# kfkq/DQMC

Measured on AMD Instinct MI355X. Metric: MC sweeps/sec, 2D Hubbard N=256 Ltau=200, higher is better.
Workload: dtype f64; 1 GPU; cfg3: 16x16 Hubbard U=8.0 beta=8.0 Ltau=200 n_stab=10 t=1 mu=-0.1; chains_per_gpu=1, n_chains_total=1, parallelism=independent chains, 1 gpu x 1 chain

## Files before the change

### dqmc_amd/csrc/common.h

```cpp
#pragma once

#include <hip/hip_runtime.h>
#include <cstdint>
#include <memory>
#include <string>

struct dqmc_engine;

namespace dq {

constexpr int WAVE = 64;

void set_error(const std::string& msg);
const char* get_error();

#define DQ_HIP(call)                                                                    \
    do {                                                                                \
        hipError_t _e = (call);                                                         \
        if (_e != hipSuccess) {                                                         \
            ::dq::set_error(std::string(#call) + ": " + hipGetErrorString(_e));         \
            return -2;                                              \
        }                                                                               \
    } while (0)

#define DQ_TRY(expr)                \
    do {                            \
        int _rc = (expr);           \
        if (_rc != 0) return _rc;   \
    } while (0)

template <class T, hipError_t (*Free)(void*)> struct HipDelete { void operator()(T* p) const { (void)Free(p); } };
template <class T> using DevPtr = std::unique_ptr<T[], HipDelete<T, hipFree>>;
using PinnedPtr = std::unique_ptr<char[], HipDelete<char, hipHostFree>>;
template <class T> int dev_alloc(DevPtr<T>& out, size_t count) {
    void* p = nullptr;
    DQ_HIP(hipMalloc(&p, sizeof(T) * count));
    out.reset(static_cast<T*>(p));
    return 0;
}

constexpr int DQ_STATUS_PIVOT = 1;
constexpr int DQ_STATUS_COOP_QR = 2;
constexpr int DQ_STATUS_HANDOFF = 4;
constexpr int DQ_STATUS_CENSUS = 8;

struct Mat {
    double* p = nullptr;
    long stride = 0;
    __host__ __device__ double* at(int c) const { return p + (long)c * stride; }
};
struct CMat {
    const double* p = nullptr;
    long stride = 0;
    CMat() = default;
    __host__ __device__ CMat(const double* p_, long s) : p(p_), stride(s) {}
    __host__ __device__ CMat(const Mat& m) : p(m.p), stride(m.stride) {}
    __host__ __device__ const double* at(int c) const { return p + (long)c * stride; }
};
using Vec = Mat;
using CVec = CMat;

struct GemmDesc {
    CMat A, B;
    Mat C;
    Mat CT{nullptr, 0};
    CVec rs, ks, cs;
    int n = 0;
    int transA = 0;
    int accumulate = 0;
};
int launch_gemm(const GemmDesc& g, int n_chains, hipStream_t s);

int launch_build_expv(const int8_t* fields, long f_stride, int nt, int n, const double* tab_expv ,
                      double* expv, double* invexpv, long v_stride, int n_chains, hipStream_t s);
int launch_split_d(CVec d, Vec dl_inv, Vec ds, double* logsum, int n, int n_chains, hipStream_t s);
int launch_split_d2(CVec d1, Vec dl1, Vec ds1, CVec d2, Vec dl2, Vec ds2, int n, int n_chains, hipStream_t s);
int launch_measure_equal_time(CMat G, double* out, long out_stride, int L1, int L2, int accumulate, int n_chains, hipStream_t s);
int launch_measure_unequal_time(const double* Gtt, const double* Gt0, const double* G0t, double* out, long out_stride, int L1, int L2, int nt,
                                int accumulate, int n_chains, hipStream_t s);
int launch_axpb_identity(CMat in, Mat out, double a, double b, int n, int n_chains, hipStream_t s);
int launch_copy(CMat in, Mat out, long count, int n_chains, hipStream_t s);
int launch_set_identity(Mat out, int n, int n_chains, hipStream_t s);
int launch_transpose_scale(CMat in, Mat out, CVec rs, int n, int n_chains, hipStream_t s);
int launch_max_abs_diff(CMat A, CMat B, double* err, long err_stride, int n, int n_chains, hipStream_t s);
int launch_add_scaled_cols(CMat A, CMat B, CVec cs, Mat C, int n, int n_chains, hipStream_t s);
int launch_scale_rows(CMat in, CVec rs, Mat out, int n, int n_chains, hipStream_t s);
struct DevStats { double acc_rate, max_err, sum_err, n_err; long long n_accepted, n_proposed; };
int launch_fold_stats(DevStats* st, const int* acc, long acc_stride, int n_slices, const double* err, long err_stride, int n_err,
                      int n, int nt, int n_chains, hipStream_t s);

struct QrWork {
    double* tau; long tau_stride;
    int* jpvt; long jpvt_stride;
    unsigned long long* sync = nullptr; long sync_stride = 0;
    int* abort_words = nullptr;
    int* info = nullptr;
    double* pw = nullptr; long pw_stride = 0;
    int* pivpos = nullptr; long pivpos_stride = 0;
};
long qr_panel_work_doubles(int n);
int launch_qr_panel(Mat A, Mat L, QrWork w, int n, int n_chains, hipStream_t s);
long qrcp_coop_sync_granules(int n);
int qrcp_coop_workgroups(int n, int n_chains);
enum class QrFamily { Panel, ColumnOwner, Cooperative, Streaming };
int launch_to_ldr(QrFamily f, Mat A, Mat L, Vec d, Mat R, QrWork w, int n, int n_chains, hipStream_t s);

int launch_lu_blocked(Mat A, int* perm, long perm_stride, int* rowpos, long rowpos_stride, double* logabsdet, int accumulate_logdet,
                      int* info, int n, int n_chains, hipStream_t s);
int launch_lu_solve(CMat LU, const int* perm, long perm_stride, Mat X, CVec dg, int mode, int n, int n_chains, hipStream_t s);

int launch_tri_solve(CMat R, const int* perm, long perm_stride, Mat X, CVec dg, double* scratch, long scratch_stride, int n, int n_chains, hipStream_t s);

int launch_gj_solve(Mat A, Mat B, Mat X, Mat SA, double* tinv, int* perm, long perm_stride, int* rowpos, long rowpos_stride,
                    double* logabsdet, int accumulate_logdet, int* info, int n, int n_chains, hipStream_t s);

struct UpdateTables {
    double rb[4][3];
    double delta[4][3];
    double ev[4];
    double iev[4];
    double pad[32];
};
struct UpdateDesc {
    Mat G;
    int8_t* fields; long f_stride;
    double* expv; double* invexpv; long v_stride;
    const UpdateTables* tabs;
    const int32_t* perm; const uint8_t* kprop; const double* u; long rs_stride;
    double* Upanel; double* Wpanel; long panel_stride;
    double* Cpanel = nullptr;
    int* state; long state_stride;
    double* prep; long prep_stride;
    Mat GT{nullptr, 0};
    int gt_valid = 0;
    void* slice_sync = nullptr;
    unsigned slice_epoch = 0;
    int slice_absent_tile = -1;
    int slice_absent_l = -1;
    int slice_late_tile = -1, slice_late_us = 0;
    int* info = nullptr;
    int* acc_out; long acc_stride;
    int n, nt;
};
constexpr int UPDATE_KD = 32;

struct SliceSync {
    unsigned long long seq; unsigned int error; unsigned int solo_count; unsigned int pad[12];
    unsigned int arrive[496];
};
constexpr size_t SLICE_SYNC_BYTES = 2048;
static_assert(sizeof(SliceSync) == SLICE_SYNC_BYTES, "SliceSync layout");
constexpr unsigned SLICE_EPOCH_LIMIT = 1u << 24;
constexpr unsigned SLICE_SOLO_BIT = 1u << 30, SLICE_FINAL_BIT = 1u << 31;
__host__ __device__ inline unsigned slice_tag(unsigned epoch, unsigned window) { return (epoch << 8) | window; }
enum class SlicePath { PersistentWalk, PersistentSubmatrix, Solo, Pairs, PairsTailSolo };
int launch_update_slice(SlicePath path, const UpdateDesc& d, int l, int acc_slot, int n_chains, hipStream_t s);
int launch_update_slice_sm(const UpdateDesc& d, int l, int acc_slot, int n_chains, hipStream_t s);
int slice_flush_workgroups(int n);
bool slice_reserve(int device, int n, int n_chains);
void slice_release(int device, int n, int n_chains);
int launch_rank1(Mat G, int i, double delta, double* scratch , long scratch_stride, int n, int n_chains, hipStream_t s);

int launch_rng_fill(int32_t* perm, uint8_t* kprop, double* u, int n, int nt, unsigned long long seed, unsigned first_chain, unsigned h,
                    int n_chains, hipStream_t s);

struct CbDesc {
    CMat in;
    Mat out{nullptr, 0}, outT{nullptr, 0};
    const int* partner = nullptr;
    int n_groups = 0, reverse = 0, inverse = 0;
    const double* par = nullptr; long par_stride = 0;
    CVec rs_in, cs_in, rs_out, cs_out;
    int n = 0;
};
int launch_cb_apply(const CbDesc& d, int n_chains, hipStream_t s);

int update_init_device();
int update_sm_init_device();
int qr_init_device();
int qr_colown_init_device();
int init_device_kernels(int device);

struct EngineFieldsView { int device, n, nt, n_chains; int8_t* fields; hipStream_t stream; };
int engine_fields_view(dqmc_engine* h, EngineFieldsView* v);
int engine_fields_changed(dqmc_engine* h);
int engine_exchange_scratch(dqmc_engine* h, int8_t** saved, int8_t** recv, int** tab);

}
```

### dqmc_amd/csrc/engine.hip

```cpp
#include "common.h"
#include "../../include/dqmc_hip.h"

#include <cmath>
#include <cstdlib>
#include <cstring>
#include <map>
#include <memory>
#include <mutex>
#include <vector>

namespace dq {

static thread_local std::string g_err;
void set_error(const std::string& msg) { g_err = msg; }
const char* get_error() { return g_err.c_str(); }

int init_device_kernels(int device) {
    static std::mutex mu; static bool done[64] = {};
    std::lock_guard<std::mutex> lk(mu);
    if (device < 0 || device >= 64) { set_error("device ordinal out of range"); return -1; }
    if (done[device]) return 0;
    DQ_HIP(hipSetDevice(device));
    DQ_TRY(update_init_device()); DQ_TRY(update_sm_init_device()); DQ_TRY(qr_init_device()); DQ_TRY(qr_colown_init_device());
    done[device] = true;
// ... 125 lines not shown
        w.pw = qpw.get(); w.pw_stride = qr_panel_work_doubles(n); w.pivpos = qpivpos.get(); w.pivpos_stride = n;
        if (out.tri) *out.tri = keep;
        out.touch();
        return launch_to_ldr(plan.qr, A, out.L, out.d, out.R, w, n, C, stream);
    }
    int r_inverse_scaled(LdrRef F, CVec dinv, Mat scratch, Mat lu_scratch, Mat* Xout) {
        const Mat X = F.X.p ? F.X : scratch;
        *Xout = X;
        if (F.xok && *F.xok) return 0;
        if (F.tri && *F.tri && F.jpvt) {
            if (plan.rinv == KernelPlan::Rinv::Blocked) DQ_TRY(launch_tri_solve(F.R, F.jpvt, n, X, dinv, trinv.get(), 16L * (n + 16), n, C, stream));
            else DQ_TRY(launch_lu_solve(F.R, F.jpvt, n, X, dinv, 2, n, C, stream));
        } else {
            DQ_TRY(launch_copy(F.R, lu_scratch, nn, C, stream));
            DQ_TRY(launch_lu_blocked(lu_scratch, lperm(), n, rowpos(), n, nullptr, 0, info(), n, C, stream));
            DQ_TRY(launch_lu_solve(lu_scratch, lperm(), n, X, dinv, 1, n, C, stream));
        }
        if (F.xok) *F.xok = true;
        return 0;
    }
    int mat_mul_ldr(CMat M, LdrRef F, LdrRef out) {
        DQ_TRY(gemm(M, F.L, T(0), CVec(), CVec(), CVec(F.d)));
        LdrRef q{out.L, out.d, T(1)};
        DQ_TRY(to_ldr(T(0), q));
        if (out.tri) *out.tri = false;
        out.touch();
        return gemm(T(1), F.R, out.R);
    }
    int ldr_mul_mat(LdrRef F, CMat M, LdrRef out) {
        DQ_TRY(gemm(F.R, M, T(0), CVec(F.d)));
        LdrRef q{T(1), out.d, out.R, out.jpvt, out.tri};
        q.xok = out.xok;
        DQ_TRY(to_ldr(T(0), q));
        return gemm(F.L, T(1), out.L);
    }
    int ldr_mul_ldr(LdrRef F1, LdrRef F2, LdrRef out) {
        DQ_TRY(gemm(F1.R, F2.L, T(0), CVec(F1.d), CVec(), CVec(F2.d)));
        LdrRef q{T(1), out.d, T(2)};
        DQ_TRY(to_ldr(T(0), q));
        if (out.tri) *out.tri = false;
        out.touch();
        DQ_TRY(gemm(F1.L, T(1), out.L));
        return gemm(T(2), F2.R, out.R);
    }
    int solve(Mat M, Mat RHS, Mat out, double* logdet_acc, Mat* Y) {
        if (plan.solve == KernelPlan::Solve::GaussJordan) {
            DQ_TRY(launch_gj_solve(M, RHS, out, T(5), tinv.get(), lperm(), n, rowpos(), n, logdet_acc, 1, info(), n, C, stream));
            *Y = out; return 0;
        }
        DQ_TRY(launch_lu_blocked(M, lperm(), n, rowpos(), n, logdet_acc, 1, info(), n, C, stream));
        DQ_TRY(launch_lu_solve(M, lperm(), n, RHS, CVec(), 0, n, C, stream));
        *Y = RHS; return 0;
    }
    int inv_I_plus_ldr(LdrRef F, Mat G, double* logdet ) {
        DQ_TRY(launch_split_d(F.d, V(0), V(1), logdet, n, C, stream));
        Mat X; DQ_TRY(r_inverse_scaled(F, V(0), T(1), T(0), &X));
        DQ_TRY(launch_add_scaled_cols(X, F.L, V(1), T(2), n, C, stream));
        DQ_TRY(launch_transpose_scale(T(2), T(3), CVec(), n, C, stream));
        DQ_TRY(launch_transpose_scale(X, T(4), CVec(), n, C, stream));
        Mat Y; DQ_TRY(solve(T(3), T(4), T(0), logdet, &Y));
        return launch_transpose_scale(Y, G, CVec(), n, C, stream);
    }
    int inv_I_plus_ldr_mul_ldr(LdrRef F1, LdrRef F2, Mat G, Mat GT = Mat{nullptr, 0}) {
        DQ_TRY(launch_split_d2(F1.d, V(0), V(1), F2.d, V(2), V(3), n, C, stream));
        Mat X; DQ_TRY(r_inverse_scaled(F2, V(2), T(1), T(0), &X));
        DQ_TRY(gemm(F1.L, X, T(2), V(0), CVec(), CVec(), 1));
        DQ_TRY(gemm(F1.R, F2.L, T(2), V(1), CVec(), V(3), 0, 1));
        DQ_TRY(launch_transpose_scale(F1.L, T(3), V(0), n, C, stream));
        Mat Y; DQ_TRY(solve(T(2), T(3), T(0), nullptr, &Y));
        return gemm(X, Y, G, CVec(), CVec(), CVec(), 0, 0, GT);
    }
    int inv_invldr_plus_ldr(LdrRef F1, LdrRef F2, Mat G, bool negate) {
        DQ_TRY(launch_split_d(F1.d, V(0), V(1), nullptr, n, C, stream));
        DQ_TRY(launch_split_d(F2.d, V(2), V(3), nullptr, n, C, stream));
        Mat X; DQ_TRY(r_inverse_scaled(F2, V(2), T(1), T(0), &X));
        DQ_TRY(gemm(F1.L, X, T(2), V(0), CVec(), CVec(), 1));
        DQ_TRY(gemm(F1.R, F2.L, T(2), V(1), CVec(), V(3), 0, 1));
        DQ_TRY(launch_scale_rows(F1.R, V(1), T(3), n, C, stream));
        Mat Y; DQ_TRY(solve(T(2), T(3), T(0), nullptr, &Y));
        DQ_TRY(gemm(X, Y, G));
        if (negate) DQ_TRY(launch_axpb_identity(G, G, -1.0, 0.0, n, C, stream));
        return 0;
    }
};

static int take_status(const Ctx& c, int* bits = nullptr) {
    int w[4] = {0, 0, 0, 0};
    DQ_HIP(hipMemcpy(w, c.info(), sizeof w, hipMemcpyDeviceToHost));
    if (bits) *bits = w[0];
    if (w[0] == 0) return 0;
    (void)hipMemset(c.info(), 0, sizeof w);
    if (w[0] & DQ_STATUS_HANDOFF) {
        set_error("persistent slice kernel: a workgroup that had checked in stopped answering (device fault or pre-emption beyond the spin bound); the chain state is undefined -- set the fields again and call dqmc_init; this engine uses the scan / flush kernel pairs from now on");
    } else if (w[0] & DQ_STATUS_CENSUS) {
        char msg[640];
        snprintf(msg, sizeof msg, "persistent sub-matrix slice kernel: its workgroups did not all become resident at time slice %d (device shared with other "
                 "work?).  That slice and every later slice of the call(s) in flight proposed NOTHING (fields unchanged there, acceptance counts 0, their part of "
                 "the random stream is spent); wraps and stabilisations ran, so fields, G and the stack are consistent with each other, but the sweep is not the "
                 "one the stream describes from that slice on.  This engine uses the scan / flush kernel pairs from now on: restore the fields of the last "
                 "completed sweep and call dqmc_init, or keep the state as a valid (shortened) sweep", w[1] - 1);
        set_error(msg);
    } else if (w[0] & DQ_STATUS_COOP_QR) {
        set_error("cooperative QRCP gave up waiting for a partner workgroup (not co-resident?)");
    } else {
        set_error("LU factorisation hit a zero or NaN pivot");
    }
    return DQMC_ENUMERIC;
}

struct Engine {
    int n = 0, nt = 0, n_stab = 0, n_stack = 0, C = 1, device = 0;
    long nn = 0;
    std::vector<int> loc_l_end;
    std::vector<double> g_host, gamma_host, eta_host;
    std::vector<unsigned char> seen;
    Ctx ctx;
    hipStream_t s = nullptr;

    DevPtr<double> expK, invexpK;
    bool cb = false; int cb_groups = 0;
    DevPtr<int> cb_partner;
    DevPtr<double> cb_par;
    DevPtr<int8_t> fields;
    DevPtr<double> expv, invexpv;
    DevPtr<UpdateTables> tabs; DevPtr<double> tab8;
    bool gt_valid = false;
    bool gt_check = false; long long gt_checks = 0; DevPtr<double> gt_err;
    DevPtr<double> G, Gtmp, GT;
    DevPtr<double> pg_eye, pg_ones;
    DevPtr<double> bb0, bb1;
    LdrStore stack;
    LdrStore spare;
    DevPtr<double> logdet;
    DevPtr<int32_t> rs_perm; DevPtr<uint8_t> rs_k; DevPtr<double> rs_u;
    PinnedPtr h_stage;
    bool rng_seeded = false; uint64_t rng_seed = 0; uint32_t rng_first_chain = 0, rng_counter = 0;
    hipEvent_t stage_free = nullptr;
    DevPtr<double> Upanel, Wpanel;
    DevPtr<double> Cpanel;
    struct InitBatch { DevPtr<double> bb, tau; LdrStore f; } ib;
    DevPtr<int> state;
    DevPtr<double> prep;
    DevPtr<double> meas_now, meas_sum;
    struct UnequalTime { DevPtr<double> G[3], tmp, err, meas_now, meas_sum; LdrStore bt; } ut;
    bool ut_valid = false; long long ut_meas_count = 0;
    struct HalfWarp { DevPtr<double> expK, invexpK, out; } hw;
    long long meas_count = 0;
    DevPtr<char> slice_sync;
    bool reserved = false;
    SlicePath slice_path = SlicePath::Pairs;
    unsigned slice_epoch = 0;
    int slice_absent_l = -1;
    int slice_late_tile = -1, slice_late_us = 0;
    int slice_absent_tile = -1;
    DevPtr<int> acc;
    struct Exchange { DevPtr<int8_t> saved, recv; DevPtr<int> tab; } xch;
    DevPtr<double> err;
    DevPtr<DevStats> dstats;
    bool stack_valid = false;
    bool profiling = false;
    std::vector<std::pair<hipEvent_t, hipEvent_t>> ev_pairs;
    size_t ev_used = 0;
    double upd_ms = 0.0; long long upd_launches = 0; long long upd_accept_base = 0;

    Mat mG() const { return Mat{G.get(), nn}; }
    CVec ev(int l) const { return CVec(expv.get() + (long)l * n, (long)nt * n); }
    CVec iev(int l) const { return CVec(invexpv.get() + (long)l * n, (long)nt * n); }
    int stack_idx(int l) const { return l / n_stab; }
    int local_l(int l) const { return l % n_stab; }

    ~Engine() {
        if (s) (void)hipStreamSynchronize(s);
        if (reserved) slice_release(device, n, C);
        for (auto& p : ev_pairs) { (void)hipEventDestroy(p.first); (void)hipEventDestroy(p.second); }
        if (stage_free) (void)hipEventDestroy(stage_free);
    }

    int create(int device_, int C_, int n_, int nt_, int n_stab_, const double* g, const double* gamma, const double* eta,
               const double* eK, const double* ieK) {
        device = device_; C = C_; n = n_; nt = nt_; n_stab = n_stab_; nn = (long)n * n;
        n_stack = (int)std::ceil(static_cast<double>(nt) / n_stab);
        loc_l_end.assign(n_stack, n_stab - 1);
        if (nt % n_stab != 0) loc_l_end[n_stack - 1] = nt % n_stab - 1;
        g_host.assign(g, g + C); gamma_host.assign(gamma, gamma + 4); eta_host.assign(eta, eta + 4);
        DQ_TRY(ctx.init(n, C, device)); s = ctx.stream;
        reserved = slice_reserve(device, n, C);
        slice_path = pick_slice_path(n, C, reserved);
        if (const char* a = getenv("DQMC_DEBUG_SLICE_ABSENT")) { slice_absent_tile = atoi(a); if (const char* c = strchr(a, ':')) slice_absent_l = atoi(c + 1); }
        if (const char* a = getenv("DQMC_DEBUG_SLICE_LATE")) { slice_late_tile = atoi(a); if (const char* c = strchr(a, ':')) slice_late_us = atoi(c + 1); }
        DQ_TRY(dev_alloc(expK, C * nn)); DQ_TRY(dev_alloc(invexpK, C * nn));
        DQ_TRY(dev_alloc(fields, (size_t)C * nt * n)); DQ_TRY(dev_alloc(expv, (size_t)C * nt * n)); DQ_TRY(dev_alloc(invexpv, (size_t)C * nt * n));
        DQ_TRY(dev_alloc(tabs, C)); DQ_TRY(dev_alloc(tab8, (size_t)C * 8));
        if (C == 1) { DQ_TRY(dev_alloc(pg_eye, nn)); DQ_TRY(dev_alloc(pg_ones, (size_t)n)); DQ_TRY(launch_set_identity(Mat{pg_eye.get(), nn}, n, 1, s)); const std::vector<double> one_h((size_t)n, 1.0); DQ_HIP(hipMemcpy(pg_ones.get(), one_h.data(), sizeof(double) * n, hipMemcpyHostToDevice)); }
        DQ_TRY(dev_alloc(G, C * nn)); DQ_TRY(dev_alloc(Gtmp, C * nn)); DQ_TRY(dev_alloc(GT, C * nn)); DQ_TRY(dev_alloc(bb0, C * nn)); DQ_TRY(dev_alloc(bb1, C * nn));
        DQ_TRY(stack.alloc(n_stack, n, C, C <= 8)); DQ_TRY(spare.alloc(1, n, C));
        DQ_TRY(dev_alloc(logdet, C));
        DQ_TRY(dev_alloc(rs_perm, (size_t)C * nt * n)); DQ_TRY(dev_alloc(rs_k, (size_t)C * nt * n)); DQ_TRY(dev_alloc(rs_u, (size_t)C * nt * n));
        DQ_TRY(dev_alloc(Upanel, (size_t)C * UPDATE_KD * n)); DQ_TRY(dev_alloc(Wpanel, (size_t)C * UPDATE_KD * n)); DQ_TRY(dev_alloc(Cpanel, (size_t)C * UPDATE_KD * UPDATE_KD));
        DQ_TRY(dev_alloc(state, (size_t)C * 4)); DQ_TRY(dev_alloc(prep, (size_t)C * 4 * n)); DQ_TRY(dev_alloc(meas_now, (size_t)C * (3 + n))); DQ_TRY(dev_alloc(meas_sum, (size_t)C * (3 + n))); DQ_HIP(hipMemsetAsync(meas_sum.get(), 0, sizeof(double) * C * (3 + n), s)); DQ_TRY(dev_alloc(slice_sync, (size_t)C * SLICE_SYNC_BYTES)); DQ_HIP(hipMemsetAsync(slice_sync.get(), 0, (size_t)C * SLICE_SYNC_BYTES, s)); DQ_TRY(dev_alloc(acc, (size_t)C * nt)); DQ_TRY(dev_alloc(err, (size_t)C * n_stack));
        DQ_TRY(dev_alloc(dstats, C));
        void* stage = nullptr;
        DQ_HIP(hipHostMalloc(&stage, (size_t)C * nt * n * (sizeof(int32_t) + sizeof(uint8_t) + sizeof(double)), hipHostMallocDefault)); h_stage.reset(static_cast<char*>(stage));
        DQ_HIP(hipEventCreateWithFlags(&stage_free, hipEventDisableTiming));
        DQ_HIP(hipEventRecord(stage_free, s));
        DQ_HIP(hipMemcpyAsync(expK.get(), eK, sizeof(double) * C * nn, hipMemcpyHostToDevice, s));
        DQ_HIP(hipMemcpyAsync(invexpK.get(), ieK, sizeof(double) * C * nn, hipMemcpyHostToDevice, s));
        DQ_HIP(hipMemsetAsync(fields.get(), 0, (size_t)C * nt * n, s));
        DQ_HIP(hipMemsetAsync(G.get(), 0, sizeof(double) * C * nn, s));
        DQ_HIP(hipMemsetAsync(dstats.get(), 0, sizeof(DevStats) * C, s));
        DQ_HIP(hipMemsetAsync(logdet.get(), 0, sizeof(double) * C, s));
        DQ_HIP(hipMemsetAsync(state.get(), 0, sizeof(int) * C * 4, s));
        std::vector<UpdateTables> ht(C); std::vector<double> h8((size_t)C * 8);
        static const int proposal[4][3] = {{1, 2, 3}, {0, 2, 3}, {0, 1, 3}, {0, 1, 2}};
        const double alpha = -1.0;
        for (int c = 0; c < C; ++c) {
            std::memset(&ht[c], 0, sizeof(UpdateTables));
            for (int o = 0; o < 4; ++o) for (int k = 0; k < 3; ++k) {
                const int nf = proposal[o][k];
                const double gammaR = gamma[nf] / gamma[o];
                const double d_eta = eta[nf] - eta[o];
                const double bosonR = std::exp(alpha * g[c] * d_eta);
                ht[c].rb[o][k] = gammaR * bosonR;
                ht[c].delta[o][k] = (1.0 / bosonR) - 1.0;
            }
            for (int f = 0; f < 4; ++f) { ht[c].ev[f] = std::exp(g[c] * eta[f]); ht[c].iev[f] = std::exp(-g[c] * eta[f]); h8[(size_t)c * 8 + f] = ht[c].ev[f]; h8[(size_t)c * 8 + 4 + f] = ht[c].iev[f]; }
        }
        DQ_HIP(hipMemcpyAsync(tabs.get(), ht.data(), sizeof(UpdateTables) * C, hipMemcpyHostToDevice, s));
        DQ_HIP(hipMemcpyAsync(tab8.get(), h8.data(), sizeof(double) * C * 8, hipMemcpyHostToDevice, s));
        DQ_TRY(launch_build_expv(fields.get(), (long)nt * n, nt, n, tab8.get(), expv.get(), invexpv.get(), (long)nt * n, C, s));
        DQ_HIP(hipStreamSynchronize(s));
        return 0;
    }

    int cb_apply(CMat in, Mat out, Mat outT, bool reverse, bool inverse, CVec rs_in, CVec cs_in, CVec rs_out, CVec cs_out, int chains, long par_stride) {
        CbDesc d; d.in = in; d.out = out; d.outT = outT; d.partner = cb_partner.get(); d.n_groups = cb_groups; d.reverse = reverse ? 1 : 0; d.inverse = inverse ? 1 : 0;
        d.par = cb_par.get(); d.par_stride = par_stride; d.rs_in = rs_in; d.cs_in = cs_in; d.rs_out = rs_out; d.cs_out = cs_out; d.n = n;
        return launch_cb_apply(d, chains, s);
    }
    int set_checkerboard(int n_groups, const int32_t* bonds, const int32_t* group_sizes, const double* ch, const double* sh, const double* f) {
        if (n_groups < 1 || n_groups > 64 || !bonds || !group_sizes || !ch || !sh || !f) { set_error("set_checkerboard: bad argument"); return DQMC_EINVAL; }
        if (n > 4096) { set_error("set_checkerboard: n_sites > 4096"); return DQMC_EINVAL; }
        std::vector<int> partner((size_t)n_groups * n);
        size_t b = 0;
        for (int g = 0; g < n_groups; ++g) {
            int* pt = partner.data() + (size_t)g * n;
            for (int i = 0; i < n; ++i) pt[i] = i;
            if (group_sizes[g] < 0 || group_sizes[g] > n / 2) { set_error("set_checkerboard: a group holds at most n_sites/2 bonds"); return DQMC_EINVAL; }
            for (int k = 0; k < group_sizes[g]; ++k, ++b) {
                const int i = bonds[2 * b], j = bonds[2 * b + 1];
                if (i < 0 || i >= n || j < 0 || j >= n || i == j) { set_error("set_checkerboard: bond site out of range"); return DQMC_EINVAL; }
                if (pt[i] != i || pt[j] != j) { set_error("set_checkerboard: the bonds of one group must be disjoint"); return DQMC_EINVAL; }
                pt[i] = j; pt[j] = i;
            }
        }
        std::vector<double> par((size_t)C * 4);
        for (int c = 0; c < C; ++c) {
            if (!(f[c] > 0.0) || !std::isfinite(ch[c]) || !std::isfinite(sh[c])) { set_error("set_checkerboard: diag_factor must be positive, cosh / sinh finite"); return DQMC_EINVAL; }
            par[4 * c] = ch[c]; par[4 * c + 1] = sh[c]; par[4 * c + 2] = f[c]; par[4 * c + 3] = 1.0 / f[c];
        }
        DQ_HIP(hipStreamSynchronize(s));
        if (!cb_par) DQ_TRY(dev_alloc(cb_par, (size_t)C * 4));
        DevPtr<int> pt;
        DQ_TRY(dev_alloc(pt, partner.size()));
        DQ_HIP(hipMemcpy(pt.get(), partner.data(), sizeof(int) * partner.size(), hipMemcpyHostToDevice));
        DQ_HIP(hipMemcpy(cb_par.get(), par.data(), sizeof(double) * par.size(), hipMemcpyHostToDevice));
        cb_partner = std::move(pt); cb_groups = n_groups; cb = true;
        Mat id{bb0.get(), nn};
        DQ_TRY(launch_set_identity(id, n, C, s));
        DQ_TRY(cb_apply(id, Mat{expK.get(), nn}, Mat{nullptr, 0}, false, false, CVec(), CVec(), CVec(), CVec(), C, 4));
        DQ_TRY(cb_apply(id, Mat{invexpK.get(), nn}, Mat{nullptr, 0}, true, true, CVec(), CVec(), CVec(), CVec(), C, 4));
        stack_valid = false; gt_valid = false; ut_valid = false;
        DQ_HIP(hipStreamSynchronize(s));
        return 0;
    }

    int Bbar(int is, Mat* out) {
        const int l0 = is * n_stab;
        Mat cur{bb0.get(), nn}, nxt{bb1.get(), nn};
        DQ_TRY(launch_scale_rows(CMat(expK.get(), nn), ev(l0), cur, n, C, s));
        for (int loc = 1; loc <= loc_l_end[is]; ++loc) {
            if (cb) DQ_TRY(cb_apply(cur, nxt, Mat{nullptr, 0}, false, false, CVec(), CVec(), ev(l0 + loc), CVec(), C, 4));
            else DQ_TRY(ctx.gemm(CMat(expK.get(), nn), cur, nxt, ev(l0 + loc)));
            std::swap(cur, nxt);
        }
        *out = cur; return 0;
    }
    int init() {
        if (C == 1 && n <= 256 && nt % n_stab == 0 && n_stack >= 2) return init_batched();
        const LdrRef tmp = spare.at(0);
        for (int i = n_stack - 1; i >= 0; --i) {
            Mat bb; DQ_TRY(Bbar(i, &bb));
            if (i == n_stack - 1) DQ_TRY(ctx.to_ldr(bb, stack.at(i)));
            else { DQ_TRY(ctx.to_ldr(bb, tmp)); DQ_TRY(ctx.ldr_mul_ldr(stack.at(i + 1), tmp, stack.at(i))); }
        }
        stack_valid = true;
        gt_valid = false;
        return ctx.inv_I_plus_ldr(stack.at(0), mG(), logdet.get());
    }
    int init_batched() {
        const int S = n_stack;
        if (!ib.tau) {
            InitBatch b; DQ_TRY(dev_alloc(b.bb, (size_t)2 * S * nn)); DQ_TRY(dev_alloc(b.tau, (size_t)S * n)); DQ_TRY(b.f.alloc(S, n, 1));
            ib = std::move(b);
        }
        const long bstride = (long)n_stab * n;
        Mat cur{ib.bb.get(), nn}, nxt{ib.bb.get() + (size_t)S * nn, nn};
        DQ_TRY(launch_scale_rows(CMat(expK.get(), 0), CVec(expv.get(), bstride), cur, n, S, s));
        for (int loc = 1; loc < n_stab; ++loc) {
            if (cb) DQ_TRY(cb_apply(cur, nxt, Mat{nullptr, 0}, false, false, CVec(), CVec(), CVec(expv.get() + (long)loc * n, bstride), CVec(), S, 0));
            else {
                GemmDesc g; g.A = CMat(expK.get(), 0); g.B = cur; g.C = nxt; g.rs = CVec(expv.get() + (long)loc * n, bstride); g.n = n;
                DQ_TRY(launch_gemm(g, S, s));
            }
            std::swap(cur, nxt);
        }
        const LdrRef all = ib.f.at(0);
        QrWork w{ib.tau.get(), (long)n, all.jpvt, (long)n};
        w.info = ctx.info();
        DQ_TRY(launch_to_ldr(pick_qr(n, S, false), cur, all.L, all.d, all.R, w, n, S, s));
        const LdrRef last = stack.at(S - 1), own = ib.f.at(S - 1);
        DQ_TRY(launch_copy(own.L, last.L, nn, 1, s));
        DQ_TRY(launch_copy(own.R, last.R, nn, 1, s));
        DQ_HIP(hipMemcpyAsync(last.d.p, own.d.p, sizeof(double) * n, hipMemcpyDeviceToDevice, s));
        DQ_HIP(hipMemcpyAsync(last.jpvt, own.jpvt, sizeof(int) * n, hipMemcpyDeviceToDevice, s));
        *last.tri = true; last.touch();
        for (int i = S - 2; i >= 0; --i) DQ_TRY(ctx.ldr_mul_ldr(stack.at(i + 1), ib.f.at(i), stack.at(i)));
        stack_valid = true;
        gt_valid = false;
        return ctx.inv_I_plus_ldr(stack.at(0), mG(), logdet.get());
    }
    int wrap_forward(int l) {
        if (cb) {
            DQ_TRY(cb_apply(mG(), Mat{nullptr, 0}, ctx.T(0), false, false, CVec(), CVec(), CVec(), CVec(), C, 4));
            gt_valid = use_gt();
            return cb_apply(ctx.T(0), Mat{GT.get(), nn}, mG(), false, true, CVec(), CVec(), iev(l), ev(l), C, 4);
        }
        DQ_TRY(ctx.gemm(CMat(expK.get(), nn), mG(), ctx.T(0)));
        gt_valid = use_gt();
        return ctx.gemm(ctx.T(0), CMat(invexpK.get(), nn), mG(), ev(l), CVec(), iev(l), 0, 0, use_gt() ? Mat{GT.get(), nn} : Mat{nullptr, 0});
    }
    bool piggyback() const { return C == 1 && !cb && n <= 256 && pg_eye != nullptr; }
    int wrap_forward_piggy(int l, const double* Pprev, double* Pnext) {
        GemmDesc g; g.A = CMat(expK.get(), 0); g.B = CMat(G.get(), (long)(Pprev - G.get())); g.C = Mat{ctx.T(0).p, (long)(Pnext - ctx.T(0).p)};
        g.rs = CVec(pg_ones.get(), (long)((expv.get() + (long)(l - 1) * n) - pg_ones.get())); g.n = n;
        DQ_TRY(launch_gemm(g, 2, s));
        gt_valid = use_gt();
        return ctx.gemm(ctx.T(0), CMat(invexpK.get(), nn), mG(), ev(l), CVec(), iev(l), 0, 0, use_gt() ? Mat{GT.get(), nn} : Mat{nullptr, 0});
    }
    int wrap_backward_piggy(int l, const double* Pprev, double* Pnext) {
        DQ_TRY(ctx.gemm(CMat(invexpK.get(), nn), mG(), ctx.T(0), CVec(), iev(l)));
        gt_valid = use_gt();
        GemmDesc g; g.A = CMat(ctx.T(0).p, (long)(Pprev - ctx.T(0).p)); g.B = CMat(expK.get(), 0); g.C = Mat{G.get(), (long)(Pnext - G.get())};
        g.ks = CVec(expv.get() + (long)l * n, 0); g.n = n;
        if (use_gt()) g.CT = Mat{GT.get(), (long)(ctx.T(1).p - GT.get())};
        return launch_gemm(g, 2, s);
    }
    int wrap_backward(int l) {
        if (cb) {
            DQ_TRY(cb_apply(mG(), Mat{nullptr, 0}, ctx.T(0), true, true, iev(l), ev(l), CVec(), CVec(), C, 4));
            gt_valid = use_gt();
            return cb_apply(ctx.T(0), Mat{GT.get(), nn}, mG(), true, false, CVec(), CVec(), CVec(), CVec(), C, 4);
        }
        DQ_TRY(ctx.gemm(CMat(invexpK.get(), nn), mG(), ctx.T(0), CVec(), iev(l)));
        gt_valid = use_gt();
        return ctx.gemm(ctx.T(0), CMat(expK.get(), nn), mG(), CVec(), ev(l), CVec(), 0, 0, use_gt() ? Mat{GT.get(), nn} : Mat{nullptr, 0});
    }
    bool use_gt() const { return n <= 256 || slice_path == SlicePath::PersistentSubmatrix; }
    UpdateDesc udesc() const {
        UpdateDesc d; d.G = mG(); d.fields = fields.get(); d.f_stride = (long)nt * n; d.expv = expv.get(); d.invexpv = invexpv.get(); d.v_stride = (long)nt * n;
        d.tabs = tabs.get(); d.perm = rs_perm.get(); d.kprop = rs_k.get(); d.u = rs_u.get(); d.rs_stride = (long)nt * n; d.Upanel = Upanel.get(); d.Wpanel = Wpanel.get(); d.Cpanel = Cpanel.get();
        d.panel_stride = (long)UPDATE_KD * n; d.state = state.get(); d.state_stride = 4; d.prep = prep.get(); d.prep_stride = 4L * n; d.slice_sync = is_persistent(slice_path) ? slice_sync.get() : nullptr; d.slice_epoch = slice_epoch; d.slice_absent_tile = slice_absent_tile; d.slice_absent_l = slice_absent_l; d.slice_late_tile = slice_late_tile; d.slice_late_us = slice_late_us; d.GT = Mat{GT.get(), nn}; d.gt_valid = gt_valid ? 1 : 0; d.info = ctx.info(); d.acc_out = acc.get(); d.acc_stride = nt; d.n = n; d.nt = nt;
        return d;
    }
    int local_update(int l) {
        hipEvent_t e0 = nullptr, e1 = nullptr;
        if (profiling) {
            if (ev_used == ev_pairs.size()) { hipEvent_t a, b; DQ_HIP(hipEventCreate(&a)); DQ_HIP(hipEventCreate(&b)); ev_pairs.emplace_back(a, b); }
            e0 = ev_pairs[ev_used].first; e1 = ev_pairs[ev_used].second; ++ev_used;
            DQ_HIP(hipEventRecord(e0, s));
        }
        if (is_persistent(slice_path)) {
            if (++slice_epoch >= SLICE_EPOCH_LIMIT) { DQ_HIP(hipMemsetAsync(slice_sync.get(), 0, (size_t)C * SLICE_SYNC_BYTES, s)); slice_epoch = 1; }
        }
        DQ_TRY(launch_update_slice(slice_path, udesc(), l, l, C, s));
        if (profiling) DQ_HIP(hipEventRecord(e1, s));
        return 0;
    }
    int check_stream(const char* who, const int32_t* perm, const uint8_t* kprop, const double* u, size_t rows) {
        if (!perm || !kprop || !u) { set_error(std::string(who) + ": null random-stream pointer"); return DQMC_EINVAL; }
        seen.assign((size_t)n, 0);
        for (size_t row = 0; row < rows; ++row) {
            const int32_t* pr = perm + row * n; const uint8_t* kr = kprop + row * n; const unsigned char mark = (unsigned char)(1 + (row & 1));
            if ((row & 1) == 0) std::fill(seen.begin(), seen.end(), 0);
            for (int idx = 0; idx < n; ++idx) {
                const int32_t i = pr[idx];
                if (i < 0 || i >= n || seen[i] == mark || kr[idx] > 2) { set_error(std::string(who) + ": perm is not a permutation of the sites, or kprop > 2"); return DQMC_EINVAL; }
                seen[i] = mark;
            }
        }
        return 0;
    }
    int upload_stream(const int32_t* perm, const uint8_t* kprop, const double* u) {
        const size_t cnt = (size_t)C * nt * n;
        DQ_TRY(check_stream("sweep", perm, kprop, u, (size_t)C * nt));
        DQ_HIP(hipEventSynchronize(stage_free));
        char* base = h_stage.get();
        double* hu = reinterpret_cast<double*>(base);
        int32_t* hp = reinterpret_cast<int32_t*>(base + cnt * sizeof(double));
        uint8_t* hk = reinterpret_cast<uint8_t*>(base + cnt * (sizeof(double) + sizeof(int32_t)));
        std::memcpy(hu, u, cnt * sizeof(double)); std::memcpy(hp, perm, cnt * sizeof(int32_t)); std::memcpy(hk, kprop, cnt);
        DQ_HIP(hipMemcpyAsync(rs_u.get(), hu, cnt * sizeof(double), hipMemcpyHostToDevice, s));
        DQ_HIP(hipMemcpyAsync(rs_perm.get(), hp, cnt * sizeof(int32_t), hipMemcpyHostToDevice, s));
        DQ_HIP(hipMemcpyAsync(rs_k.get(), hk, cnt, hipMemcpyHostToDevice, s));
        DQ_HIP(hipEventRecord(stage_free, s));
        return 0;
    }
    int fill_stream(uint32_t h) {
        return launch_rng_fill(rs_perm.get(), rs_k.get(), rs_u.get(), n, nt, rng_seed, rng_first_chain, h, C, s);
    }
    int stage_stream(const char* who, const int32_t* perm, const uint8_t* kprop, const double* u) {
        if (perm && kprop && u) return upload_stream(perm, kprop, u);
        if (perm || kprop || u) { set_error(std::string(who) + ": pass all three random-stream arrays or none"); return DQMC_EINVAL; }
        if (!rng_seeded) { set_error(std::string(who) + ": null random-stream pointer (the engine draws its own stream only after dqmc_rng_seed)"); return DQMC_EINVAL; }
        if (rng_counter == UINT32_MAX) { set_error(std::string(who) + ": the half-sweep counter of this seed is used up (2^32 - 1)"); return DQMC_ERANGE; }
        DQ_TRY(fill_stream(rng_counter));
        ++rng_counter;
        return 0;
    }
    int sweep_fwd() {
        int n_err = 0;
        DQ_HIP(hipMemsetAsync(err.get(), 0, sizeof(double) * C * n_stack, s));
        const bool pg = piggyback();
        double* Pcur = bb0.get(); double* Pnxt = bb1.get();
        for (int l = 0; l < nt; ++l) {
            const int is = stack_idx(l), loc = local_l(l);
            if (pg && loc >= 1) { DQ_TRY(wrap_forward_piggy(l, loc == 1 ? pg_eye.get() : Pcur, Pnxt)); std::swap(Pcur, Pnxt); }
            else DQ_TRY(wrap_forward(l));
            DQ_TRY(local_update(l));
            if (loc == loc_l_end[is]) {
                std::swap(G, Gtmp);
                Mat bb;
                if (pg) {
                    if (loc == 0) DQ_TRY(launch_scale_rows(CMat(expK.get(), nn), ev(l), Mat{Pnxt, nn}, n, C, s));
                    else DQ_TRY(ctx.gemm(CMat(expK.get(), nn), CMat(Pcur, nn), Mat{Pnxt, nn}, ev(l)));
                    std::swap(Pcur, Pnxt); bb = Mat{Pcur, nn};
                } else DQ_TRY(Bbar(is, &bb));
                if (is == 0) DQ_TRY(ctx.to_ldr(bb, stack.at(0)));
                else DQ_TRY(ctx.mat_mul_ldr(bb, stack.at(is - 1), stack.at(is)));
                gt_valid = false;
                if (l == nt - 1) DQ_TRY(ctx.inv_I_plus_ldr(stack.at(is), mG(), logdet.get()));
                else DQ_TRY(ctx.inv_I_plus_ldr_mul_ldr(stack.at(is), stack.at(is + 1), mG()));
                DQ_TRY(launch_max_abs_diff(CMat(Gtmp.get(), nn), mG(), err.get() + n_err, n_stack, n, C, s));
                ++n_err;
            }
        }
        return launch_fold_stats(dstats.get(), acc.get(), nt, nt, err.get(), n_stack, n_err, n, nt, C, s);
    }
    int sweep_bwd() {
        int n_err = 0;
        DQ_HIP(hipMemsetAsync(err.get(), 0, sizeof(double) * C * n_stack, s));
        const bool pg = piggyback();
        double* Pcur = bb0.get(); double* Pnxt = bb1.get();
        for (int l = nt - 1; l >= 0; --l) {
            DQ_TRY(local_update(l));
            const int is = stack_idx(l);
            if (pg) { DQ_TRY(wrap_backward_piggy(l, local_l(l) == loc_l_end[is] ? pg_eye.get() : Pcur, Pnxt)); std::swap(Pcur, Pnxt); }
            else DQ_TRY(wrap_backward(l));
            if (local_l(l) == 0) {
                std::swap(G, Gtmp);
                Mat bb;
                if (pg) bb = Mat{Pcur, nn}; else DQ_TRY(Bbar(is, &bb));
                if (is == n_stack - 1) DQ_TRY(ctx.to_ldr(bb, stack.at(is)));
                else DQ_TRY(ctx.ldr_mul_mat(stack.at(is + 1), bb, stack.at(is)));
                gt_valid = false;
                if (l == 0) DQ_TRY(ctx.inv_I_plus_ldr(stack.at(is), mG(), logdet.get()));
                else {
                    DQ_TRY(ctx.inv_I_plus_ldr_mul_ldr(stack.at(is - 1), stack.at(is), mG(), use_gt() ? Mat{GT.get(), nn} : Mat{nullptr, 0}));
                    gt_valid = use_gt();
                    if (gt_check && gt_valid) {
                        DQ_TRY(launch_transpose_scale(mG(), ctx.T(0), CVec(), n, C, s));
                        DQ_TRY(launch_max_abs_diff(CMat(GT.get(), nn), ctx.T(0), gt_err.get(), 1, n, C, s));
                        ++gt_checks;
                    }
                }
                DQ_TRY(launch_max_abs_diff(CMat(Gtmp.get(), nn), mG(), err.get() + n_err, n_stack, n, C, s));
                ++n_err;
            }
        }
        return launch_fold_stats(dstats.get(), acc.get(), nt, nt, err.get(), n_stack, n_err, n, nt, C, s);
    }
    Mat utm(int which, int l) const { return Mat{ut.G[which].get() + (long)l * C * nn, nn}; }
    int sweep_unequal() {
        if (!ut.tmp) {
            UnequalTime u;
            for (int w = 0; w < 3; ++w) DQ_TRY(dev_alloc(u.G[w], (size_t)(nt + 1) * C * nn));
            DQ_TRY(dev_alloc(u.tmp, (size_t)3 * C * nn)); DQ_TRY(dev_alloc(u.err, (size_t)C * 3 * n_stack));
            const size_t mcount = (size_t)C * 3 * (nt + 1) * n;
            DQ_TRY(dev_alloc(u.meas_now, mcount)); DQ_TRY(dev_alloc(u.meas_sum, mcount)); DQ_TRY(u.bt.alloc(2, n, C));
            DQ_HIP(hipMemsetAsync(u.meas_sum.get(), 0, sizeof(double) * mcount, s));
            ut = std::move(u);
        }
        auto bt = [&](int b) { return ut.bt.at(b); };
        int cur = 0, n_err = 0;
        DQ_HIP(hipMemsetAsync(ut.err.get(), 0, sizeof(double) * C * 3 * n_stack, s));
        DQ_TRY(launch_copy(mG(), utm(0, 0), nn, C, s));
        for (int l = 0; l < nt; ++l) {
            if (l == 0) {
                DQ_TRY(launch_copy(utm(0, 0), utm(1, 0), nn, C, s));
                DQ_TRY(launch_axpb_identity(utm(0, 0), utm(2, 0), 1.0, -1.0, n, C, s));
            }
            DQ_TRY(ctx.gemm(CMat(expK.get(), nn), utm(0, l), ctx.T(0)));
            DQ_TRY(ctx.gemm(ctx.T(0), CMat(invexpK.get(), nn), utm(0, l + 1), ev(l), CVec(), iev(l)));
            DQ_TRY(ctx.gemm(CMat(expK.get(), nn), utm(1, l), utm(1, l + 1), ev(l)));
            DQ_TRY(ctx.gemm(utm(2, l), CMat(invexpK.get(), nn), utm(2, l + 1), CVec(), CVec(), iev(l)));
            const int is = stack_idx(l);
            if (local_l(l) == loc_l_end[is]) {
                for (int w = 0; w < 3; ++w) DQ_TRY(launch_copy(utm(w, l + 1), Mat{ut.tmp.get() + (long)w * C * nn, nn}, nn, C, s));
                Mat bb; DQ_TRY(Bbar(is, &bb));
                if (is == 0) DQ_TRY(ctx.to_ldr(bb, bt(cur)));
                else { DQ_TRY(ctx.mat_mul_ldr(bb, bt(cur), bt(cur ^ 1))); cur ^= 1; }
                if (l == nt - 1) {
                    DQ_TRY(ctx.inv_I_plus_ldr(bt(cur), utm(0, l + 1), logdet.get()));
                    DQ_TRY(launch_axpb_identity(utm(0, l + 1), utm(1, l + 1), -1.0, 1.0, n, C, s));
                    DQ_TRY(launch_axpb_identity(utm(0, l + 1), utm(2, l + 1), -1.0, 0.0, n, C, s));
// ... 502 lines not shown
```

### dqmc_amd/csrc/update.hip

```cpp
#include "common.h"
#include <cstdlib>
#include <mutex>
#include "wave.h"

namespace dq {

using d4 = __attribute__((ext_vector_type(4))) double;

__constant__ int c_proposal[4][3] = {{1, 2, 3}, {0, 2, 3}, {0, 1, 3}, {0, 1, 2}};

constexpr int SCAN_PF = 8;

__device__ __forceinline__ double ld_coh(const double* p) {
    return __longlong_as_double((long long)__hip_atomic_load(reinterpret_cast<const unsigned long long*>(p), __ATOMIC_RELAXED, __HIP_MEMORY_SCOPE_AGENT));
}
__device__ __forceinline__ void st_coh(double* p, double x) {
    __hip_atomic_store(reinterpret_cast<unsigned long long*>(p), (unsigned long long)__double_as_longlong(x), __ATOMIC_RELAXED, __HIP_MEMORY_SCOPE_AGENT);
}

__host__ __device__ inline size_t scan_lds_bytes(int n, int kd, bool regs) {
    const size_t base = (((size_t)16 * kd * n + (size_t)n * 32 + 256 + (size_t)n * 4 + (size_t)n) + 63) & ~(size_t)63;
    return base + (regs ? (size_t)n * 8 + 4 * (UPDATE_KD + 4) : 0);
}

__device__ __forceinline__ void lds_barrier() {
    asm volatile("s_waitcnt lgkmcnt(0)" ::: "memory");
    __builtin_amdgcn_s_barrier();
    asm volatile("" ::: "memory");
}

struct ScanShared {
    double2* UW; double* diag; double* dlt; double* rbv; double* ur; double* tl; int* site; signed char* newf;
    double* diag2 = nullptr;
    int* acc_site = nullptr;
};

template <bool COH>
__device__ __forceinline__ void scan_prefetch(double (&pc)[SCAN_PF], double (&pr)[SCAN_PF], const double* __restrict__ G, const ScanShared& sh,
                                              int g, int n, int j, bool live) {
#pragma unroll
    for (int q = 0; q < SCAN_PF; ++q) {
        const int pos = min(g * SCAN_PF + q, n - 1);
        const int jj = live ? j : n - 1;
        const int i = sh.site[pos];
        if (COH) { pc[q] = ld_coh(G + jj + (long)n * i); pr[q] = ld_coh(G + i + (long)n * jj); }
        else { pc[q] = G[jj + (long)n * i]; pr[q] = G[i + (long)n * jj]; }
    }
}

#ifdef DQ_SCAN_STAMPS
#define STAMP(v) { unsigned long long _t; asm volatile("s_memtime %0\n\ts_waitcnt lgkmcnt(0)" : "=s"(_t) :: "memory"); v = _t; }
struct ScanProf { unsigned long long t_rej = 0, t_kloop = 0, t_tail = 0, t_wait = 0, t_first = 0, t_dump = 0, t_noacc = 0, t_pub = 0, t_fin = 0, t_finwait = 0; int n_rej = 0, n_acc = 0, n_noacc = 0, n_pub = 0, n_fin_k = 0, n_fin_g = 0, n_fin_e = 0; };
#define PROF_ARG , ScanProf& prof
#else
#define PROF_ARG
#endif
template <bool COH>
__device__ __forceinline__ bool scan_group(const double (&pc)[SCAN_PF], const double (&pr)[SCAN_PF], const ScanShared& sh, int g, int n, int kd,
                                           int j, bool live, int& pos, int& k, const UpdateDesc& d, long slice_off, int chain, int8_t* fields_g,
                                           double* __restrict__ Up, double* __restrict__ Wp PROF_ARG) {
#pragma unroll
    for (int q = 0; q < SCAN_PF; ++q) {
        const int mypos = g * SCAN_PF + q;
        if (mypos < pos) continue;
        if (mypos >= n || k >= kd) return false;
#ifdef DQ_SCAN_STAMPS
        unsigned long long t0, t1, t2, t3; STAMP(t0)
#endif
        const int i = sh.site[mypos];
        const double delta = sh.dlt[mypos];
        const double r = 1.0 + (1.0 - sh.diag[i]) * delta;
        const double R = sh.rbv[mypos] * (r * r);
        const double pacc = fmin(1.0, fabs(R));
        if (sh.ur[mypos] < pacc) {
            const double pref = delta / r;
            double uj = pc[q], wj = pr[q];
#ifdef DQ_SCAN_STAMPS
            asm volatile("s_waitcnt vmcnt(0)" ::: "memory"); STAMP(t1)
#endif
            if (live) {
                const double2* own_p = sh.UW + j;
                const double2* piv_p = sh.UW + i;
                double u1 = 0.0, w1 = 0.0, u2 = 0.0, w2 = 0.0, u3 = 0.0, w3 = 0.0;
                int m = 0;
                for (; m + 8 <= k; m += 8) {
                    double2 o[8], pv[8];
#pragma unroll
                    for (int e = 0; e < 8; ++e) { const int off = (m + e) * n; o[e] = own_p[off]; pv[e] = piv_p[off]; }
                    uj += o[0].x * pv[0].y; wj += pv[0].x * o[0].y; u1 += o[1].x * pv[1].y; w1 += pv[1].x * o[1].y;
                    u2 += o[2].x * pv[2].y; w2 += pv[2].x * o[2].y; u3 += o[3].x * pv[3].y; w3 += pv[3].x * o[3].y;
                    uj += o[4].x * pv[4].y; wj += pv[4].x * o[4].y; u1 += o[5].x * pv[5].y; w1 += pv[5].x * o[5].y;
                    u2 += o[6].x * pv[6].y; w2 += pv[6].x * o[6].y; u3 += o[7].x * pv[7].y; w3 += pv[7].x * o[7].y;
                }
                if (m < k) {
                    double2 o[8], pv[8];
#pragma unroll
                    for (int e = 0; e < 8; ++e) {
                        const int mm = (m + e < k) ? m + e : m;
                        const int off = mm * n; o[e] = own_p[off]; pv[e] = piv_p[off];
                    }
#pragma unroll
                    for (int e = 1; e < 8; ++e) if (m + e >= k) { o[e].x = 0.0; o[e].y = 0.0; }
                    uj += o[0].x * pv[0].y; wj += pv[0].x * o[0].y; u1 += o[1].x * pv[1].y; w1 += pv[1].x * o[1].y;
                    u2 += o[2].x * pv[2].y; w2 += pv[2].x * o[2].y; u3 += o[3].x * pv[3].y; w3 += pv[3].x * o[3].y;
                    uj += o[4].x * pv[4].y; wj += pv[4].x * o[4].y; u1 += o[5].x * pv[5].y; w1 += pv[5].x * o[5].y;
                    u2 += o[6].x * pv[6].y; w2 += pv[6].x * o[6].y; u3 += o[7].x * pv[7].y; w3 += pv[7].x * o[7].y;
                }
                uj += (u1 + u2) + u3; wj += (w1 + w2) + w3;
                if (j == i) wj -= 1.0;
            }
#ifdef DQ_SCAN_STAMPS
            STAMP(t2)
#endif
            lds_barrier();
            if (live) {
                const double pu = pref * uj;
                sh.UW[k * n + j] = make_double2(pu, wj);
                sh.diag[j] += pu * wj;
                if (COH) { st_coh(Up + k * n + j, pu); st_coh(Wp + k * n + j, wj); }
                else { Up[k * n + j] = pu; Wp[k * n + j] = wj; }
                if (j == i) {
                    const int new_f = sh.newf[mypos];
                    fields_g[i] = (int8_t)new_f;
                    d.expv[(long)chain * d.v_stride + slice_off + i] = sh.tl[24 + new_f];
                    d.invexpv[(long)chain * d.v_stride + slice_off + i] = sh.tl[28 + new_f];
                }
            }
            ++k;
            lds_barrier();
#ifdef DQ_SCAN_STAMPS
            STAMP(t3) prof.t_wait += t1 - t0; prof.t_kloop += t2 - t1; prof.t_tail += t3 - t2; prof.n_acc++;
        } else { STAMP(t1) prof.t_rej += t1 - t0; prof.n_rej++;
#endif
        }
        pos = mypos + 1;
    }
    return true;
}


#define DQ_WALK_REGS __attribute__((amdgpu_num_vgpr(128)))
#ifndef DQ_W6_KPUB
#define DQ_W6_KPUB 24
#define DQ_W6_XOVER 8
#endif
#define DQ_W6_CAT2(a, b) a##b
#define DQ_W6_CAT(a, b) DQ_W6_CAT2(a, b)
#define DQ_W6_REBASE DQ_W6_CAT(DQ_W6_REBASE_, DQ_W6_KPUB)
#include "walk_bodies.inc"
#pragma clang diagnostic ignored "-Winline-asm"

template <bool COH>
__device__ __forceinline__ void walk6_load_group(const double* __restrict__ G, const double* __restrict__ GT, const ScanShared& sh, int g, int gs, int n, int j, bool live) {
    const unsigned jj8 = (unsigned)(live ? j : n - 1) * 8u, n8 = (unsigned)n * 8u;
    const int ig = sh.site[min(g * 8 + (int)(threadIdx.x & 7), n - 1)];
    const unsigned igs = (unsigned)ig * n8;
    unsigned off8[8];
    asm("s_nop 1\n\t"
        "v_add_u32_dpp %0, %8, %9 row_newbcast:0 row_mask:0xf bank_mask:0xf\n\tv_add_u32_dpp %1, %8, %9 row_newbcast:1 row_mask:0xf bank_mask:0xf\n\t"
        "v_add_u32_dpp %2, %8, %9 row_newbcast:2 row_mask:0xf bank_mask:0xf\n\tv_add_u32_dpp %3, %8, %9 row_newbcast:3 row_mask:0xf bank_mask:0xf\n\t"
        "v_add_u32_dpp %4, %8, %9 row_newbcast:4 row_mask:0xf bank_mask:0xf\n\tv_add_u32_dpp %5, %8, %9 row_newbcast:5 row_mask:0xf bank_mask:0xf\n\t"
        "v_add_u32_dpp %6, %8, %9 row_newbcast:6 row_mask:0xf bank_mask:0xf\n\tv_add_u32_dpp %7, %8, %9 row_newbcast:7 row_mask:0xf bank_mask:0xf"
        : "=&v"(off8[0]), "=&v"(off8[1]), "=&v"(off8[2]), "=&v"(off8[3]), "=&v"(off8[4]), "=&v"(off8[5]), "=&v"(off8[6]), "=&v"(off8[7])
        : "v"(igs), "v"(jj8));
    if (gs == 0) { if (COH) { DQ_W6_LOADSET_0_COH } else { DQ_W6_LOADSET_0_PLAIN } }
    else if (gs == 1) { if (COH) { DQ_W6_LOADSET_1_COH } else { DQ_W6_LOADSET_1_PLAIN } }
    else { if (COH) { DQ_W6_LOADSET_2_COH } else { DQ_W6_LOADSET_2_PLAIN } }
}

constexpr unsigned SLICE_SPIN_LIMIT = 1u << 22;
constexpr unsigned SLICE_CENSUS_SPINS = 256;

__device__ __attribute__((noinline)) void solo_flush(double* G, double* GT, const double2* UW, int n, int k);
__device__ __forceinline__ bool slice_census_missing(SliceSync* sy, unsigned epoch, int F, unsigned first, int* flag) {
    const int lane = threadIdx.x & 63, wave = threadIdx.x >> 6;
    if (wave == 0) {
        unsigned spins = 0; bool all_in = __all(first == slice_tag(epoch, 0));
        while (!all_in) {
            if (++spins > SLICE_CENSUS_SPINS) break;
            __builtin_amdgcn_s_sleep(8);
            const unsigned a = lane < F ? __hip_atomic_load(&sy->arrive[lane], __ATOMIC_RELAXED, __HIP_MEMORY_SCOPE_AGENT) : slice_tag(epoch, 0);
            all_in = __all(a == slice_tag(epoch, 0));
        }
        if (lane == 0) *flag = all_in ? 0 : 1;
    }
    __syncthreads();
    const bool missing = *flag != 0;
    __syncthreads();
    return missing;
}
__device__ __forceinline__ void slice_wait_arrivals(SliceSync* sy, unsigned epoch, unsigned win, int F, int* info) {
    const int lane = threadIdx.x & 63, wave = threadIdx.x >> 6;
    if (wave == 0) {
        unsigned spins = 0; bool broken = false;
        for (;;) {
            const unsigned a = lane < F ? __hip_atomic_load(&sy->arrive[lane], __ATOMIC_RELAXED, __HIP_MEMORY_SCOPE_AGENT) : slice_tag(epoch, win);
            if (__all(a == slice_tag(epoch, win))) break;
            if (++spins > SLICE_SPIN_LIMIT) { broken = true; break; }
            __builtin_amdgcn_s_sleep(1);
        }
        if (broken && lane == 0) { __hip_atomic_store(&sy->error, 1u, __ATOMIC_RELAXED, __HIP_MEMORY_SCOPE_AGENT); if (info) atomicOr(info, DQ_STATUS_HANDOFF); }
    }
    __syncthreads();
}

struct NoAsync { static constexpr bool enabled = false; };
__device__ __forceinline__ bool as_inflight(const NoAsync&) { return false; }
struct SliceAsync {
    static constexpr bool enabled = true;
    SliceSync* sy; unsigned epoch; int F; int* info; int* flag;
    unsigned win = 1;
    int published = 0;
    bool solo = false;
    bool inflight = false;
    int g_limit = 0;
};

__device__ __forceinline__ bool as_inflight(const SliceAsync& a) { return a.inflight; }

template <bool COH, bool PANELS = true, class AS = NoAsync>
__device__ __forceinline__ int walk_window6(const ScanShared& sh, int& pos, double& dg, int n, int kd, int j, bool live, const double* __restrict__ G,
                                            const double* __restrict__ GT, const UpdateDesc& d, long slice_off, int chain, int8_t* fields_g,
                                            double* __restrict__ Up, double* __restrict__ Wp, AS& as PROF_ARG) {
    const int lane = threadIdx.x & 63, r16 = lane & 15, q8 = lane & 7;
    DQ_W6_RESERVE;
    int par = 0, k = 0;
#ifdef DQ_SCAN_STAMPS
#define DQ_ST(...) __VA_ARGS__
#else
#define DQ_ST(...)
#endif
    auto async_finish = [&]() {
        if constexpr (AS::enabled) {
            DQ_ST(unsigned long long tf0, tf1, tf2; STAMP(tf0))
            slice_wait_arrivals(as.sy, as.epoch, as.win, as.F, as.info);
            DQ_ST(STAMP(tf1))
            DQ_W6_REBASE;
            if (live) for (int t = 0; t < k - DQ_W6_KPUB; ++t) sh.UW[t * n + j] = sh.UW[(DQ_W6_KPUB + t) * n + j];
            if (j < k - DQ_W6_KPUB) sh.acc_site[j] = sh.acc_site[DQ_W6_KPUB + j];
            k -= DQ_W6_KPUB; ++as.win; as.inflight = false;
            lds_barrier();
            DQ_ST(STAMP(tf2) prof.t_finwait += tf1 - tf0; prof.t_fin += tf2 - tf1;)
        }
    };
    int g = pos >> 3;
    bool done = false;
    asm volatile("s_waitcnt vmcnt(0)" ::: "memory");
    __builtin_amdgcn_s_waitcnt(0x0F70);
    walk6_load_group<COH>(G, GT, sh, g, g % 3, n, j, live);
    walk6_load_group<COH>(G, GT, sh, g + 1, (g + 1) % 3, n, j, live);
    while (!done) {
        DQ_ST(unsigned long long tg0, tg1; STAMP(tg0))
        const int gs = g % 3;
        if constexpr (AS::enabled) {
            if (as.inflight && g > as.g_limit) {
                DQ_ST(prof.n_fin_g++;)
                async_finish();
                walk6_load_group<COH>(G, GT, sh, g, gs, n, j, live);
                walk6_load_group<COH>(G, GT, sh, g + 1, (g + 1) % 3, n, j, live);
            }
            if (!as.inflight) walk6_load_group<COH>(G, GT, sh, g + 2, (g + 2) % 3, n, j, live);
        } else
        walk6_load_group<COH>(G, GT, sh, g + 2, (g + 2) % 3, n, j, live);
        DQ_ST(STAMP(tg1) prof.t_first += tg1 - tg0;)
        const int gbase = g * 8;
        const int p_l = gbase + q8, pc_l = min(p_l, n - 1);
        const int i_l = sh.site[pc_l];
        const double dl_l = sh.dlt[pc_l], rb_l = sh.rbv[pc_l], ur_l = sh.ur[pc_l];
        for (;;) {
            DQ_ST(unsigned long long t0, t1, t2, t3; STAMP(t0))
            const double* dcur = par ? sh.diag2 : sh.diag;
            const double r_l = 1.0 + (1.0 - dcur[i_l]) * dl_l;
            const double R_l = rb_l * (r_l * r_l);
            const bool acc_l = p_l >= pos && p_l < n && ur_l < fmin(1.0, fabs(R_l));
            const unsigned bal = (unsigned)__ballot(acc_l) & 0xffu;
            if (bal == 0u) { pos = min(gbase + 8, n); DQ_ST(STAMP(t1) prof.t_noacc += t1 - t0; prof.n_noacc++;) break; }
            const int first = __ffs((int)bal) - 1;
            const int p = gbase + first;
            pos = p + 1;
            const int i = __builtin_amdgcn_readlane(i_l, first);
            const double dl_p = readlane_f64(dl_l, first), r_p = readlane_f64(r_l, first);
            const int kc = max(k - 1, 0);
            const double2 pa = sh.UW[min(r16, kc) * n + i], pb = sh.UW[min(16 + r16, kc) * n + i];
            const double pref = dl_p / r_p;
            int ulo, uhi, wlo, whi;
            asm volatile("s_waitcnt vmcnt(32)" ::: "memory");
            DQ_W6_PICK(gs * 8 + first);
            double uj = __hiloint2double(uhi, ulo), wj = __hiloint2double(whi, wlo);
            DQ_ST(STAMP(t1))
            {
                double u1 = 0.0, w1 = 0.0;
                DQ_W6_PAIRS;
                uj += u1; wj += w1;
                if (j == i) wj -= 1.0;
                const double pu = pref * uj;
                dg += pu * wj;
                if (live) { sh.UW[k * n + j] = make_double2(pu, wj); (par ? sh.diag : sh.diag2)[j] = dg; }
                if (j == 0) sh.acc_site[k] = p;
                DQ_W6_SETPAIR(pu, wj);
            }
            DQ_ST(STAMP(t2))
            ++k; par ^= 1;
            lds_barrier();
            DQ_ST(STAMP(t3) prof.t_wait += t1 - t0; prof.t_kloop += t2 - t1; prof.t_tail += t3 - t2; prof.n_acc++;)
            if constexpr (AS::enabled) {
                if (k == DQ_W6_KPUB && kd == UPDATE_KD && !as.inflight && !as.solo && pos < n) {
                    DQ_ST(unsigned long long tp0, tp1; STAMP(tp0))
                    if (live) DQ_W6_DUMP_PUB;
                    if (j < DQ_W6_KPUB) {
                        const int pp = sh.acc_site[j];
                        const int ii = sh.site[pp], new_f = sh.newf[pp];
                        fields_g[ii] = (int8_t)new_f;
                        d.expv[(long)chain * d.v_stride + slice_off + ii] = sh.tl[24 + new_f];
                        d.invexpv[(long)chain * d.v_stride + slice_off + ii] = sh.tl[28 + new_f];
                    }
                    unsigned census = slice_tag(as.epoch, 0);
                    if (as.win == 1 && threadIdx.x < (unsigned)as.F) census = __hip_atomic_load(&as.sy->arrive[threadIdx.x], __ATOMIC_RELAXED, __HIP_MEMORY_SCOPE_AGENT);
                    asm volatile("s_waitcnt vmcnt(0)" ::: "memory");
                    __syncthreads();
                    if (as.win == 1 && slice_census_missing(as.sy, as.epoch, as.F, census, as.flag)) {
                        as.solo = true;
                        if (threadIdx.x == 0) {
                            __hip_atomic_store(&as.sy->seq, ((unsigned long long)slice_tag(as.epoch, as.win) << 32) | SLICE_SOLO_BIT | (unsigned)k, __ATOMIC_RELAXED, __HIP_MEMORY_SCOPE_AGENT);
                            __hip_atomic_fetch_add(&as.sy->solo_count, 1u, __ATOMIC_RELAXED, __HIP_MEMORY_SCOPE_AGENT);
                        }
                        solo_flush(const_cast<double*>(G), const_cast<double*>(GT), sh.UW, n, k);
                        asm volatile("s_waitcnt vmcnt(0)" ::: "memory");
                        __syncthreads();
                        as.published += k; k = 0; ++as.win;
                        walk6_load_group<COH>(G, GT, sh, g, gs, n, j, live);
                        walk6_load_group<COH>(G, GT, sh, g + 1, (g + 1) % 3, n, j, live);
                        walk6_load_group<COH>(G, GT, sh, g + 2, (g + 2) % 3, n, j, live);
                    } else {
                        if (threadIdx.x == 0)
                            __hip_atomic_store(&as.sy->seq, ((unsigned long long)slice_tag(as.epoch, as.win) << 32) | (unsigned)DQ_W6_KPUB, __ATOMIC_RELAXED, __HIP_MEMORY_SCOPE_AGENT);
                        as.published += DQ_W6_KPUB; as.inflight = true; as.g_limit = g + 2;
                    }
                    DQ_ST(STAMP(tp1) prof.t_pub += tp1 - tp0; prof.n_pub++;)
                }
                if (k >= kd || (as.inflight && k >= DQ_W6_KPUB + DQ_W6_XOVER)) {
                    if (!as.inflight) { done = true; break; }
                    DQ_ST(prof.n_fin_k++;)
                    async_finish();
                    walk6_load_group<COH>(G, GT, sh, g, gs, n, j, live);
                    walk6_load_group<COH>(G, GT, sh, g + 1, (g + 1) % 3, n, j, live);
                    walk6_load_group<COH>(G, GT, sh, g + 2, (g + 2) % 3, n, j, live);
                }
            } else
            if (k >= kd) { done = true; break; }
        }
        if (pos >= n) done = true;
        ++g;
    }
    if constexpr (AS::enabled) { if (as.inflight) { DQ_ST(prof.n_fin_e++;) async_finish(); } }
#undef DQ_ST
#ifdef DQ_SCAN_STAMPS
    unsigned long long td0; STAMP(td0)
#endif
    if (PANELS && live) DQ_W6_DUMP;
    if (j < k) {
        const int p = sh.acc_site[j];
        const int i = sh.site[p], new_f = sh.newf[p];
        fields_g[i] = (int8_t)new_f;
        d.expv[(long)chain * d.v_stride + slice_off + i] = sh.tl[24 + new_f];
        d.invexpv[(long)chain * d.v_stride + slice_off + i] = sh.tl[28 + new_f];
    }
#ifdef DQ_SCAN_STAMPS
    { asm volatile("s_waitcnt vmcnt(0)" ::: "memory"); unsigned long long td1; STAMP(td1) prof.t_dump += td1 - td0; }
#endif
    return k;
}

__device__ __forceinline__ void scan_shared_init(ScanShared& sh, unsigned char* smem, int n, int kd, bool regs) {
    sh.UW = reinterpret_cast<double2*>(smem);
    sh.diag = reinterpret_cast<double*>(sh.UW + (size_t)kd * n);
    sh.dlt = sh.diag + n; sh.rbv = sh.dlt + n; sh.ur = sh.rbv + n; sh.tl = sh.ur + n;
    sh.site = reinterpret_cast<int*>(sh.tl + 32);
    sh.newf = reinterpret_cast<signed char*>(sh.site + n);
    if (regs) { sh.diag2 = reinterpret_cast<double*>(smem + scan_lds_bytes(n, kd, false)); sh.acc_site = reinterpret_cast<int*>(sh.diag2 + n); }
}

template <int MAXT>
__global__ __launch_bounds__(MAXT) DQ_WALK_REGS void scan_kernel(UpdateDesc d, int l, int acc_slot, int first, int kd) {
    extern __shared__ __attribute__((aligned(16))) unsigned char smem[];
    const int chain = blockIdx.y;
    const int n = d.n;
    const int j = threadIdx.x;
    const bool live = j < n;
    constexpr bool REGS = MAXT <= 256;

    ScanShared sh;
    scan_shared_init(sh, smem, n, kd, REGS);

    double* __restrict__ G = d.G.at(chain);
    int* state = d.state + (long)chain * d.state_stride;
    const double* tab_g = reinterpret_cast<const double*>(d.tabs + chain);
    const long slice_off = (long)l * n;
    int8_t* fields_g = d.fields + (long)chain * d.f_stride + slice_off;

    int pos = first ? 0 : state[0];
    if (pos >= n) {
        if (j == 0) state[1] = 0;
        return;
    }
    if (live) {
        double* prep = d.prep + (long)chain * d.prep_stride;
        if (first) {
            const long off = (long)chain * d.rs_stride + slice_off + j;
            const int i = d.perm[off];
            const int kp = d.kprop[off];
            const int old_f = fields_g[i];
            const int new_f = c_proposal[old_f][kp];
            const double rb = tab_g[old_f * 3 + kp], dl = tab_g[12 + old_f * 3 + kp], uu = d.u[off];
            sh.site[j] = i; sh.newf[j] = (signed char)new_f; sh.rbv[j] = rb; sh.dlt[j] = dl; sh.ur[j] = uu;
            prep[j] = __longlong_as_double(((long long)new_f << 32) | (unsigned int)i);
            prep[n + j] = dl; prep[2 * n + j] = rb; prep[3 * n + j] = uu;
        } else {
            const long long pk = __double_as_longlong(prep[j]);
            sh.site[j] = (int)(pk & 0xffffffffLL); sh.newf[j] = (signed char)(pk >> 32);
            sh.dlt[j] = prep[n + j]; sh.rbv[j] = prep[2 * n + j]; sh.ur[j] = prep[3 * n + j];
        }
        sh.diag[j] = G[j + (long)n * j];
    }
    if (j < 32) sh.tl[j] = tab_g[j];
    __syncthreads();

    int k = 0;
    double* __restrict__ Up = d.Upanel + (long)chain * d.panel_stride;
    double* __restrict__ Wp = d.Wpanel + (long)chain * d.panel_stride;
#ifdef DQ_SCAN_STAMPS
    ScanProf prof; unsigned long long tk0; STAMP(tk0)
#define PROF_PASS , prof
#else
#define PROF_PASS
#endif
    if constexpr (REGS) {
        const double* __restrict__ GT = d.GT.at(chain);
        double dg0 = live ? sh.diag[j] : 0.0;
        { NoAsync na; k = walk_window6<false>(sh, pos, dg0, n, kd, j, live, G, GT, d, slice_off, chain, fields_g, Up, Wp, na PROF_PASS); }
    } else {
        double pcA[SCAN_PF], prA[SCAN_PF], pcB[SCAN_PF], prB[SCAN_PF];
        int g = pos / SCAN_PF;
        scan_prefetch<false>(pcA, prA, G, sh, g, n, j, live);
        scan_prefetch<false>(pcB, prB, G, sh, g + 1, n, j, live);
        for (;;) {
            if (!scan_group<false>(pcA, prA, sh, g, n, kd, j, live, pos, k, d, slice_off, chain, fields_g, Up, Wp PROF_PASS)) break;
            scan_prefetch<false>(pcA, prA, G, sh, g + 2, n, j, live);
            if (!scan_group<false>(pcB, prB, sh, g + 1, n, kd, j, live, pos, k, d, slice_off, chain, fields_g, Up, Wp PROF_PASS)) break;
            scan_prefetch<false>(pcB, prB, G, sh, g + 3, n, j, live);
            g += 2;
        }
    }
    if (j == 0) {
        state[0] = pos;
        state[1] = k;
        int* acc = d.acc_out + (long)chain * d.acc_stride + acc_slot;
        *acc = (first ? 0 : *acc) + k;
#ifdef DQ_SCAN_STAMPS
        unsigned long long tk1; STAMP(tk1)
        printf("scan l=%d first=%d: total %llu cyc | %d rej %llu cyc | %d acc: wait %llu kloop %llu tail %llu\n", l, first, tk1 - tk0,
               prof.n_rej, prof.t_rej, prof.n_acc, prof.t_wait, prof.t_kloop, prof.t_tail);
#endif
    }
}

template <bool COH, bool WITH_GT, bool PAIRED>
__device__ __forceinline__ void flush_tile(double* __restrict__ G, double* __restrict__ GT, const double* __restrict__ Up, const double* __restrict__ Wp,
                                           int a0, int b0, int n, int k, int kd, int lane) {
    const int r = lane & 15, kk = lane >> 4;
    const int a = min(a0 + r, n - 1), b = min(b0 + r, n - 1);
    const bool a_ok = a0 + r < n, b_ok = b0 + r < n;
    double uv[UPDATE_KD / 4], wv[UPDATE_KD / 4], gv[4], gt[4];
#pragma unroll
    for (int s = 0; s < UPDATE_KD / 4; ++s) {
        const int m = min(4 * s + kk, kd - 1);
        const int ib = PAIRED ? (m >> 1) * 2 * n + 2 * b + (m & 1) : m * n + b, ia = PAIRED ? (m >> 1) * 2 * n + 2 * a + (m & 1) : m * n + a;
        if (COH) { wv[s] = ld_coh(Wp + ib); uv[s] = ld_coh(Up + ia); }
        else { wv[s] = Wp[ib]; uv[s] = Up[ia]; }
    }
#pragma unroll
    for (int reg = 0; reg < 4; ++reg) {
        const int bb = min(b0 + kk + 4 * reg, n - 1), aa = min(a0 + kk + 4 * reg, n - 1);
        if (COH) { gv[reg] = ld_coh(G + a + (long)n * bb); if (WITH_GT) gt[reg] = ld_coh(GT + b + (long)n * aa); }
        else { gv[reg] = G[a + (long)n * bb]; if (WITH_GT) gt[reg] = GT[b + (long)n * aa]; }
    }
    if (k == 0) return;
    d4 acc = {0.0, 0.0, 0.0, 0.0}, acc_t = {0.0, 0.0, 0.0, 0.0};
#pragma unroll
    for (int s = 0; s < UPDATE_KD / 4; ++s) {
        const bool ok = 4 * s + kk < k;
        const double wm = (ok && b_ok) ? wv[s] : 0.0, um = (ok && a_ok) ? uv[s] : 0.0;
        acc = __builtin_amdgcn_mfma_f64_16x16x4f64(wm, um, acc, 0, 0, 0);
        if (WITH_GT) acc_t = __builtin_amdgcn_mfma_f64_16x16x4f64(um, wm, acc_t, 0, 0, 0);
    }
#pragma unroll
    for (int reg = 0; reg < 4; ++reg) {
        const int bb = b0 + kk + 4 * reg, aa = a0 + kk + 4 * reg;
        if (a_ok && bb < n) { if (COH) st_coh(G + a + (long)n * bb, gv[reg] + acc[reg]); else G[a + (long)n * bb] = gv[reg] + acc[reg]; }
        if (WITH_GT && b_ok && aa < n) { if (COH) st_coh(GT + b + (long)n * aa, gt[reg] + acc_t[reg]); else GT[b + (long)n * aa] = gt[reg] + acc_t[reg]; }
    }
}

template <bool WITH_GT>
__global__ __launch_bounds__(256) void flush_kernel(UpdateDesc d, int tiles_per_dim, int kd) {
    const int chain = blockIdx.y;
    const int n = d.n;
    const int lane = threadIdx.x & 63, wave = threadIdx.x >> 6;
    const int a0 = (blockIdx.x % tiles_per_dim) * 32 + (wave & 1) * 16;
    const int b0 = (blockIdx.x / tiles_per_dim) * 32 + (wave >> 1) * 16;
    if (a0 >= n || b0 >= n) return;
    const int k = __builtin_amdgcn_readfirstlane(d.state[(long)chain * d.state_stride + 1]);
    if (k == 0) return;
    flush_tile<false, WITH_GT, WITH_GT>(d.G.at(chain), WITH_GT ? d.GT.at(chain) : nullptr, d.Upanel + (long)chain * d.panel_stride, d.Wpanel + (long)chain * d.panel_stride,
                               a0, b0, n, k, kd, lane);
}

template <int NB>
__device__ __forceinline__ void flush_tiles_lds(double* __restrict__ G, double* __restrict__ GT, const double2* __restrict__ UW, int st0, int st_step,
                                                int n_st, int tiles16, int n, int k, int lane) {
    const int r = lane & 15, kk = lane >> 4;
    double gv[NB][4], gt[NB][4];
#pragma unroll
    for (int q = 0; q < NB; ++q) {
        const int st = min(st0 + q * st_step, n_st - 1);
        const int a0 = (st % tiles16) * 16, b0 = (st / tiles16) * 16;
        const int a = min(a0 + r, n - 1), b = min(b0 + r, n - 1);
#pragma unroll
        for (int reg = 0; reg < 4; ++reg) {
            const int bb = min(b0 + kk + 4 * reg, n - 1), aa = min(a0 + kk + 4 * reg, n - 1);
            gv[q][reg] = G[a + (long)n * bb]; gt[q][reg] = GT[b + (long)n * aa];
        }
    }
#pragma unroll
    for (int q = 0; q < NB; ++q) {
        const int st = st0 + q * st_step;
        if (st >= n_st) break;
        const int a0 = (st % tiles16) * 16, b0 = (st / tiles16) * 16;
        const int a = min(a0 + r, n - 1), b = min(b0 + r, n - 1);
        const bool a_ok = a0 + r < n, b_ok = b0 + r < n;
        d4 acc = {0.0, 0.0, 0.0, 0.0}, acc_t = {0.0, 0.0, 0.0, 0.0};
#pragma unroll
        for (int s = 0; s < UPDATE_KD / 4; ++s) {
            if (4 * s >= k) break;
            const int m = 4 * s + kk;
            const bool ok = m < k;
            const int mc = min(m, k - 1);
            const double um = (ok && a_ok) ? UW[mc * n + a].x : 0.0, wm = (ok && b_ok) ? UW[mc * n + b].y : 0.0;
            acc = __builtin_amdgcn_mfma_f64_16x16x4f64(wm, um, acc, 0, 0, 0);
            acc_t = __builtin_amdgcn_mfma_f64_16x16x4f64(um, wm, acc_t, 0, 0, 0);
        }
#pragma unroll
        for (int reg = 0; reg < 4; ++reg) {
            const int bb = b0 + kk + 4 * reg, aa = a0 + kk + 4 * reg;
            if (a_ok && bb < n) G[a + (long)n * bb] = gv[q][reg] + acc[reg];
            if (b_ok && aa < n) GT[b + (long)n * aa] = gt[q][reg] + acc_t[reg];
        }
    }
}

__device__ __attribute__((noinline)) void solo_flush(double* G, double* GT, const double2* UW, int n, int k) {
    const int lane = threadIdx.x & 63, wave = threadIdx.x >> 6;
    const int tiles16 = (n + 15) / 16, n_st = tiles16 * tiles16;
    for (int st = wave; st < n_st; st += 4 * 4) flush_tiles_lds<4>(G, GT, UW, st, 4, n_st, tiles16, n, k, lane);
}

template <int NFIX, int KFIX>
__global__ __launch_bounds__(256) DQ_WALK_REGS void slice_kernel(UpdateDesc d, SliceSync* sync_p, int l, int acc_slot, int kd_arg, int tiles_arg, int* info) {
    extern __shared__ __attribute__((aligned(16))) unsigned char smem[];
    const int chain = blockIdx.y;
    const int n = NFIX ? NFIX : d.n;
    const int kd = KFIX ? KFIX : kd_arg;
    const int tiles_per_dim = NFIX ? (NFIX + 31) / 32 : tiles_arg;
    const int F = tiles_per_dim * tiles_per_dim;
    SliceSync* sy = sync_p + chain;
    double* __restrict__ G = d.G.at(chain);
    double* __restrict__ GT = d.GT.at(chain);
    double* __restrict__ Up = d.Upanel + (long)chain * d.panel_stride;
    double* __restrict__ Wp = d.Wpanel + (long)chain * d.panel_stride;
    const int t = threadIdx.x, lane = t & 63, wave = t >> 6;
    const unsigned epoch = d.slice_epoch;

    if (blockIdx.x > 0) {
        const int tile = blockIdx.x - 1;
        if (tile == d.slice_absent_tile && (d.slice_absent_l < 0 || d.slice_absent_l == l)) return;
        if (tile == d.slice_late_tile) {
            const unsigned long long t0 = wall_clock64();
            while (wall_clock64() - t0 < 100ull * (unsigned long long)d.slice_late_us) __builtin_amdgcn_s_sleep(64);
        }
        const int a0 = (tile % tiles_per_dim) * 32 + (wave & 1) * 16;
        const int b0 = (tile / tiles_per_dim) * 32 + (wave >> 1) * 16;
        if (t == 0) __hip_atomic_store(&sy->arrive[tile], slice_tag(epoch, 0), __ATOMIC_RELAXED, __HIP_MEMORY_SCOPE_AGENT);
        unsigned long long* bcast = reinterpret_cast<unsigned long long*>(smem);
        for (unsigned win = 1;; ++win) {
            if (wave == 0) {
                unsigned long long word = 0; unsigned spins = 0; bool give_up = false;
                for (;;) {
                    word = __hip_atomic_load(&sy->seq, __ATOMIC_RELAXED, __HIP_MEMORY_SCOPE_AGENT);
                    const unsigned tag = (unsigned)(word >> 32);
                    if (tag == slice_tag(epoch, win)) break;
                    if ((tag >> 8) == (slice_tag(epoch, 0) >> 8)) {
                        if ((unsigned)word & SLICE_SOLO_BIT) break;
                        if ((tag & 0xffu) > win) { give_up = true; break; }
                    }
                    if (++spins > SLICE_SPIN_LIMIT) { give_up = true; break; }
                    __builtin_amdgcn_s_sleep(1);
                }
                if (give_up && lane == 0) { __hip_atomic_store(&sy->error, 1u, __ATOMIC_RELAXED, __HIP_MEMORY_SCOPE_AGENT); if (info) atomicOr(info, DQ_STATUS_HANDOFF); }
                if (lane == 0) bcast[win & 1] = give_up ? ~0ULL : word;
            }
            __syncthreads();
            const unsigned long long word = bcast[win & 1];
            if (word == ~0ULL) break;
            const unsigned lo = (unsigned)word;
            if (lo & SLICE_SOLO_BIT) break;
            const int k = (int)(lo & 0x3fffffffu);
            const bool final = (lo & SLICE_FINAL_BIT) != 0;
            if (k > 0 && a0 < n && b0 < n) flush_tile<true, true, true>(G, GT, Up, Wp, a0, b0, n, k, kd, lane);
            if (final) break;
            asm volatile("s_waitcnt vmcnt(0)" ::: "memory");
            __syncthreads();
            if (t == 0) __hip_atomic_store(&sy->arrive[tile], slice_tag(epoch, win), __ATOMIC_RELAXED, __HIP_MEMORY_SCOPE_AGENT);
        }
    } else {
        const int j = t;
        const bool live = j < n;
        ScanShared sh;
        scan_shared_init(sh, smem, n, kd, true);
        const double* tab_g = reinterpret_cast<const double*>(d.tabs + chain);
        const long slice_off = (long)l * n;
        int8_t* fields_g = d.fields + (long)chain * d.f_stride + slice_off;
        double dg = 0.0;
        if (live) {
            const long off = (long)chain * d.rs_stride + slice_off + j;
            const int i = d.perm[off];
            const int kp = d.kprop[off];
            const int old_f = fields_g[i];
            sh.site[j] = i; sh.newf[j] = (signed char)c_proposal[old_f][kp];
            sh.rbv[j] = tab_g[old_f * 3 + kp]; sh.dlt[j] = tab_g[12 + old_f * 3 + kp]; sh.ur[j] = d.u[off];
            dg = G[j + (long)n * j];
            sh.diag[j] = dg;
        }
        if (j < 32) sh.tl[j] = tab_g[j];
        __syncthreads();
        int pos = 0, total_acc = 0;
        int* flag = sh.acc_site + UPDATE_KD;
#ifdef DQ_SCAN_STAMPS
        ScanProf prof; unsigned long long tk0, t_hand = 0; STAMP(tk0)
#endif
        SliceAsync as{sy, epoch, F, info, flag};
        for (;; ++as.win) {
            const int k = walk_window6<true, true, SliceAsync>(sh, pos, dg, n, kd, j, live, G, GT, d, slice_off, chain, fields_g, Up, Wp, as PROF_PASS);
            total_acc += k + as.published; as.published = 0;
            const unsigned win = as.win;
            bool solo = as.solo;
            const bool final = pos >= n;
#ifdef DQ_SCAN_STAMPS
            unsigned long long th0; STAMP(th0)
#endif
            unsigned census = slice_tag(epoch, 0);
            if (win == 1 && wave == 0 && lane < F) census = __hip_atomic_load(&sy->arrive[lane], __ATOMIC_RELAXED, __HIP_MEMORY_SCOPE_AGENT);
            asm volatile("s_waitcnt vmcnt(0)" ::: "memory");
            __syncthreads();
            if (win == 1) { solo = slice_census_missing(sy, epoch, F, census, flag); as.solo = solo; }
            if (t == 0) {
                __hip_atomic_store(&sy->seq, ((unsigned long long)slice_tag(epoch, win) << 32) | (final ? SLICE_FINAL_BIT : 0u) | (solo ? SLICE_SOLO_BIT : 0u) | (unsigned)k,
                                   __ATOMIC_RELAXED, __HIP_MEMORY_SCOPE_AGENT);
                if (solo && win == 1) __hip_atomic_fetch_add(&sy->solo_count, 1u, __ATOMIC_RELAXED, __HIP_MEMORY_SCOPE_AGENT);
            }
            if (solo) {
                if (k > 0) solo_flush(G, GT, sh.UW, n, k);
                if (final) break;
                asm volatile("s_waitcnt vmcnt(0)" ::: "memory");
                __syncthreads();
                if (live) sh.diag[j] = dg;
                __syncthreads();
                continue;
            }
            if (final) break;
            slice_wait_arrivals(sy, epoch, win, F, info);
            if (live) sh.diag[j] = dg;
            __syncthreads();
#ifdef DQ_SCAN_STAMPS
            { unsigned long long th1; STAMP(th1) t_hand += th1 - th0; }
#endif
        }
        if (j == 0) d.acc_out[(long)chain * d.acc_stride + acc_slot] = total_acc;
#ifdef DQ_SCAN_STAMPS
        if (j == 0) { unsigned long long tk1; STAMP(tk1)
#if 1
            printf("slice l=%d: total %llu cyc | hand-offs %llu | %d acc: decide+fetch %llu pairs %llu tail %llu | window start->first flip %llu | %d empty passes %llu | dump+drain %llu | %d async publishes %llu, finishes (full %d / columns %d / end %d): wait %llu rebase %llu\n",
                   l, tk1 - tk0, t_hand, prof.n_acc, prof.t_wait, prof.t_kloop, prof.t_tail, prof.t_first, prof.n_noacc, prof.t_noacc, prof.t_dump,
                   prof.n_pub, prof.t_pub, prof.n_fin_k, prof.n_fin_g, prof.n_fin_e, prof.t_finwait, prof.t_fin);
#endif
        }
#endif
    }
}

__global__ __launch_bounds__(256) DQ_WALK_REGS void slice_solo_kernel(UpdateDesc d, int l, int acc_slot, int kd, int resume) {
    extern __shared__ __attribute__((aligned(16))) unsigned char smem[];
    const int chain = blockIdx.y;
    const int n = d.n;
    double* __restrict__ G = d.G.at(chain);
    double* __restrict__ GT = d.GT.at(chain);
    const int j = threadIdx.x, lane = j & 63, wave = j >> 6;
    const bool live = j < n;
    int pos = resume ? d.state[(long)chain * d.state_stride] : 0;
    if (pos >= n) return;
    ScanShared sh;
    scan_shared_init(sh, smem, n, kd, true);
    const double* tab_g = reinterpret_cast<const double*>(d.tabs + chain);
    const long slice_off = (long)l * n;
    int8_t* fields_g = d.fields + (long)chain * d.f_stride + slice_off;
    double dg = 0.0;
    if (live) {
        const long off = (long)chain * d.rs_stride + slice_off + j;
        const int i = d.perm[off];
        const int kp = d.kprop[off];
        const int old_f = fields_g[i];
        sh.site[j] = i; sh.newf[j] = (signed char)c_proposal[old_f][kp];
        sh.rbv[j] = tab_g[old_f * 3 + kp]; sh.dlt[j] = tab_g[12 + old_f * 3 + kp]; sh.ur[j] = d.u[off];
        dg = G[j + (long)n * j];
        sh.diag[j] = dg;
    }
    if (j < 32) sh.tl[j] = tab_g[j];
    __syncthreads();
    int total_acc = 0;
    const int tiles16 = (n + 15) / 16;
#ifdef DQ_SCAN_STAMPS
    ScanProf prof;
#endif
    for (;;) {
        NoAsync na; const int k = walk_window6<false, false>(sh, pos, dg, n, kd, j, live, G, GT, d, slice_off, chain, fields_g, nullptr, nullptr, na PROF_PASS);
        total_acc += k;
        __syncthreads();
        if (k > 0) {
            const int n_st = tiles16 * tiles16;
            for (int st = wave; st < n_st; st += 4 * 8) flush_tiles_lds<8>(G, GT, sh.UW, st, 4, n_st, tiles16, n, k, lane);
        }
        if (pos >= n) break;
        __syncthreads();
        if (live) { dg = G[j + (long)n * j]; sh.diag[j] = dg; }
        __syncthreads();
    }
    if (j == 0) { int* acc = d.acc_out + (long)chain * d.acc_stride + acc_slot; *acc = (resume ? *acc : 0) + total_acc; }
}

static int pick_kd(int n) {
    const long budget = 150 * 1024 - (long)n * 48 - 1024;
    long kd = budget / (16L * n);
    if (kd > UPDATE_KD) kd = UPDATE_KD;
    if (kd < 1) kd = 1;
    return (int)kd;
}

static std::mutex g_resv_mu;
static int g_resv_used[64] = {};
static int g_resv_cap[64] = {};
int slice_workgroups(int n, int n_chains) { return (1 + slice_flush_workgroups(n)) * n_chains; }
bool slice_reserve(int device, int n, int n_chains) {
    if (device < 0 || device >= 64 || n > 1024) return false;
    std::lock_guard<std::mutex> lk(g_resv_mu);
    if (g_resv_cap[device] == 0) {
        hipDeviceProp_t prop;
        if (hipGetDeviceProperties(&prop, device) != hipSuccess) return false;
        const char* m = getenv("DQMC_SLICE_CU_MARGIN");
        g_resv_cap[device] = prop.multiProcessorCount - (m ? atoi(m) : 32);
    }
    const int want = slice_workgroups(n, n_chains);
    if (g_resv_used[device] + want > g_resv_cap[device]) return false;
    g_resv_used[device] += want;
    return true;
}
void slice_release(int device, int n, int n_chains) {
    if (device < 0 || device >= 64) return;
    std::lock_guard<std::mutex> lk(g_resv_mu);
    g_resv_used[device] -= slice_workgroups(n, n_chains);
}

int update_init_device() {
    DQ_HIP(hipFuncSetAttribute(reinterpret_cast<const void*>(scan_kernel<256>), hipFuncAttributeMaxDynamicSharedMemorySize, 160 * 1024));
    DQ_HIP(hipFuncSetAttribute(reinterpret_cast<const void*>(scan_kernel<1024>), hipFuncAttributeMaxDynamicSharedMemorySize, 160 * 1024));
    DQ_HIP(hipFuncSetAttribute(reinterpret_cast<const void*>(slice_kernel<0, 0>), hipFuncAttributeMaxDynamicSharedMemorySize, 160 * 1024));
    DQ_HIP(hipFuncSetAttribute(reinterpret_cast<const void*>(slice_kernel<256, UPDATE_KD>), hipFuncAttributeMaxDynamicSharedMemorySize, 160 * 1024));
    DQ_HIP(hipFuncSetAttribute(reinterpret_cast<const void*>(slice_solo_kernel), hipFuncAttributeMaxDynamicSharedMemorySize, 160 * 1024));
    return 0;
}

int launch_update_slice(SlicePath path, const UpdateDesc& d, int l, int acc_slot, int n_chains, hipStream_t s) {
    const int n = d.n;
    if (n > 1024) { set_error("local update kernel supports n_sites <= 1024"); return -1; }
    const int kd = pick_kd(n);
    const int threads = ((n + 63) / 64) * 64;
    const bool regs = threads <= 256;
    const size_t lds = scan_lds_bytes(n, kd, regs);
    const int tiles = (n + 31) / 32;
    if (!regs && path != SlicePath::Pairs && path != SlicePath::PersistentSubmatrix) { set_error("local update: the walk kernels of update.hip need n_sites <= 256"); return -1; }
    if (regs || path == SlicePath::PersistentSubmatrix) {
        if (!d.GT.p) { set_error("local update: transposed workspace missing"); return -1; }
        if (!d.gt_valid) { if (int rc = launch_transpose_scale(CMat(d.G.p, d.G.stride), d.GT, CVec(), n, n_chains, s)) return rc; }
    }
    switch (path) {
    case SlicePath::PersistentSubmatrix: return launch_update_slice_sm(d, l, acc_slot, n_chains, s);
    case SlicePath::PersistentWalk:
        if (!d.slice_sync) { set_error("persistent slice kernel: hand-off words missing"); return -1; }
        if (n == 256 && kd == UPDATE_KD)
            hipLaunchKernelGGL((slice_kernel<256, UPDATE_KD>), dim3(1 + tiles * tiles, n_chains), dim3(256), lds, s, d, reinterpret_cast<SliceSync*>(d.slice_sync), l, acc_slot, kd,
                               tiles, d.info);
        else
            hipLaunchKernelGGL((slice_kernel<0, 0>), dim3(1 + tiles * tiles, n_chains), dim3(256), lds, s, d, reinterpret_cast<SliceSync*>(d.slice_sync), l, acc_slot, kd,
                               tiles, d.info);
        DQ_HIP(hipGetLastError());
        return 0;
    case SlicePath::Solo:
        hipLaunchKernelGGL(slice_solo_kernel, dim3(1, n_chains), dim3(256), lds, s, d, l, acc_slot, kd, 0);
        DQ_HIP(hipGetLastError());
        return 0;
    case SlicePath::Pairs: case SlicePath::PairsTailSolo: break;
    }
    int windows = (n + kd - 1) / kd;
    const bool tail_solo = path == SlicePath::PairsTailSolo && windows > 4;
    if (tail_solo) windows = 4;
    for (int w = 0; w < windows; ++w) {
        if (regs) {
            hipLaunchKernelGGL(scan_kernel<256>, dim3(1, n_chains), dim3(threads), lds, s, d, l, acc_slot, w == 0 ? 1 : 0, kd);
            hipLaunchKernelGGL(flush_kernel<true>, dim3(tiles * tiles, n_chains), dim3(256), 0, s, d, tiles, kd);
        } else {
            hipLaunchKernelGGL(scan_kernel<1024>, dim3(1, n_chains), dim3(threads), lds, s, d, l, acc_slot, w == 0 ? 1 : 0, kd);
            hipLaunchKernelGGL(flush_kernel<false>, dim3(tiles * tiles, n_chains), dim3(256), 0, s, d, tiles, kd);
        }
    }
    if (tail_solo) {
        hipLaunchKernelGGL(slice_solo_kernel, dim3(1, n_chains), dim3(256), lds, s, d, l, acc_slot, kd, 1);
    }
    DQ_HIP(hipGetLastError());
    return 0;
}

__global__ void rank1_gather_kernel(Mat G, int i, double delta, double* scratch, long scratch_stride, int n) {
    const int c = blockIdx.y;
    const double* g = G.at(c);
    double* sc = scratch + (long)c * scratch_stride;
    for (int j = threadIdx.x; j < n; j += blockDim.x) {
        sc[j] = g[j + (long)n * i];
        sc[n + j] = g[i + (long)n * j] - (j == i ? 1.0 : 0.0);
// ... 24 lines not shown
```

### dqmc_amd/csrc/walk_bodies.inc

```
#define DQ_W6_RESERVE asm volatile("" ::: "v128", "v129", "v130", "v131", "v132", "v133", "v134", "v135", "v136", "v137", "v138", "v139", "v140", "v141", "v142", "v143", "v144", "v145", "v146", "v147", "v148", "v149", "v150", "v151", "v152", "v153", "v154", "v155", "v156", "v157", "v158", "v159", "v160", "v161", "v162", "v163", "v164", "v165", "v166", "v167", "v168", "v169", "v170", "v171", "v172", "v173", "v174", "v175", "v176", "v177", "v178", "v179", "v180", "v181", "v182", "v183", "v184", "v185", "v186", "v187", "v188", "v189", "v190", "v191", "v192", "v193", "v194", "v195", "v196", "v197", "v198", "v199", "v200", "v201", "v202", "v203", "v204", "v205", "v206", "v207", "v208", "v209", "v210", "v211", "v212", "v213", "v214", "v215", "v216", "v217", "v218", "v219", "v220", "v221", "v222", "v223", "v224", "v225", "v226", "v227", "v228", "v229", "v230", "v231", "v232", "v233", "v234", "v235", "v236", "v237", "v238", "v239", "v240", "v241", "v242", "v243", "v244", "v245", "v246", "v247", "v248", "v249", "v250", "v251", "v252", "v253", "v254", "v255", "a128", "a129", "a130", "a131", "a132", "a133", "a134", "a135", "a136", "a137", "a138", "a139", "a140", "a141", "a142", "a143", "a144", "a145", "a146", "a147", "a148", "a149", "a150", "a151", "a152", "a153", "a154", "a155", "a156", "a157", "a158", "a159", "a160", "a161", "a162", "a163", "a164", "a165", "a166", "a167", "a168", "a169", "a170", "a171", "a172", "a173", "a174", "a175", "a176", "a177", "a178", "a179", "a180", "a181", "a182", "a183", "a184", "a185", "a186", "a187", "a188", "a189", "a190", "a191", "a192", "a193", "a194", "a195", "a196", "a197", "a198", "a199", "a200", "a201", "a202", "a203", "a204", "a205", "a206", "a207", "a208", "a209", "a210", "a211", "a212", "a213", "a214", "a215", "a216", "a217", "a218", "a219", "a220", "a221", "a222", "a223")
#define DQ_W6_LOADSET_0_PLAIN asm volatile("global_load_dwordx2 a[128:129], %0, %1\n\tglobal_load_dwordx2 a[130:131], %0, %2" :: "v"(off8[0]), "s"(G), "s"(GT)); asm volatile("global_load_dwordx2 a[132:133], %0, %1\n\tglobal_load_dwordx2 a[134:135], %0, %2" :: "v"(off8[1]), "s"(G), "s"(GT)); asm volatile("global_load_dwordx2 a[136:137], %0, %1\n\tglobal_load_dwordx2 a[138:139], %0, %2" :: "v"(off8[2]), "s"(G), "s"(GT)); asm volatile("global_load_dwordx2 a[140:141], %0, %1\n\tglobal_load_dwordx2 a[142:143], %0, %2" :: "v"(off8[3]), "s"(G), "s"(GT)); asm volatile("global_load_dwordx2 a[144:145], %0, %1\n\tglobal_load_dwordx2 a[146:147], %0, %2" :: "v"(off8[4]), "s"(G), "s"(GT)); asm volatile("global_load_dwordx2 a[148:149], %0, %1\n\tglobal_load_dwordx2 a[150:151], %0, %2" :: "v"(off8[5]), "s"(G), "s"(GT)); asm volatile("global_load_dwordx2 a[152:153], %0, %1\n\tglobal_load_dwordx2 a[154:155], %0, %2" :: "v"(off8[6]), "s"(G), "s"(GT)); asm volatile("global_load_dwordx2 a[156:157], %0, %1\n\tglobal_load_dwordx2 a[158:159], %0, %2" :: "v"(off8[7]), "s"(G), "s"(GT));
#define DQ_W6_LOADSET_0_COH asm volatile("global_load_dwordx2 a[128:129], %0, %1 sc1\n\tglobal_load_dwordx2 a[130:131], %0, %2 sc1" :: "v"(off8[0]), "s"(G), "s"(GT)); asm volatile("global_load_dwordx2 a[132:133], %0, %1 sc1\n\tglobal_load_dwordx2 a[134:135], %0, %2 sc1" :: "v"(off8[1]), "s"(G), "s"(GT)); asm volatile("global_load_dwordx2 a[136:137], %0, %1 sc1\n\tglobal_load_dwordx2 a[138:139], %0, %2 sc1" :: "v"(off8[2]), "s"(G), "s"(GT)); asm volatile("global_load_dwordx2 a[140:141], %0, %1 sc1\n\tglobal_load_dwordx2 a[142:143], %0, %2 sc1" :: "v"(off8[3]), "s"(G), "s"(GT)); asm volatile("global_load_dwordx2 a[144:145], %0, %1 sc1\n\tglobal_load_dwordx2 a[146:147], %0, %2 sc1" :: "v"(off8[4]), "s"(G), "s"(GT)); asm volatile("global_load_dwordx2 a[148:149], %0, %1 sc1\n\tglobal_load_dwordx2 a[150:151], %0, %2 sc1" :: "v"(off8[5]), "s"(G), "s"(GT)); asm volatile("global_load_dwordx2 a[152:153], %0, %1 sc1\n\tglobal_load_dwordx2 a[154:155], %0, %2 sc1" :: "v"(off8[6]), "s"(G), "s"(GT)); asm volatile("global_load_dwordx2 a[156:157], %0, %1 sc1\n\tglobal_load_dwordx2 a[158:159], %0, %2 sc1" :: "v"(off8[7]), "s"(G), "s"(GT));
#define DQ_W6_LOADSET_1_PLAIN asm volatile("global_load_dwordx2 a[160:161], %0, %1\n\tglobal_load_dwordx2 a[162:163], %0, %2" :: "v"(off8[0]), "s"(G), "s"(GT)); asm volatile("global_load_dwordx2 a[164:165], %0, %1\n\tglobal_load_dwordx2 a[166:167], %0, %2" :: "v"(off8[1]), "s"(G), "s"(GT)); asm volatile("global_load_dwordx2 a[168:169], %0, %1\n\tglobal_load_dwordx2 a[170:171], %0, %2" :: "v"(off8[2]), "s"(G), "s"(GT)); asm volatile("global_load_dwordx2 a[172:173], %0, %1\n\tglobal_load_dwordx2 a[174:175], %0, %2" :: "v"(off8[3]), "s"(G), "s"(GT)); asm volatile("global_load_dwordx2 a[176:177], %0, %1\n\tglobal_load_dwordx2 a[178:179], %0, %2" :: "v"(off8[4]), "s"(G), "s"(GT)); asm volatile("global_load_dwordx2 a[180:181], %0, %1\n\tglobal_load_dwordx2 a[182:183], %0, %2" :: "v"(off8[5]), "s"(G), "s"(GT)); asm volatile("global_load_dwordx2 a[184:185], %0, %1\n\tglobal_load_dwordx2 a[186:187], %0, %2" :: "v"(off8[6]), "s"(G), "s"(GT)); asm volatile("global_load_dwordx2 a[188:189], %0, %1\n\tglobal_load_dwordx2 a[190:191], %0, %2" :: "v"(off8[7]), "s"(G), "s"(GT));
#define DQ_W6_LOADSET_1_COH asm volatile("global_load_dwordx2 a[160:161], %0, %1 sc1\n\tglobal_load_dwordx2 a[162:163], %0, %2 sc1" :: "v"(off8[0]), "s"(G), "s"(GT)); asm volatile("global_load_dwordx2 a[164:165], %0, %1 sc1\n\tglobal_load_dwordx2 a[166:167], %0, %2 sc1" :: "v"(off8[1]), "s"(G), "s"(GT)); asm volatile("global_load_dwordx2 a[168:169], %0, %1 sc1\n\tglobal_load_dwordx2 a[170:171], %0, %2 sc1" :: "v"(off8[2]), "s"(G), "s"(GT)); asm volatile("global_load_dwordx2 a[172:173], %0, %1 sc1\n\tglobal_load_dwordx2 a[174:175], %0, %2 sc1" :: "v"(off8[3]), "s"(G), "s"(GT)); asm volatile("global_load_dwordx2 a[176:177], %0, %1 sc1\n\tglobal_load_dwordx2 a[178:179], %0, %2 sc1" :: "v"(off8[4]), "s"(G), "s"(GT)); asm volatile("global_load_dwordx2 a[180:181], %0, %1 sc1\n\tglobal_load_dwordx2 a[182:183], %0, %2 sc1" :: "v"(off8[5]), "s"(G), "s"(GT)); asm volatile("global_load_dwordx2 a[184:185], %0, %1 sc1\n\tglobal_load_dwordx2 a[186:187], %0, %2 sc1" :: "v"(off8[6]), "s"(G), "s"(GT)); asm volatile("global_load_dwordx2 a[188:189], %0, %1 sc1\n\tglobal_load_dwordx2 a[190:191], %0, %2 sc1" :: "v"(off8[7]), "s"(G), "s"(GT));
#define DQ_W6_LOADSET_2_PLAIN asm volatile("global_load_dwordx2 a[192:193], %0, %1\n\tglobal_load_dwordx2 a[194:195], %0, %2" :: "v"(off8[0]), "s"(G), "s"(GT)); asm volatile("global_load_dwordx2 a[196:197], %0, %1\n\tglobal_load_dwordx2 a[198:199], %0, %2" :: "v"(off8[1]), "s"(G), "s"(GT)); asm volatile("global_load_dwordx2 a[200:201], %0, %1\n\tglobal_load_dwordx2 a[202:203], %0, %2" :: "v"(off8[2]), "s"(G), "s"(GT)); asm volatile("global_load_dwordx2 a[204:205], %0, %1\n\tglobal_load_dwordx2 a[206:207], %0, %2" :: "v"(off8[3]), "s"(G), "s"(GT)); asm volatile("global_load_dwordx2 a[208:209], %0, %1\n\tglobal_load_dwordx2 a[210:211], %0, %2" :: "v"(off8[4]), "s"(G), "s"(GT)); asm volatile("global_load_dwordx2 a[212:213], %0, %1\n\tglobal_load_dwordx2 a[214:215], %0, %2" :: "v"(off8[5]), "s"(G), "s"(GT)); asm volatile("global_load_dwordx2 a[216:217], %0, %1\n\tglobal_load_dwordx2 a[218:219], %0, %2" :: "v"(off8[6]), "s"(G), "s"(GT)); asm volatile("global_load_dwordx2 a[220:221], %0, %1\n\tglobal_load_dwordx2 a[222:223], %0, %2" :: "v"(off8[7]), "s"(G), "s"(GT));
#define DQ_W6_LOADSET_2_COH asm volatile("global_load_dwordx2 a[192:193], %0, %1 sc1\n\tglobal_load_dwordx2 a[194:195], %0, %2 sc1" :: "v"(off8[0]), "s"(G), "s"(GT)); asm volatile("global_load_dwordx2 a[196:197], %0, %1 sc1\n\tglobal_load_dwordx2 a[198:199], %0, %2 sc1" :: "v"(off8[1]), "s"(G), "s"(GT)); asm volatile("global_load_dwordx2 a[200:201], %0, %1 sc1\n\tglobal_load_dwordx2 a[202:203], %0, %2 sc1" :: "v"(off8[2]), "s"(G), "s"(GT)); asm volatile("global_load_dwordx2 a[204:205], %0, %1 sc1\n\tglobal_load_dwordx2 a[206:207], %0, %2 sc1" :: "v"(off8[3]), "s"(G), "s"(GT)); asm volatile("global_load_dwordx2 a[208:209], %0, %1 sc1\n\tglobal_load_dwordx2 a[210:211], %0, %2 sc1" :: "v"(off8[4]), "s"(G), "s"(GT)); asm volatile("global_load_dwordx2 a[212:213], %0, %1 sc1\n\tglobal_load_dwordx2 a[214:215], %0, %2 sc1" :: "v"(off8[5]), "s"(G), "s"(GT)); asm volatile("global_load_dwordx2 a[216:217], %0, %1 sc1\n\tglobal_load_dwordx2 a[218:219], %0, %2 sc1" :: "v"(off8[6]), "s"(G), "s"(GT)); asm volatile("global_load_dwordx2 a[220:221], %0, %1 sc1\n\tglobal_load_dwordx2 a[222:223], %0, %2 sc1" :: "v"(off8[7]), "s"(G), "s"(GT));
#define DQ_W6_PICK(SEL) do { const unsigned poff_ = (unsigned)__builtin_amdgcn_readfirstlane((int)(12u + (unsigned)(SEL) * 40u)); asm volatile("s_getpc_b64 s[96:97]\n\ts_add_u32 s96, s96, %4\n\ts_addc_u32 s97, s97, 0\n\ts_setpc_b64 s[96:97]\n\t" "v_accvgpr_read_b32 %0, a128\n\tv_accvgpr_read_b32 %1, a129\n\tv_accvgpr_read_b32 %2, a130\n\tv_accvgpr_read_b32 %3, a131\n\ts_branch 1f\n\ts_nop 0\n\t" "v_accvgpr_read_b32 %0, a132\n\tv_accvgpr_read_b32 %1, a133\n\tv_accvgpr_read_b32 %2, a134\n\tv_accvgpr_read_b32 %3, a135\n\ts_branch 1f\n\ts_nop 0\n\t" "v_accvgpr_read_b32 %0, a136\n\tv_accvgpr_read_b32 %1, a137\n\tv_accvgpr_read_b32 %2, a138\n\tv_accvgpr_read_b32 %3, a139\n\ts_branch 1f\n\ts_nop 0\n\t" "v_accvgpr_read_b32 %0, a140\n\tv_accvgpr_read_b32 %1, a141\n\tv_accvgpr_read_b32 %2, a142\n\tv_accvgpr_read_b32 %3, a143\n\ts_branch 1f\n\ts_nop 0\n\t" "v_accvgpr_read_b32 %0, a144\n\tv_accvgpr_read_b32 %1, a145\n\tv_accvgpr_read_b32 %2, a146\n\tv_accvgpr_read_b32 %3, a147\n\ts_branch 1f\n\ts_nop 0\n\t" "v_accvgpr_read_b32 %0, a148\n\tv_accvgpr_read_b32 %1, a149\n\tv_accvgpr_read_b32 %2, a150\n\tv_accvgpr_read_b32 %3, a151\n\ts_branch 1f\n\ts_nop 0\n\t" "v_accvgpr_read_b32 %0, a152\n\tv_accvgpr_read_b32 %1, a153\n\tv_accvgpr_read_b32 %2, a154\n\tv_accvgpr_read_b32 %3, a155\n\ts_branch 1f\n\ts_nop 0\n\t" "v_accvgpr_read_b32 %0, a156\n\tv_accvgpr_read_b32 %1, a157\n\tv_accvgpr_read_b32 %2, a158\n\tv_accvgpr_read_b32 %3, a159\n\ts_branch 1f\n\ts_nop 0\n\t" "v_accvgpr_read_b32 %0, a160\n\tv_accvgpr_read_b32 %1, a161\n\tv_accvgpr_read_b32 %2, a162\n\tv_accvgpr_read_b32 %3, a163\n\ts_branch 1f\n\ts_nop 0\n\t" "v_accvgpr_read_b32 %0, a164\n\tv_accvgpr_read_b32 %1, a165\n\tv_accvgpr_read_b32 %2, a166\n\tv_accvgpr_read_b32 %3, a167\n\ts_branch 1f\n\ts_nop 0\n\t" "v_accvgpr_read_b32 %0, a168\n\tv_accvgpr_read_b32 %1, a169\n\tv_accvgpr_read_b32 %2, a170\n\tv_accvgpr_read_b32 %3, a171\n\ts_branch 1f\n\ts_nop 0\n\t" "v_accvgpr_read_b32 %0, a172\n\tv_accvgpr_read_b32 %1, a173\n\tv_accvgpr_read_b32 %2, a174\n\tv_accvgpr_read_b32 %3, a175\n\ts_branch 1f\n\ts_nop 0\n\t" "v_accvgpr_read_b32 %0, a176\n\tv_accvgpr_read_b32 %1, a177\n\tv_accvgpr_read_b32 %2, a178\n\tv_accvgpr_read_b32 %3, a179\n\ts_branch 1f\n\ts_nop 0\n\t" "v_accvgpr_read_b32 %0, a180\n\tv_accvgpr_read_b32 %1, a181\n\tv_accvgpr_read_b32 %2, a182\n\tv_accvgpr_read_b32 %3, a183\n\ts_branch 1f\n\ts_nop 0\n\t" "v_accvgpr_read_b32 %0, a184\n\tv_accvgpr_read_b32 %1, a185\n\tv_accvgpr_read_b32 %2, a186\n\tv_accvgpr_read_b32 %3, a187\n\ts_branch 1f\n\ts_nop 0\n\t" "v_accvgpr_read_b32 %0, a188\n\tv_accvgpr_read_b32 %1, a189\n\tv_accvgpr_read_b32 %2, a190\n\tv_accvgpr_read_b32 %3, a191\n\ts_branch 1f\n\ts_nop 0\n\t" "v_accvgpr_read_b32 %0, a192\n\tv_accvgpr_read_b32 %1, a193\n\tv_accvgpr_read_b32 %2, a194\n\tv_accvgpr_read_b32 %3, a195\n\ts_branch 1f\n\ts_nop 0\n\t" "v_accvgpr_read_b32 %0, a196\n\tv_accvgpr_read_b32 %1, a197\n\tv_accvgpr_read_b32 %2, a198\n\tv_accvgpr_read_b32 %3, a199\n\ts_branch 1f\n\ts_nop 0\n\t" "v_accvgpr_read_b32 %0, a200\n\tv_accvgpr_read_b32 %1, a201\n\tv_accvgpr_read_b32 %2, a202\n\tv_accvgpr_read_b32 %3, a203\n\ts_branch 1f\n\ts_nop 0\n\t" "v_accvgpr_read_b32 %0, a204\n\tv_accvgpr_read_b32 %1, a205\n\tv_accvgpr_read_b32 %2, a206\n\tv_accvgpr_read_b32 %3, a207\n\ts_branch 1f\n\ts_nop 0\n\t" "v_accvgpr_read_b32 %0, a208\n\tv_accvgpr_read_b32 %1, a209\n\tv_accvgpr_read_b32 %2, a210\n\tv_accvgpr_read_b32 %3, a211\n\ts_branch 1f\n\ts_nop 0\n\t" "v_accvgpr_read_b32 %0, a212\n\tv_accvgpr_read_b32 %1, a213\n\tv_accvgpr_read_b32 %2, a214\n\tv_accvgpr_read_b32 %3, a215\n\ts_branch 1f\n\ts_nop 0\n\t" "v_accvgpr_read_b32 %0, a216\n\tv_accvgpr_read_b32 %1, a217\n\tv_accvgpr_read_b32 %2, a218\n\tv_accvgpr_read_b32 %3, a219\n\ts_branch 1f\n\ts_nop 0\n\t" "v_accvgpr_read_b32 %0, a220\n\tv_accvgpr_read_b32 %1, a221\n\tv_accvgpr_read_b32 %2, a222\n\tv_accvgpr_read_b32 %3, a223\n\ts_branch 1f\n\ts_nop 0\n\t" "1:" : "=v"(ulo), "=v"(uhi), "=v"(wlo), "=v"(whi) : "s"(poff_) : "s96", "s97", "scc"); } while (0)
#define DQ_W6_PAIRS do { const unsigned off_ = (unsigned)__builtin_amdgcn_readfirstlane((int)(12u + (unsigned)(32 - k) * 16u)); asm("s_getpc_b64 s[96:97]\n\t" "s_add_u32 s96, s96, %[off]\n\t" "s_addc_u32 s97, s97, 0\n\t" "s_setpc_b64 s[96:97]\n\t" "v_fmac_f64_dpp %[u1], %[pby], v[190:191] row_newbcast:15 row_mask:0xf bank_mask:0xf\n\t" "v_fmac_f64_dpp %[w1], %[pbx], v[254:255] row_newbcast:15 row_mask:0xf bank_mask:0xf\n\t" "v_fmac_f64_dpp %[uj], %[pby], v[188:189] row_newbcast:14 row_mask:0xf bank_mask:0xf\n\t" "v_fmac_f64_dpp %[wj], %[pbx], v[252:253] row_newbcast:14 row_mask:0xf bank_mask:0xf\n\t" "v_fmac_f64_dpp %[u1], %[pby], v[186:187] row_newbcast:13 row_mask:0xf bank_mask:0xf\n\t" "v_fmac_f64_dpp %[w1], %[pbx], v[250:251] row_newbcast:13 row_mask:0xf bank_mask:0xf\n\t" "v_fmac_f64_dpp %[uj], %[pby], v[184:185] row_newbcast:12 row_mask:0xf bank_mask:0xf\n\t" "v_fmac_f64_dpp %[wj], %[pbx], v[248:249] row_newbcast:12 row_mask:0xf bank_mask:0xf\n\t" "v_fmac_f64_dpp %[u1], %[pby], v[182:183] row_newbcast:11 row_mask:0xf bank_mask:0xf\n\t" "v_fmac_f64_dpp %[w1], %[pbx], v[246:247] row_newbcast:11 row_mask:0xf bank_mask:0xf\n\t" "v_fmac_f64_dpp %[uj], %[pby], v[180:181] row_newbcast:10 row_mask:0xf bank_mask:0xf\n\t" "v_fmac_f64_dpp %[wj], %[pbx], v[244:245] row_newbcast:10 row_mask:0xf bank_mask:0xf\n\t" "v_fmac_f64_dpp %[u1], %[pby], v[178:179] row_newbcast:9 row_mask:0xf bank_mask:0xf\n\t" "v_fmac_f64_dpp %[w1], %[pbx], v[242:243] row_newbcast:9 row_mask:0xf bank_mask:0xf\n\t" "v_fmac_f64_dpp %[uj], %[pby], v[176:177] row_newbcast:8 row_mask:0xf bank_mask:0xf\n\t" "v_fmac_f64_dpp %[wj], %[pbx], v[240:241] row_newbcast:8 row_mask:0xf bank_mask:0xf\n\t" "v_fmac_f64_dpp %[u1], %[pby], v[174:175] row_newbcast:7 row_mask:0xf bank_mask:0xf\n\t" "v_fmac_f64_dpp %[w1], %[pbx], v[238:239] row_newbcast:7 row_mask:0xf bank_mask:0xf\n\t" "v_fmac_f64_dpp %[uj], %[pby], v[172:173] row_newbcast:6 row_mask:0xf bank_mask:0xf\n\t" "v_fmac_f64_dpp %[wj], %[pbx], v[236:237] row_newbcast:6 row_mask:0xf bank_mask:0xf\n\t" "v_fmac_f64_dpp %[u1], %[pby], v[170:171] row_newbcast:5 row_mask:0xf bank_mask:0xf\n\t" "v_fmac_f64_dpp %[w1], %[pbx], v[234:235] row_newbcast:5 row_mask:0xf bank_mask:0xf\n\t" "v_fmac_f64_dpp %[uj], %[pby], v[168:169] row_newbcast:4 row_mask:0xf bank_mask:0xf\n\t" "v_fmac_f64_dpp %[wj], %[pbx], v[232:233] row_newbcast:4 row_mask:0xf bank_mask:0xf\n\t" "v_fmac_f64_dpp %[u1], %[pby], v[166:167] row_newbcast:3 row_mask:0xf bank_mask:0xf\n\t" "v_fmac_f64_dpp %[w1], %[pbx], v[230:231] row_newbcast:3 row_mask:0xf bank_mask:0xf\n\t" "v_fmac_f64_dpp %[uj], %[pby], v[164:165] row_newbcast:2 row_mask:0xf bank_mask:0xf\n\t" "v_fmac_f64_dpp %[wj], %[pbx], v[228:229] row_newbcast:2 row_mask:0xf bank_mask:0xf\n\t" "v_fmac_f64_dpp %[u1], %[pby], v[162:163] row_newbcast:1 row_mask:0xf bank_mask:0xf\n\t" "v_fmac_f64_dpp %[w1], %[pbx], v[226:227] row_newbcast:1 row_mask:0xf bank_mask:0xf\n\t" "v_fmac_f64_dpp %[uj], %[pby], v[160:161] row_newbcast:0 row_mask:0xf bank_mask:0xf\n\t" "v_fmac_f64_dpp %[wj], %[pbx], v[224:225] row_newbcast:0 row_mask:0xf bank_mask:0xf\n\t" "v_fmac_f64_dpp %[u1], %[pay], v[158:159] row_newbcast:15 row_mask:0xf bank_mask:0xf\n\t" "v_fmac_f64_dpp %[w1], %[pax], v[222:223] row_newbcast:15 row_mask:0xf bank_mask:0xf\n\t" "v_fmac_f64_dpp %[uj], %[pay], v[156:157] row_newbcast:14 row_mask:0xf bank_mask:0xf\n\t" "v_fmac_f64_dpp %[wj], %[pax], v[220:221] row_newbcast:14 row_mask:0xf bank_mask:0xf\n\t" "v_fmac_f64_dpp %[u1], %[pay], v[154:155] row_newbcast:13 row_mask:0xf bank_mask:0xf\n\t" "v_fmac_f64_dpp %[w1], %[pax], v[218:219] row_newbcast:13 row_mask:0xf bank_mask:0xf\n\t" "v_fmac_f64_dpp %[uj], %[pay], v[152:153] row_newbcast:12 row_mask:0xf bank_mask:0xf\n\t" "v_fmac_f64_dpp %[wj], %[pax], v[216:217] row_newbcast:12 row_mask:0xf bank_mask:0xf\n\t" "v_fmac_f64_dpp %[u1], %[pay], v[150:151] row_newbcast:11 row_mask:0xf bank_mask:0xf\n\t" "v_fmac_f64_dpp %[w1], %[pax], v[214:215] row_newbcast:11 row_mask:0xf bank_mask:0xf\n\t" "v_fmac_f64_dpp %[uj], %[pay], v[148:149] row_newbcast:10 row_mask:0xf bank_mask:0xf\n\t" "v_fmac_f64_dpp %[wj], %[pax], v[212:213] row_newbcast:10 row_mask:0xf bank_mask:0xf\n\t" "v_fmac_f64_dpp %[u1], %[pay], v[146:147] row_newbcast:9 row_mask:0xf bank_mask:0xf\n\t" "v_fmac_f64_dpp %[w1], %[pax], v[210:211] row_newbcast:9 row_mask:0xf bank_mask:0xf\n\t" "v_fmac_f64_dpp %[uj], %[pay], v[144:145] row_newbcast:8 row_mask:0xf bank_mask:0xf\n\t" "v_fmac_f64_dpp %[wj], %[pax], v[208:209] row_newbcast:8 row_mask:0xf bank_mask:0xf\n\t" "v_fmac_f64_dpp %[u1], %[pay], v[142:143] row_newbcast:7 row_mask:0xf bank_mask:0xf\n\t" "v_fmac_f64_dpp %[w1], %[pax], v[206:207] row_newbcast:7 row_mask:0xf bank_mask:0xf\n\t" "v_fmac_f64_dpp %[uj], %[pay], v[140:141] row_newbcast:6 row_mask:0xf bank_mask:0xf\n\t" "v_fmac_f64_dpp %[wj], %[pax], v[204:205] row_newbcast:6 row_mask:0xf bank_mask:0xf\n\t" "v_fmac_f64_dpp %[u1], %[pay], v[138:139] row_newbcast:5 row_mask:0xf bank_mask:0xf\n\t" "v_fmac_f64_dpp %[w1], %[pax], v[202:203] row_newbcast:5 row_mask:0xf bank_mask:0xf\n\t" "v_fmac_f64_dpp %[uj], %[pay], v[136:137] row_newbcast:4 row_mask:0xf bank_mask:0xf\n\t" "v_fmac_f64_dpp %[wj], %[pax], v[200:201] row_newbcast:4 row_mask:0xf bank_mask:0xf\n\t" "v_fmac_f64_dpp %[u1], %[pay], v[134:135] row_newbcast:3 row_mask:0xf bank_mask:0xf\n\t" "v_fmac_f64_dpp %[w1], %[pax], v[198:199] row_newbcast:3 row_mask:0xf bank_mask:0xf\n\t" "v_fmac_f64_dpp %[uj], %[pay], v[132:133] row_newbcast:2 row_mask:0xf bank_mask:0xf\n\t" "v_fmac_f64_dpp %[wj], %[pax], v[196:197] row_newbcast:2 row_mask:0xf bank_mask:0xf\n\t" "v_fmac_f64_dpp %[u1], %[pay], v[130:131] row_newbcast:1 row_mask:0xf bank_mask:0xf\n\t" "v_fmac_f64_dpp %[w1], %[pax], v[194:195] row_newbcast:1 row_mask:0xf bank_mask:0xf\n\t" "v_fmac_f64_dpp %[uj], %[pay], v[128:129] row_newbcast:0 row_mask:0xf bank_mask:0xf\n\t" "v_fmac_f64_dpp %[wj], %[pax], v[192:193] row_newbcast:0 row_mask:0xf bank_mask:0xf" : [uj] "+v"(uj), [wj] "+v"(wj), [u1] "+v"(u1), [w1] "+v"(w1) : [pax] "v"(pa.x), [pay] "v"(pa.y), [pbx] "v"(pb.x), [pby] "v"(pb.y), [off] "s"(off_) : "s96", "s97", "scc"); } while (0)
#define DQ_W6_SETPAIR(PU, WJ) asm volatile("s_set_gpr_idx_on %4, gpr_idx(DST)\n\tv_mov_b32 v128, %0\n\tv_mov_b32 v129, %1\n\tv_mov_b32 v192, %2\n\tv_mov_b32 v193, %3\n\ts_set_gpr_idx_off" :: "v"(__double2loint(PU)), "v"(__double2hiint(PU)), "v"(__double2loint(WJ)), "v"(__double2hiint(WJ)), "s"(__builtin_amdgcn_readfirstlane(2 * k)) : "m0")
#define DQ_W6_DUMP do { const unsigned long long rowpair_bytes = 16ull * (unsigned)n; unsigned long long ua_ = (unsigned long long)Up + 16ull * (unsigned)j, wa_ = (unsigned long long)Wp + 16ull * (unsigned)j; \
    if (0 >= k) break; if (COH) asm volatile("global_store_dwordx4 %0, v[128:131], off sc1\n\tglobal_store_dwordx4 %1, v[192:195], off sc1" : "+v"(ua_), "+v"(wa_) :: "memory"); else asm volatile("global_store_dwordx4 %0, v[128:131], off\n\tglobal_store_dwordx4 %1, v[192:195], off" : "+v"(ua_), "+v"(wa_) :: "memory"); ua_ += rowpair_bytes; wa_ += rowpair_bytes; \
    if (2 >= k) break; if (COH) asm volatile("global_store_dwordx4 %0, v[132:135], off sc1\n\tglobal_store_dwordx4 %1, v[196:199], off sc1" : "+v"(ua_), "+v"(wa_) :: "memory"); else asm volatile("global_store_dwordx4 %0, v[132:135], off\n\tglobal_store_dwordx4 %1, v[196:199], off" : "+v"(ua_), "+v"(wa_) :: "memory"); ua_ += rowpair_bytes; wa_ += rowpair_bytes; \
    if (4 >= k) break; if (COH) asm volatile("global_store_dwordx4 %0, v[136:139], off sc1\n\tglobal_store_dwordx4 %1, v[200:203], off sc1" : "+v"(ua_), "+v"(wa_) :: "memory"); else asm volatile("global_store_dwordx4 %0, v[136:139], off\n\tglobal_store_dwordx4 %1, v[200:203], off" : "+v"(ua_), "+v"(wa_) :: "memory"); ua_ += rowpair_bytes; wa_ += rowpair_bytes; \
    if (6 >= k) break; if (COH) asm volatile("global_store_dwordx4 %0, v[140:143], off sc1\n\tglobal_store_dwordx4 %1, v[204:207], off sc1" : "+v"(ua_), "+v"(wa_) :: "memory"); else asm volatile("global_store_dwordx4 %0, v[140:143], off\n\tglobal_store_dwordx4 %1, v[204:207], off" : "+v"(ua_), "+v"(wa_) :: "memory"); ua_ += rowpair_bytes; wa_ += rowpair_bytes; \
    if (8 >= k) break; if (COH) asm volatile("global_store_dwordx4 %0, v[144:147], off sc1\n\tglobal_store_dwordx4 %1, v[208:211], off sc1" : "+v"(ua_), "+v"(wa_) :: "memory"); else asm volatile("global_store_dwordx4 %0, v[144:147], off\n\tglobal_store_dwordx4 %1, v[208:211], off" : "+v"(ua_), "+v"(wa_) :: "memory"); ua_ += rowpair_bytes; wa_ += rowpair_bytes; \
    if (10 >= k) break; if (COH) asm volatile("global_store_dwordx4 %0, v[148:151], off sc1\n\tglobal_store_dwordx4 %1, v[212:215], off sc1" : "+v"(ua_), "+v"(wa_) :: "memory"); else asm volatile("global_store_dwordx4 %0, v[148:151], off\n\tglobal_store_dwordx4 %1, v[212:215], off" : "+v"(ua_), "+v"(wa_) :: "memory"); ua_ += rowpair_bytes; wa_ += rowpair_bytes; \
    if (12 >= k) break; if (COH) asm volatile("global_store_dwordx4 %0, v[152:155], off sc1\n\tglobal_store_dwordx4 %1, v[216:219], off sc1" : "+v"(ua_), "+v"(wa_) :: "memory"); else asm volatile("global_store_dwordx4 %0, v[152:155], off\n\tglobal_store_dwordx4 %1, v[216:219], off" : "+v"(ua_), "+v"(wa_) :: "memory"); ua_ += rowpair_bytes; wa_ += rowpair_bytes; \
    if (14 >= k) break; if (COH) asm volatile("global_store_dwordx4 %0, v[156:159], off sc1\n\tglobal_store_dwordx4 %1, v[220:223], off sc1" : "+v"(ua_), "+v"(wa_) :: "memory"); else asm volatile("global_store_dwordx4 %0, v[156:159], off\n\tglobal_store_dwordx4 %1, v[220:223], off" : "+v"(ua_), "+v"(wa_) :: "memory"); ua_ += rowpair_bytes; wa_ += rowpair_bytes; \
    if (16 >= k) break; if (COH) asm volatile("global_store_dwordx4 %0, v[160:163], off sc1\n\tglobal_store_dwordx4 %1, v[224:227], off sc1" : "+v"(ua_), "+v"(wa_) :: "memory"); else asm volatile("global_store_dwordx4 %0, v[160:163], off\n\tglobal_store_dwordx4 %1, v[224:227], off" : "+v"(ua_), "+v"(wa_) :: "memory"); ua_ += rowpair_bytes; wa_ += rowpair_bytes; \
    if (18 >= k) break; if (COH) asm volatile("global_store_dwordx4 %0, v[164:167], off sc1\n\tglobal_store_dwordx4 %1, v[228:231], off sc1" : "+v"(ua_), "+v"(wa_) :: "memory"); else asm volatile("global_store_dwordx4 %0, v[164:167], off\n\tglobal_store_dwordx4 %1, v[228:231], off" : "+v"(ua_), "+v"(wa_) :: "memory"); ua_ += rowpair_bytes; wa_ += rowpair_bytes; \
    if (20 >= k) break; if (COH) asm volatile("global_store_dwordx4 %0, v[168:171], off sc1\n\tglobal_store_dwordx4 %1, v[232:235], off sc1" : "+v"(ua_), "+v"(wa_) :: "memory"); else asm volatile("global_store_dwordx4 %0, v[168:171], off\n\tglobal_store_dwordx4 %1, v[232:235], off" : "+v"(ua_), "+v"(wa_) :: "memory"); ua_ += rowpair_bytes; wa_ += rowpair_bytes; \
    if (22 >= k) break; if (COH) asm volatile("global_store_dwordx4 %0, v[172:175], off sc1\n\tglobal_store_dwordx4 %1, v[236:239], off sc1" : "+v"(ua_), "+v"(wa_) :: "memory"); else asm volatile("global_store_dwordx4 %0, v[172:175], off\n\tglobal_store_dwordx4 %1, v[236:239], off" : "+v"(ua_), "+v"(wa_) :: "memory"); ua_ += rowpair_bytes; wa_ += rowpair_bytes; \
    if (24 >= k) break; if (COH) asm volatile("global_store_dwordx4 %0, v[176:179], off sc1\n\tglobal_store_dwordx4 %1, v[240:243], off sc1" : "+v"(ua_), "+v"(wa_) :: "memory"); else asm volatile("global_store_dwordx4 %0, v[176:179], off\n\tglobal_store_dwordx4 %1, v[240:243], off" : "+v"(ua_), "+v"(wa_) :: "memory"); ua_ += rowpair_bytes; wa_ += rowpair_bytes; \
    if (26 >= k) break; if (COH) asm volatile("global_store_dwordx4 %0, v[180:183], off sc1\n\tglobal_store_dwordx4 %1, v[244:247], off sc1" : "+v"(ua_), "+v"(wa_) :: "memory"); else asm volatile("global_store_dwordx4 %0, v[180:183], off\n\tglobal_store_dwordx4 %1, v[244:247], off" : "+v"(ua_), "+v"(wa_) :: "memory"); ua_ += rowpair_bytes; wa_ += rowpair_bytes; \
    if (28 >= k) break; if (COH) asm volatile("global_store_dwordx4 %0, v[184:187], off sc1\n\tglobal_store_dwordx4 %1, v[248:251], off sc1" : "+v"(ua_), "+v"(wa_) :: "memory"); else asm volatile("global_store_dwordx4 %0, v[184:187], off\n\tglobal_store_dwordx4 %1, v[248:251], off" : "+v"(ua_), "+v"(wa_) :: "memory"); ua_ += rowpair_bytes; wa_ += rowpair_bytes; \
    if (30 >= k) break; if (COH) asm volatile("global_store_dwordx4 %0, v[188:191], off sc1\n\tglobal_store_dwordx4 %1, v[252:255], off sc1" : "+v"(ua_), "+v"(wa_) :: "memory"); else asm volatile("global_store_dwordx4 %0, v[188:191], off\n\tglobal_store_dwordx4 %1, v[252:255], off" : "+v"(ua_), "+v"(wa_) :: "memory"); ua_ += rowpair_bytes; wa_ += rowpair_bytes; \
} while (0)
#define DQ_W6_DUMP_PUB do { const unsigned long long rowpair_bytes = 16ull * (unsigned)n; unsigned long long ua_ = (unsigned long long)Up + 16ull * (unsigned)j, wa_ = (unsigned long long)Wp + 16ull * (unsigned)j; \
    if (0 >= DQ_W6_KPUB) break; asm volatile("global_store_dwordx4 %0, v[128:131], off sc1\n\tglobal_store_dwordx4 %1, v[192:195], off sc1" : "+v"(ua_), "+v"(wa_) :: "memory"); ua_ += rowpair_bytes; wa_ += rowpair_bytes; \
    if (2 >= DQ_W6_KPUB) break; asm volatile("global_store_dwordx4 %0, v[132:135], off sc1\n\tglobal_store_dwordx4 %1, v[196:199], off sc1" : "+v"(ua_), "+v"(wa_) :: "memory"); ua_ += rowpair_bytes; wa_ += rowpair_bytes; \
    if (4 >= DQ_W6_KPUB) break; asm volatile("global_store_dwordx4 %0, v[136:139], off sc1\n\tglobal_store_dwordx4 %1, v[200:203], off sc1" : "+v"(ua_), "+v"(wa_) :: "memory"); ua_ += rowpair_bytes; wa_ += rowpair_bytes; \
    if (6 >= DQ_W6_KPUB) break; asm volatile("global_store_dwordx4 %0, v[140:143], off sc1\n\tglobal_store_dwordx4 %1, v[204:207], off sc1" : "+v"(ua_), "+v"(wa_) :: "memory"); ua_ += rowpair_bytes; wa_ += rowpair_bytes; \
    if (8 >= DQ_W6_KPUB) break; asm volatile("global_store_dwordx4 %0, v[144:147], off sc1\n\tglobal_store_dwordx4 %1, v[208:211], off sc1" : "+v"(ua_), "+v"(wa_) :: "memory"); ua_ += rowpair_bytes; wa_ += rowpair_bytes; \
    if (10 >= DQ_W6_KPUB) break; asm volatile("global_store_dwordx4 %0, v[148:151], off sc1\n\tglobal_store_dwordx4 %1, v[212:215], off sc1" : "+v"(ua_), "+v"(wa_) :: "memory"); ua_ += rowpair_bytes; wa_ += rowpair_bytes; \
    if (12 >= DQ_W6_KPUB) break; asm volatile("global_store_dwordx4 %0, v[152:155], off sc1\n\tglobal_store_dwordx4 %1, v[216:219], off sc1" : "+v"(ua_), "+v"(wa_) :: "memory"); ua_ += rowpair_bytes; wa_ += rowpair_bytes; \
    if (14 >= DQ_W6_KPUB) break; asm volatile("global_store_dwordx4 %0, v[156:159], off sc1\n\tglobal_store_dwordx4 %1, v[220:223], off sc1" : "+v"(ua_), "+v"(wa_) :: "memory"); ua_ += rowpair_bytes; wa_ += rowpair_bytes; \
    if (16 >= DQ_W6_KPUB) break; asm volatile("global_store_dwordx4 %0, v[160:163], off sc1\n\tglobal_store_dwordx4 %1, v[224:227], off sc1" : "+v"(ua_), "+v"(wa_) :: "memory"); ua_ += rowpair_bytes; wa_ += rowpair_bytes; \
    if (18 >= DQ_W6_KPUB) break; asm volatile("global_store_dwordx4 %0, v[164:167], off sc1\n\tglobal_store_dwordx4 %1, v[228:231], off sc1" : "+v"(ua_), "+v"(wa_) :: "memory"); ua_ += rowpair_bytes; wa_ += rowpair_bytes; \
    if (20 >= DQ_W6_KPUB) break; asm volatile("global_store_dwordx4 %0, v[168:171], off sc1\n\tglobal_store_dwordx4 %1, v[232:235], off sc1" : "+v"(ua_), "+v"(wa_) :: "memory"); ua_ += rowpair_bytes; wa_ += rowpair_bytes; \
    if (22 >= DQ_W6_KPUB) break; asm volatile("global_store_dwordx4 %0, v[172:175], off sc1\n\tglobal_store_dwordx4 %1, v[236:239], off sc1" : "+v"(ua_), "+v"(wa_) :: "memory"); ua_ += rowpair_bytes; wa_ += rowpair_bytes; \
    if (24 >= DQ_W6_KPUB) break; asm volatile("global_store_dwordx4 %0, v[176:179], off sc1\n\tglobal_store_dwordx4 %1, v[240:243], off sc1" : "+v"(ua_), "+v"(wa_) :: "memory"); ua_ += rowpair_bytes; wa_ += rowpair_bytes; \
    if (26 >= DQ_W6_KPUB) break; asm volatile("global_store_dwordx4 %0, v[180:183], off sc1\n\tglobal_store_dwordx4 %1, v[244:247], off sc1" : "+v"(ua_), "+v"(wa_) :: "memory"); ua_ += rowpair_bytes; wa_ += rowpair_bytes; \
    if (28 >= DQ_W6_KPUB) break; asm volatile("global_store_dwordx4 %0, v[184:187], off sc1\n\tglobal_store_dwordx4 %1, v[248:251], off sc1" : "+v"(ua_), "+v"(wa_) :: "memory"); ua_ += rowpair_bytes; wa_ += rowpair_bytes; \
    if (30 >= DQ_W6_KPUB) break; asm volatile("global_store_dwordx4 %0, v[188:191], off sc1\n\tglobal_store_dwordx4 %1, v[252:255], off sc1" : "+v"(ua_), "+v"(wa_) :: "memory"); ua_ += rowpair_bytes; wa_ += rowpair_bytes; \
} while (0)
#define DQ_W6_REBASE_16 asm volatile("v_mov_b64 v[128:129], v[160:161]\n\tv_mov_b64 v[192:193], v[224:225]\n\t" "v_mov_b64 v[130:131], v[162:163]\n\tv_mov_b64 v[194:195], v[226:227]\n\t" "v_mov_b64 v[132:133], v[164:165]\n\tv_mov_b64 v[196:197], v[228:229]\n\t" "v_mov_b64 v[134:135], v[166:167]\n\tv_mov_b64 v[198:199], v[230:231]\n\t" "v_mov_b64 v[136:137], v[168:169]\n\tv_mov_b64 v[200:201], v[232:233]\n\t" "v_mov_b64 v[138:139], v[170:171]\n\tv_mov_b64 v[202:203], v[234:235]\n\t" "v_mov_b64 v[140:141], v[172:173]\n\tv_mov_b64 v[204:205], v[236:237]\n\t" "v_mov_b64 v[142:143], v[174:175]\n\tv_mov_b64 v[206:207], v[238:239]\n\t" "v_mov_b64 v[144:145], v[176:177]\n\tv_mov_b64 v[208:209], v[240:241]\n\t" "v_mov_b64 v[146:147], v[178:179]\n\tv_mov_b64 v[210:211], v[242:243]\n\t" "v_mov_b64 v[148:149], v[180:181]\n\tv_mov_b64 v[212:213], v[244:245]\n\t" "v_mov_b64 v[150:151], v[182:183]\n\tv_mov_b64 v[214:215], v[246:247]\n\t" "v_mov_b64 v[152:153], v[184:185]\n\tv_mov_b64 v[216:217], v[248:249]\n\t" "v_mov_b64 v[154:155], v[186:187]\n\tv_mov_b64 v[218:219], v[250:251]\n\t" "v_mov_b64 v[156:157], v[188:189]\n\tv_mov_b64 v[220:221], v[252:253]\n\t" "v_mov_b64 v[158:159], v[190:191]\n\tv_mov_b64 v[222:223], v[254:255]")
#define DQ_W6_REBASE_20 asm volatile("v_mov_b64 v[128:129], v[168:169]\n\tv_mov_b64 v[192:193], v[232:233]\n\t" "v_mov_b64 v[130:131], v[170:171]\n\tv_mov_b64 v[194:195], v[234:235]\n\t" "v_mov_b64 v[132:133], v[172:173]\n\tv_mov_b64 v[196:197], v[236:237]\n\t" "v_mov_b64 v[134:135], v[174:175]\n\tv_mov_b64 v[198:199], v[238:239]\n\t" "v_mov_b64 v[136:137], v[176:177]\n\tv_mov_b64 v[200:201], v[240:241]\n\t" "v_mov_b64 v[138:139], v[178:179]\n\tv_mov_b64 v[202:203], v[242:243]\n\t" "v_mov_b64 v[140:141], v[180:181]\n\tv_mov_b64 v[204:205], v[244:245]\n\t" "v_mov_b64 v[142:143], v[182:183]\n\tv_mov_b64 v[206:207], v[246:247]\n\t" "v_mov_b64 v[144:145], v[184:185]\n\tv_mov_b64 v[208:209], v[248:249]\n\t" "v_mov_b64 v[146:147], v[186:187]\n\tv_mov_b64 v[210:211], v[250:251]\n\t" "v_mov_b64 v[148:149], v[188:189]\n\tv_mov_b64 v[212:213], v[252:253]\n\t" "v_mov_b64 v[150:151], v[190:191]\n\tv_mov_b64 v[214:215], v[254:255]")
#define DQ_W6_REBASE_22 asm volatile("v_mov_b64 v[128:129], v[172:173]\n\tv_mov_b64 v[192:193], v[236:237]\n\t" "v_mov_b64 v[130:131], v[174:175]\n\tv_mov_b64 v[194:195], v[238:239]\n\t" "v_mov_b64 v[132:133], v[176:177]\n\tv_mov_b64 v[196:197], v[240:241]\n\t" "v_mov_b64 v[134:135], v[178:179]\n\tv_mov_b64 v[198:199], v[242:243]\n\t" "v_mov_b64 v[136:137], v[180:181]\n\tv_mov_b64 v[200:201], v[244:245]\n\t" "v_mov_b64 v[138:139], v[182:183]\n\tv_mov_b64 v[202:203], v[246:247]\n\t" "v_mov_b64 v[140:141], v[184:185]\n\tv_mov_b64 v[204:205], v[248:249]\n\t" "v_mov_b64 v[142:143], v[186:187]\n\tv_mov_b64 v[206:207], v[250:251]\n\t" "v_mov_b64 v[144:145], v[188:189]\n\tv_mov_b64 v[208:209], v[252:253]\n\t" "v_mov_b64 v[146:147], v[190:191]\n\tv_mov_b64 v[210:211], v[254:255]")
#define DQ_W6_REBASE_24 asm volatile("v_mov_b64 v[128:129], v[176:177]\n\tv_mov_b64 v[192:193], v[240:241]\n\t" "v_mov_b64 v[130:131], v[178:179]\n\tv_mov_b64 v[194:195], v[242:243]\n\t" "v_mov_b64 v[132:133], v[180:181]\n\tv_mov_b64 v[196:197], v[244:245]\n\t" "v_mov_b64 v[134:135], v[182:183]\n\tv_mov_b64 v[198:199], v[246:247]\n\t" "v_mov_b64 v[136:137], v[184:185]\n\tv_mov_b64 v[200:201], v[248:249]\n\t" "v_mov_b64 v[138:139], v[186:187]\n\tv_mov_b64 v[202:203], v[250:251]\n\t" "v_mov_b64 v[140:141], v[188:189]\n\tv_mov_b64 v[204:205], v[252:253]\n\t" "v_mov_b64 v[142:143], v[190:191]\n\tv_mov_b64 v[206:207], v[254:255]")
#define DQ_W6_REBASE_26 asm volatile("v_mov_b64 v[128:129], v[180:181]\n\tv_mov_b64 v[192:193], v[244:245]\n\t" "v_mov_b64 v[130:131], v[182:183]\n\tv_mov_b64 v[194:195], v[246:247]\n\t" "v_mov_b64 v[132:133], v[184:185]\n\tv_mov_b64 v[196:197], v[248:249]\n\t" "v_mov_b64 v[134:135], v[186:187]\n\tv_mov_b64 v[198:199], v[250:251]\n\t" "v_mov_b64 v[136:137], v[188:189]\n\tv_mov_b64 v[200:201], v[252:253]\n\t" "v_mov_b64 v[138:139], v[190:191]\n\tv_mov_b64 v[202:203], v[254:255]")
#define DQ_W6_REBASE_28 asm volatile("v_mov_b64 v[128:129], v[184:185]\n\tv_mov_b64 v[192:193], v[248:249]\n\t" "v_mov_b64 v[130:131], v[186:187]\n\tv_mov_b64 v[194:195], v[250:251]\n\t" "v_mov_b64 v[132:133], v[188:189]\n\tv_mov_b64 v[196:197], v[252:253]\n\t" "v_mov_b64 v[134:135], v[190:191]\n\tv_mov_b64 v[198:199], v[254:255]")
```

Baseline: 12.78 sweeps/s.

## Deepen group prefetch to four slots and add optional early arrival polling

New measurement: 12.00 sweeps/s. 6.1% lower.

```diff
diff --git a/dqmc_amd/csrc/common.h b/dqmc_amd/csrc/common.h
--- a/dqmc_amd/csrc/common.h
+++ b/dqmc_amd/csrc/common.h
@@ -138,6 +138,7 @@
     int slice_absent_tile = -1;
     int slice_absent_l = -1;
     int slice_late_tile = -1, slice_late_us = 0;
+    int slice_no_early = 0;
     int* info = nullptr;
     int* acc_out; long acc_stride;
     int n, nt;
@@ -145,7 +146,7 @@
 constexpr int UPDATE_KD = 32;
 
 struct SliceSync {
-    unsigned long long seq; unsigned int error; unsigned int solo_count; unsigned int pad[12];
+    unsigned long long seq; unsigned int error; unsigned int solo_count; unsigned int win_early, win_block; unsigned int pad[10];
     unsigned int arrive[496];
 };
 constexpr size_t SLICE_SYNC_BYTES = 2048;
diff --git a/dqmc_amd/csrc/engine.hip b/dqmc_amd/csrc/engine.hip
--- a/dqmc_amd/csrc/engine.hip
+++ b/dqmc_amd/csrc/engine.hip
@@ -301,6 +301,7 @@
     unsigned slice_epoch = 0;
     int slice_absent_l = -1;
     int slice_late_tile = -1, slice_late_us = 0;
+    int slice_no_early = 1;
     int slice_absent_tile = -1;
     DevPtr<int> acc;
     struct Exchange { DevPtr<int8_t> saved, recv; DevPtr<int> tab; } xch;
@@ -336,6 +337,8 @@
         reserved = slice_reserve(device, n, C);
         slice_path = pick_slice_path(n, C, reserved);
         if (const char* a = getenv("DQMC_DEBUG_SLICE_ABSENT")) { slice_absent_tile = atoi(a); if (const char* c = strchr(a, ':')) slice_absent_l = atoi(c + 1); }
+        if (const char* a = getenv("DQMC_SLICE_EARLY_POLL")) slice_no_early = atoi(a) == 0;
+        if (const char* a = getenv("DQMC_DEBUG_SLICE_NOPOLL")) { if (atoi(a) != 0) slice_no_early = 1; }
         if (const char* a = getenv("DQMC_DEBUG_SLICE_LATE")) { slice_late_tile = atoi(a); if (const char* c = strchr(a, ':')) slice_late_us = atoi(c + 1); }
         DQ_TRY(dev_alloc(expK, C * nn)); DQ_TRY(dev_alloc(invexpK, C * nn));
         DQ_TRY(dev_alloc(fields, (size_t)C * nt * n)); DQ_TRY(dev_alloc(expv, (size_t)C * nt * n)); DQ_TRY(dev_alloc(invexpv, (size_t)C * nt * n));
@@ -518,7 +521,7 @@
     UpdateDesc udesc() const {
         UpdateDesc d; d.G = mG(); d.fields = fields.get(); d.f_stride = (long)nt * n; d.expv = expv.get(); d.invexpv = invexpv.get(); d.v_stride = (long)nt * n;
         d.tabs = tabs.get(); d.perm = rs_perm.get(); d.kprop = rs_k.get(); d.u = rs_u.get(); d.rs_stride = (long)nt * n; d.Upanel = Upanel.get(); d.Wpanel = Wpanel.get(); d.Cpanel = Cpanel.get();
-        d.panel_stride = (long)UPDATE_KD * n; d.state = state.get(); d.state_stride = 4; d.prep = prep.get(); d.prep_stride = 4L * n; d.slice_sync = is_persistent(slice_path) ? slice_sync.get() : nullptr; d.slice_epoch = slice_epoch; d.slice_absent_tile = slice_absent_tile; d.slice_absent_l = slice_absent_l; d.slice_late_tile = slice_late_tile; d.slice_late_us = slice_late_us; d.GT = Mat{GT.get(), nn}; d.gt_valid = gt_valid ? 1 : 0; d.info = ctx.info(); d.acc_out = acc.get(); d.acc_stride = nt; d.n = n; d.nt = nt;
+        d.panel_stride = (long)UPDATE_KD * n; d.state = state.get(); d.state_stride = 4; d.prep = prep.get(); d.prep_stride = 4L * n; d.slice_sync = is_persistent(slice_path) ? slice_sync.get() : nullptr; d.slice_epoch = slice_epoch; d.slice_absent_tile = slice_absent_tile; d.slice_absent_l = slice_absent_l; d.slice_late_tile = slice_late_tile; d.slice_late_us = slice_late_us; d.slice_no_early = slice_no_early; d.GT = Mat{GT.get(), nn}; d.gt_valid = gt_valid ? 1 : 0; d.info = ctx.info(); d.acc_out = acc.get(); d.acc_stride = nt; d.n = n; d.nt = nt;
         return d;
     }
     int local_update(int l) {
diff --git a/dqmc_amd/csrc/update.hip b/dqmc_amd/csrc/update.hip
--- a/dqmc_amd/csrc/update.hip
+++ b/dqmc_amd/csrc/update.hip
@@ -50,7 +50,7 @@
 
 #ifdef DQ_SCAN_STAMPS
 #define STAMP(v) { unsigned long long _t; asm volatile("s_memtime %0\n\ts_waitcnt lgkmcnt(0)" : "=s"(_t) :: "memory"); v = _t; }
-struct ScanProf { unsigned long long t_rej = 0, t_kloop = 0, t_tail = 0, t_wait = 0, t_first = 0, t_dump = 0, t_noacc = 0, t_pub = 0, t_fin = 0, t_finwait = 0; int n_rej = 0, n_acc = 0, n_noacc = 0, n_pub = 0, n_fin_k = 0, n_fin_g = 0, n_fin_e = 0; };
+struct ScanProf { unsigned long long t_rej = 0, t_kloop = 0, t_tail = 0, t_wait = 0, t_first = 0, t_dump = 0, t_noacc = 0, t_pub = 0, t_fin = 0, t_finwait = 0; int n_rej = 0, n_acc = 0, n_noacc = 0, n_pub = 0, n_fin_k = 0, n_fin_g = 0, n_fin_e = 0, n_seen = 0, seen_flips = 0, seen_groups = 0; };
 #define PROF_ARG , ScanProf& prof
 #else
 #define PROF_ARG
@@ -144,6 +144,9 @@
 #define DQ_W6_KPUB 24
 #define DQ_W6_XOVER 8
 #endif
+#ifndef DQ_W6_POLL_FROM
+#define DQ_W6_POLL_FROM 4
+#endif
 #define DQ_W6_CAT2(a, b) a##b
 #define DQ_W6_CAT(a, b) DQ_W6_CAT2(a, b)
 #define DQ_W6_REBASE DQ_W6_CAT(DQ_W6_REBASE_, DQ_W6_KPUB)
@@ -165,7 +168,8 @@
         : "v"(igs), "v"(jj8));
     if (gs == 0) { if (COH) { DQ_W6_LOADSET_0_COH } else { DQ_W6_LOADSET_0_PLAIN } }
     else if (gs == 1) { if (COH) { DQ_W6_LOADSET_1_COH } else { DQ_W6_LOADSET_1_PLAIN } }
-    else { if (COH) { DQ_W6_LOADSET_2_COH } else { DQ_W6_LOADSET_2_PLAIN } }
+    else if (gs == 2) { if (COH) { DQ_W6_LOADSET_2_COH } else { DQ_W6_LOADSET_2_PLAIN } }
+    else { if (COH) { DQ_W6_LOADSET_3_COH } else { DQ_W6_LOADSET_3_PLAIN } }
 }
 
 constexpr unsigned SLICE_SPIN_LIMIT = 1u << 22;
@@ -214,6 +218,12 @@
     bool solo = false;
     bool inflight = false;
     int g_limit = 0;
+    bool poll = true;
+    bool polling = false;
+    bool seen = false;
+    int g_early = 0;
+    int since = 0;
+    int n_early = 0, n_block = 0;
 };
 
 __device__ __forceinline__ bool as_inflight(const SliceAsync& a) { return a.inflight; }
@@ -230,15 +240,20 @@
 #else
 #define DQ_ST(...)
 #endif
-    auto async_finish = [&]() {
+    const int wave = __builtin_amdgcn_readfirstlane((int)(threadIdx.x >> 6));
+    unsigned arr = 0; bool polled = false, w0_seen = false;
+    auto load_g = [&](int gg) { walk6_load_group<COH>(G, GT, sh, gg, gg & 3, n, j, live); };
+    auto async_finish = [&](int g_from, int g_to, bool keep_early) {
         if constexpr (AS::enabled) {
             DQ_ST(unsigned long long tf0, tf1, tf2; STAMP(tf0))
-            slice_wait_arrivals(as.sy, as.epoch, as.win, as.F, as.info);
+            if (as.seen) ++as.n_early;
+            else { slice_wait_arrivals(as.sy, as.epoch, as.win, as.F, as.info); ++as.n_block; }
             DQ_ST(STAMP(tf1))
+            for (int gg = g_from; gg <= g_to; ++gg) if (!keep_early || gg > as.g_early) load_g(gg);
             DQ_W6_REBASE;
             if (live) for (int t = 0; t < k - DQ_W6_KPUB; ++t) sh.UW[t * n + j] = sh.UW[(DQ_W6_KPUB + t) * n + j];
             if (j < k - DQ_W6_KPUB) sh.acc_site[j] = sh.acc_site[DQ_W6_KPUB + j];
-            k -= DQ_W6_KPUB; ++as.win; as.inflight = false;
+            k -= DQ_W6_KPUB; ++as.win; as.inflight = false; as.seen = false; as.polling = false; polled = false; w0_seen = false;
             lds_barrier();
             DQ_ST(STAMP(tf2) prof.t_finwait += tf1 - tf0; prof.t_fin += tf2 - tf1;)
         }
@@ -247,21 +262,23 @@
     bool done = false;
     asm volatile("s_waitcnt vmcnt(0)" ::: "memory");
     __builtin_amdgcn_s_waitcnt(0x0F70);
-    walk6_load_group<COH>(G, GT, sh, g, g % 3, n, j, live);
-    walk6_load_group<COH>(G, GT, sh, g + 1, (g + 1) % 3, n, j, live);
+    auto early_request = [&]() {
+        if constexpr (AS::enabled) { while (as.g_early < g + 3) { ++as.g_early; load_g(as.g_early); } }
+    };
+    load_g(g); load_g(g + 1); load_g(g + 2);
     while (!done) {
         DQ_ST(unsigned long long tg0, tg1; STAMP(tg0))
-        const int gs = g % 3;
+        const int gs = g & 3;
         if constexpr (AS::enabled) {
-            if (as.inflight && g > as.g_limit) {
-                DQ_ST(prof.n_fin_g++;)
-                async_finish();
-                walk6_load_group<COH>(G, GT, sh, g, gs, n, j, live);
-                walk6_load_group<COH>(G, GT, sh, g + 1, (g + 1) % 3, n, j, live);
+            if (as.inflight) {
+                if (g > as.g_limit) {
+                    DQ_ST(prof.n_fin_g++;)
+                    async_finish(g, g + 2, true);
+                } else if (as.seen) early_request();
             }
-            if (!as.inflight) walk6_load_group<COH>(G, GT, sh, g + 2, (g + 2) % 3, n, j, live);
+            if (!as.inflight) load_g(g + 3);
         } else
-        walk6_load_group<COH>(G, GT, sh, g + 2, (g + 2) % 3, n, j, live);
+        load_g(g + 3);
         DQ_ST(STAMP(tg1) prof.t_first += tg1 - tg0;)
         const int gbase = g * 8;
         const int p_l = gbase + q8, pc_l = min(p_l, n - 1);
@@ -270,10 +287,19 @@
         for (;;) {
             DQ_ST(unsigned long long t0, t1, t2, t3; STAMP(t0))
             const double* dcur = par ? sh.diag2 : sh.diag;
+            int verdict = 0;
+            if constexpr (AS::enabled) { if (as.polling) verdict = as.flag[1 + (par ^ 1)]; }
             const double r_l = 1.0 + (1.0 - dcur[i_l]) * dl_l;
             const double R_l = rb_l * (r_l * r_l);
             const bool acc_l = p_l >= pos && p_l < n && ur_l < fmin(1.0, fabs(R_l));
             const unsigned bal = (unsigned)__ballot(acc_l) & 0xffu;
+            if constexpr (AS::enabled) {
+                if (as.polling && __builtin_amdgcn_readfirstlane(verdict)) {
+                    as.seen = true; as.polling = false;
+                    DQ_ST(prof.n_seen++; prof.seen_flips += as.since; prof.seen_groups += g - (as.g_limit - 3);)
+                    early_request();
+                }
+            }
             if (bal == 0u) { pos = min(gbase + 8, n); DQ_ST(STAMP(t1) prof.t_noacc += t1 - t0; prof.n_noacc++;) break; }
             const int first = __ffs((int)bal) - 1;
             const int p = gbase + first;
@@ -284,7 +310,7 @@
             const double2 pa = sh.UW[min(r16, kc) * n + i], pb = sh.UW[min(16 + r16, kc) * n + i];
             const double pref = dl_p / r_p;
             int ulo, uhi, wlo, whi;
-            asm volatile("s_waitcnt vmcnt(32)" ::: "memory");
+            asm volatile("s_waitcnt vmcnt(48)" ::: "memory");
             DQ_W6_PICK(gs * 8 + first);
             double uj = __hiloint2double(uhi, ulo), wj = __hiloint2double(whi, wlo);
             DQ_ST(STAMP(t1))
@@ -300,6 +326,12 @@
                 DQ_W6_SETPAIR(pu, wj);
             }
             DQ_ST(STAMP(t2))
+            if constexpr (AS::enabled) {
+                if (as.polling && wave == 0) {
+                    if (polled) { polled = false; if (__all(arr == slice_tag(as.epoch, as.win))) w0_seen = true; }
+                    if (w0_seen && lane == 0) as.flag[1 + par] = 1;
+                }
+            }
             ++k; par ^= 1;
             lds_barrier();
             DQ_ST(STAMP(t3) prof.t_wait += t1 - t0; prof.t_kloop += t2 - t1; prof.t_tail += t3 - t2; prof.n_acc++;)
@@ -314,6 +346,7 @@
                         d.expv[(long)chain * d.v_stride + slice_off + ii] = sh.tl[24 + new_f];
                         d.invexpv[(long)chain * d.v_stride + slice_off + ii] = sh.tl[28 + new_f];
                     }
+                    if (threadIdx.x == 0) { as.flag[1] = 0; as.flag[2] = 0; }
                     unsigned census = slice_tag(as.epoch, 0);
                     if (as.win == 1 && threadIdx.x < (unsigned)as.F) census = __hip_atomic_load(&as.sy->arrive[threadIdx.x], __ATOMIC_RELAXED, __HIP_MEMORY_SCOPE_AGENT);
                     asm volatile("s_waitcnt vmcnt(0)" ::: "memory");
@@ -328,23 +361,25 @@
                         asm volatile("s_waitcnt vmcnt(0)" ::: "memory");
                         __syncthreads();
                         as.published += k; k = 0; ++as.win;
-                        walk6_load_group<COH>(G, GT, sh, g, gs, n, j, live);
-                        walk6_load_group<COH>(G, GT, sh, g + 1, (g + 1) % 3, n, j, live);
-                        walk6_load_group<COH>(G, GT, sh, g + 2, (g + 2) % 3, n, j, live);
+                        for (int gg = g; gg <= g + 3; ++gg) load_g(gg);
                     } else {
                         if (threadIdx.x == 0)
                             __hip_atomic_store(&as.sy->seq, ((unsigned long long)slice_tag(as.epoch, as.win) << 32) | (unsigned)DQ_W6_KPUB, __ATOMIC_RELAXED, __HIP_MEMORY_SCOPE_AGENT);
-                        as.published += DQ_W6_KPUB; as.inflight = true; as.g_limit = g + 2;
+                        as.published += DQ_W6_KPUB; as.inflight = true; as.g_limit = g + 3;
+                        as.g_early = as.g_limit; as.seen = false; as.polling = as.poll; as.since = -1; polled = false; w0_seen = false;
                     }
                     DQ_ST(STAMP(tp1) prof.t_pub += tp1 - tp0; prof.n_pub++;)
                 }
                 if (k >= kd || (as.inflight && k >= DQ_W6_KPUB + DQ_W6_XOVER)) {
                     if (!as.inflight) { done = true; break; }
                     DQ_ST(prof.n_fin_k++;)
-                    async_finish();
-                    walk6_load_group<COH>(G, GT, sh, g, gs, n, j, live);
-                    walk6_load_group<COH>(G, GT, sh, g + 1, (g + 1) % 3, n, j, live);
-                    walk6_load_group<COH>(G, GT, sh, g + 2, (g + 2) % 3, n, j, live);
+                    async_finish(g, g + 3, false);
+                }
+                if (as.polling) {
+                    if (++as.since >= DQ_W6_POLL_FROM && wave == 0 && !w0_seen) {
+                        arr = lane < as.F ? __hip_atomic_load(&as.sy->arrive[lane], __ATOMIC_RELAXED, __HIP_MEMORY_SCOPE_AGENT) : slice_tag(as.epoch, as.win);
+                        polled = true;
+                    }
                 }
             } else
             if (k >= kd) { done = true; break; }
@@ -352,7 +387,7 @@
         if (pos >= n) done = true;
         ++g;
     }
-    if constexpr (AS::enabled) { if (as.inflight) { DQ_ST(prof.n_fin_e++;) async_finish(); } }
+    if constexpr (AS::enabled) { if (as.inflight) { DQ_ST(prof.n_fin_e++;) async_finish(1, 0, false); } }
 #undef DQ_ST
 #ifdef DQ_SCAN_STAMPS
     unsigned long long td0; STAMP(td0)
@@ -647,7 +682,7 @@
 #ifdef DQ_SCAN_STAMPS
         ScanProf prof; unsigned long long tk0, t_hand = 0; STAMP(tk0)
 #endif
-        SliceAsync as{sy, epoch, F, info, flag};
+        SliceAsync as{sy, epoch, F, info, flag}; as.poll = d.slice_no_early == 0;
         for (;; ++as.win) {
             const int k = walk_window6<true, true, SliceAsync>(sh, pos, dg, n, kd, j, live, G, GT, d, slice_off, chain, fields_g, Up, Wp, as PROF_PASS);
             total_acc += k + as.published; as.published = 0;
@@ -684,13 +719,17 @@
             { unsigned long long th1; STAMP(th1) t_hand += th1 - th0; }
 #endif
         }
-        if (j == 0) d.acc_out[(long)chain * d.acc_stride + acc_slot] = total_acc;
+        if (j == 0) {
+            d.acc_out[(long)chain * d.acc_stride + acc_slot] = total_acc;
+            if (as.n_early) __hip_atomic_fetch_add(&sy->win_early, (unsigned)as.n_early, __ATOMIC_RELAXED, __HIP_MEMORY_SCOPE_AGENT);
+            if (as.n_block) __hip_atomic_fetch_add(&sy->win_block, (unsigned)as.n_block, __ATOMIC_RELAXED, __HIP_MEMORY_SCOPE_AGENT);
+        }
 #ifdef DQ_SCAN_STAMPS
         if (j == 0) { unsigned long long tk1; STAMP(tk1)
 #if 1
-            printf("slice l=%d: total %llu cyc | hand-offs %llu | %d acc: decide+fetch %llu pairs %llu tail %llu | window start->first flip %llu | %d empty passes %llu | dump+drain %llu | %d async publishes %llu, finishes (full %d / columns %d / end %d): wait %llu rebase %llu\n",
+            printf("slice l=%d: total %llu cyc | hand-offs %llu | %d acc: decide+fetch %llu pairs %llu tail %llu | window start->first flip %llu | %d empty passes %llu | dump+drain %llu | %d async publishes %llu, finishes (full %d / columns %d / end %d): wait %llu rebase %llu | windows early %d blocking %d | arrivals seen in %d windows, after %d flips / %d groups in all\n",
                    l, tk1 - tk0, t_hand, prof.n_acc, prof.t_wait, prof.t_kloop, prof.t_tail, prof.t_first, prof.n_noacc, prof.t_noacc, prof.t_dump,
-                   prof.n_pub, prof.t_pub, prof.n_fin_k, prof.n_fin_g, prof.n_fin_e, prof.t_finwait, prof.t_fin);
+                   prof.n_pub, prof.t_pub, prof.n_fin_k, prof.n_fin_g, prof.n_fin_e, prof.t_finwait, prof.t_fin, as.n_early, as.n_block, prof.n_seen, prof.seen_flips, prof.seen_groups);
 #endif
         }
 #endif
diff --git a/dqmc_amd/csrc/walk_bodies.inc b/dqmc_amd/csrc/walk_bodies.inc
--- a/dqmc_amd/csrc/walk_bodies.inc
+++ b/dqmc_amd/csrc/walk_bodies.inc
@@ -1,11 +1,13 @@
-#define DQ_W6_RESERVE asm volatile("" ::: "v128", "v129", "v130", "v131", "v132", "v133", "v134", "v135", "v136", "v137", "v138", "v139", "v140", "v141", "v142", "v143", "v144", "v145", "v146", "v147", "v148", "v149", "v150", "v151", "v152", "v153", "v154", "v155", "v156", "v157", "v158", "v159", "v160", "v161", "v162", "v163", "v164", "v165", "v166", "v167", "v168", "v169", "v170", "v171", "v172", "v173", "v174", "v175", "v176", "v177", "v178", "v179", "v180", "v181", "v182", "v183", "v184", "v185", "v186", "v187", "v188", "v189", "v190", "v191", "v192", "v193", "v194", "v195", "v196", "v197", "v198", "v199", "v200", "v201", "v202", "v203", "v204", "v205", "v206", "v207", "v208", "v209", "v210", "v211", "v212", "v213", "v214", "v215", "v216", "v217", "v218", "v219", "v220", "v221", "v222", "v223", "v224", "v225", "v226", "v227", "v228", "v229", "v230", "v231", "v232", "v233", "v234", "v235", "v236", "v237", "v238", "v239", "v240", "v241", "v242", "v243", "v244", "v245", "v246", "v247", "v248", "v249", "v250", "v251", "v252", "v253", "v254", "v255", "a128", "a129", "a130", "a131", "a132", "a133", "a134", "a135", "a136", "a137", "a138", "a139", "a140", "a141", "a142", "a143", "a144", "a145", "a146", "a147", "a148", "a149", "a150", "a151", "a152", "a153", "a154", "a155", "a156", "a157", "a158", "a159", "a160", "a161", "a162", "a163", "a164", "a165", "a166", "a167", "a168", "a169", "a170", "a171", "a172", "a173", "a174", "a175", "a176", "a177", "a178", "a179", "a180", "a181", "a182", "a183", "a184", "a185", "a186", "a187", "a188", "a189", "a190", "a191", "a192", "a193", "a194", "a195", "a196", "a197", "a198", "a199", "a200", "a201", "a202", "a203", "a204", "a205", "a206", "a207", "a208", "a209", "a210", "a211", "a212", "a213", "a214", "a215", "a216", "a217", "a218", "a219", "a220", "a221", "a222", "a223")
+#define DQ_W6_RESERVE asm volatile("" ::: "v128", "v129", "v130", "v131", "v132", "v133", "v134", "v135", "v136", "v137", "v138", "v139", "v140", "v141", "v142", "v143", "v144", "v145", "v146", "v147", "v148", "v149", "v150", "v151", "v152", "v153", "v154", "v155", "v156", "v157", "v158", "v159", "v160", "v161", "v162", "v163", "v164", "v165", "v166", "v167", "v168", "v169", "v170", "v171", "v172", "v173", "v174", "v175", "v176", "v177", "v178", "v179", "v180", "v181", "v182", "v183", "v184", "v185", "v186", "v187", "v188", "v189", "v190", "v191", "v192", "v193", "v194", "v195", "v196", "v197", "v198", "v199", "v200", "v201", "v202", "v203", "v204", "v205", "v206", "v207", "v208", "v209", "v210", "v211", "v212", "v213", "v214", "v215", "v216", "v217", "v218", "v219", "v220", "v221", "v222", "v223", "v224", "v225", "v226", "v227", "v228", "v229", "v230", "v231", "v232", "v233", "v234", "v235", "v236", "v237", "v238", "v239", "v240", "v241", "v242", "v243", "v244", "v245", "v246", "v247", "v248", "v249", "v250", "v251", "v252", "v253", "v254", "v255", "a128", "a129", "a130", "a131", "a132", "a133", "a134", "a135", "a136", "a137", "a138", "a139", "a140", "a141", "a142", "a143", "a144", "a145", "a146", "a147", "a148", "a149", "a150", "a151", "a152", "a153", "a154", "a155", "a156", "a157", "a158", "a159", "a160", "a161", "a162", "a163", "a164", "a165", "a166", "a167", "a168", "a169", "a170", "a171", "a172", "a173", "a174", "a175", "a176", "a177", "a178", "a179", "a180", "a181", "a182", "a183", "a184", "a185", "a186", "a187", "a188", "a189", "a190", "a191", "a192", "a193", "a194", "a195", "a196", "a197", "a198", "a199", "a200", "a201", "a202", "a203", "a204", "a205", "a206", "a207", "a208", "a209", "a210", "a211", "a212", "a213", "a214", "a215", "a216", "a217", "a218", "a219", "a220", "a221", "a222", "a223", "a224", "a225", "a226", "a227", "a228", "a229", "a230", "a231", "a232", "a233", "a234", "a235", "a236", "a237", "a238", "a239", "a240", "a241", "a242", "a243", "a244", "a245", "a246", "a247", "a248", "a249", "a250", "a251", "a252", "a253", "a254", "a255")
 #define DQ_W6_LOADSET_0_PLAIN asm volatile("global_load_dwordx2 a[128:129], %0, %1\n\tglobal_load_dwordx2 a[130:131], %0, %2" :: "v"(off8[0]), "s"(G), "s"(GT)); asm volatile("global_load_dwordx2 a[132:133], %0, %1\n\tglobal_load_dwordx2 a[134:135], %0, %2" :: "v"(off8[1]), "s"(G), "s"(GT)); asm volatile("global_load_dwordx2 a[136:137], %0, %1\n\tglobal_load_dwordx2 a[138:139], %0, %2" :: "v"(off8[2]), "s"(G), "s"(GT)); asm volatile("global_load_dwordx2 a[140:141], %0, %1\n\tglobal_load_dwordx2 a[142:143], %0, %2" :: "v"(off8[3]), "s"(G), "s"(GT)); asm volatile("global_load_dwordx2 a[144:145], %0, %1\n\tglobal_load_dwordx2 a[146:147], %0, %2" :: "v"(off8[4]), "s"(G), "s"(GT)); asm volatile("global_load_dwordx2 a[148:149], %0, %1\n\tglobal_load_dwordx2 a[150:151], %0, %2" :: "v"(off8[5]), "s"(G), "s"(GT)); asm volatile("global_load_dwordx2 a[152:153], %0, %1\n\tglobal_load_dwordx2 a[154:155], %0, %2" :: "v"(off8[6]), "s"(G), "s"(GT)); asm volatile("global_load_dwordx2 a[156:157], %0, %1\n\tglobal_load_dwordx2 a[158:159], %0, %2" :: "v"(off8[7]), "s"(G), "s"(GT));
 #define DQ_W6_LOADSET_0_COH asm volatile("global_load_dwordx2 a[128:129], %0, %1 sc1\n\tglobal_load_dwordx2 a[130:131], %0, %2 sc1" :: "v"(off8[0]), "s"(G), "s"(GT)); asm volatile("global_load_dwordx2 a[132:133], %0, %1 sc1\n\tglobal_load_dwordx2 a[134:135], %0, %2 sc1" :: "v"(off8[1]), "s"(G), "s"(GT)); asm volatile("global_load_dwordx2 a[136:137], %0, %1 sc1\n\tglobal_load_dwordx2 a[138:139], %0, %2 sc1" :: "v"(off8[2]), "s"(G), "s"(GT)); asm volatile("global_load_dwordx2 a[140:141], %0, %1 sc1\n\tglobal_load_dwordx2 a[142:143], %0, %2 sc1" :: "v"(off8[3]), "s"(G), "s"(GT)); asm volatile("global_load_dwordx2 a[144:145], %0, %1 sc1\n\tglobal_load_dwordx2 a[146:147], %0, %2 sc1" :: "v"(off8[4]), "s"(G), "s"(GT)); asm volatile("global_load_dwordx2 a[148:149], %0, %1 sc1\n\tglobal_load_dwordx2 a[150:151], %0, %2 sc1" :: "v"(off8[5]), "s"(G), "s"(GT)); asm volatile("global_load_dwordx2 a[152:153], %0, %1 sc1\n\tglobal_load_dwordx2 a[154:155], %0, %2 sc1" :: "v"(off8[6]), "s"(G), "s"(GT)); asm volatile("global_load_dwordx2 a[156:157], %0, %1 sc1\n\tglobal_load_dwordx2 a[158:159], %0, %2 sc1" :: "v"(off8[7]), "s"(G), "s"(GT));
 #define DQ_W6_LOADSET_1_PLAIN asm volatile("global_load_dwordx2 a[160:161], %0, %1\n\tglobal_load_dwordx2 a[162:163], %0, %2" :: "v"(off8[0]), "s"(G), "s"(GT)); asm volatile("global_load_dwordx2 a[164:165], %0, %1\n\tglobal_load_dwordx2 a[166:167], %0, %2" :: "v"(off8[1]), "s"(G), "s"(GT)); asm volatile("global_load_dwordx2 a[168:169], %0, %1\n\tglobal_load_dwordx2 a[170:171], %0, %2" :: "v"(off8[2]), "s"(G), "s"(GT)); asm volatile("global_load_dwordx2 a[172:173], %0, %1\n\tglobal_load_dwordx2 a[174:175], %0, %2" :: "v"(off8[3]), "s"(G), "s"(GT)); asm volatile("global_load_dwordx2 a[176:177], %0, %1\n\tglobal_load_dwordx2 a[178:179], %0, %2" :: "v"(off8[4]), "s"(G), "s"(GT)); asm volatile("global_load_dwordx2 a[180:181], %0, %1\n\tglobal_load_dwordx2 a[182:183], %0, %2" :: "v"(off8[5]), "s"(G), "s"(GT)); asm volatile("global_load_dwordx2 a[184:185], %0, %1\n\tglobal_load_dwordx2 a[186:187], %0, %2" :: "v"(off8[6]), "s"(G), "s"(GT)); asm volatile("global_load_dwordx2 a[188:189], %0, %1\n\tglobal_load_dwordx2 a[190:191], %0, %2" :: "v"(off8[7]), "s"(G), "s"(GT));
 #define DQ_W6_LOADSET_1_COH asm volatile("global_load_dwordx2 a[160:161], %0, %1 sc1\n\tglobal_load_dwordx2 a[162:163], %0, %2 sc1" :: "v"(off8[0]), "s"(G), "s"(GT)); asm volatile("global_load_dwordx2 a[164:165], %0, %1 sc1\n\tglobal_load_dwordx2 a[166:167], %0, %2 sc1" :: "v"(off8[1]), "s"(G), "s"(GT)); asm volatile("global_load_dwordx2 a[168:169], %0, %1 sc1\n\tglobal_load_dwordx2 a[170:171], %0, %2 sc1" :: "v"(off8[2]), "s"(G), "s"(GT)); asm volatile("global_load_dwordx2 a[172:173], %0, %1 sc1\n\tglobal_load_dwordx2 a[174:175], %0, %2 sc1" :: "v"(off8[3]), "s"(G), "s"(GT)); asm volatile("global_load_dwordx2 a[176:177], %0, %1 sc1\n\tglobal_load_dwordx2 a[178:179], %0, %2 sc1" :: "v"(off8[4]), "s"(G), "s"(GT)); asm volatile("global_load_dwordx2 a[180:181], %0, %1 sc1\n\tglobal_load_dwordx2 a[182:183], %0, %2 sc1" :: "v"(off8[5]), "s"(G), "s"(GT)); asm volatile("global_load_dwordx2 a[184:185], %0, %1 sc1\n\tglobal_load_dwordx2 a[186:187], %0, %2 sc1" :: "v"(off8[6]), "s"(G), "s"(GT)); asm volatile("global_load_dwordx2 a[188:189], %0, %1 sc1\n\tglobal_load_dwordx2 a[190:191], %0, %2 sc1" :: "v"(off8[7]), "s"(G), "s"(GT));
 #define DQ_W6_LOADSET_2_PLAIN asm volatile("global_load_dwordx2 a[192:193], %0, %1\n\tglobal_load_dwordx2 a[194:195], %0, %2" :: "v"(off8[0]), "s"(G), "s"(GT)); asm volatile("global_load_dwordx2 a[196:197], %0, %1\n\tglobal_load_dwordx2 a[198:199], %0, %2" :: "v"(off8[1]), "s"(G), "s"(GT)); asm volatile("global_load_dwordx2 a[200:201], %0, %1\n\tglobal_load_dwordx2 a[202:203], %0, %2" :: "v"(off8[2]), "s"(G), "s"(GT)); asm volatile("global_load_dwordx2 a[204:205], %0, %1\n\tglobal_load_dwordx2 a[206:207], %0, %2" :: "v"(off8[3]), "s"(G), "s"(GT)); asm volatile("global_load_dwordx2 a[208:209], %0, %1\n\tglobal_load_dwordx2 a[210:211], %0, %2" :: "v"(off8[4]), "s"(G), "s"(GT)); asm volatile("global_load_dwordx2 a[212:213], %0, %1\n\tglobal_load_dwordx2 a[214:215], %0, %2" :: "v"(off8[5]), "s"(G), "s"(GT)); asm volatile("global_load_dwordx2 a[216:217], %0, %1\n\tglobal_load_dwordx2 a[218:219], %0, %2" :: "v"(off8[6]), "s"(G), "s"(GT)); asm volatile("global_load_dwordx2 a[220:221], %0, %1\n\tglobal_load_dwordx2 a[222:223], %0, %2" :: "v"(off8[7]), "s"(G), "s"(GT));
 #define DQ_W6_LOADSET_2_COH asm volatile("global_load_dwordx2 a[192:193], %0, %1 sc1\n\tglobal_load_dwordx2 a[194:195], %0, %2 sc1" :: "v"(off8[0]), "s"(G), "s"(GT)); asm volatile("global_load_dwordx2 a[196:197], %0, %1 sc1\n\tglobal_load_dwordx2 a[198:199], %0, %2 sc1" :: "v"(off8[1]), "s"(G), "s"(GT)); asm volatile("global_load_dwordx2 a[200:201], %0, %1 sc1\n\tglobal_load_dwordx2 a[202:203], %0, %2 sc1" :: "v"(off8[2]), "s"(G), "s"(GT)); asm volatile("global_load_dwordx2 a[204:205], %0, %1 sc1\n\tglobal_load_dwordx2 a[206:207], %0, %2 sc1" :: "v"(off8[3]), "s"(G), "s"(GT)); asm volatile("global_load_dwordx2 a[208:209], %0, %1 sc1\n\tglobal_load_dwordx2 a[210:211], %0, %2 sc1" :: "v"(off8[4]), "s"(G), "s"(GT)); asm volatile("global_load_dwordx2 a[212:213], %0, %1 sc1\n\tglobal_load_dwordx2 a[214:215], %0, %2 sc1" :: "v"(off8[5]), "s"(G), "s"(GT)); asm volatile("global_load_dwordx2 a[216:217], %0, %1 sc1\n\tglobal_load_dwordx2 a[218:219], %0, %2 sc1" :: "v"(off8[6]), "s"(G), "s"(GT)); asm volatile("global_load_dwordx2 a[220:221], %0, %1 sc1\n\tglobal_load_dwordx2 a[222:223], %0, %2 sc1" :: "v"(off8[7]), "s"(G), "s"(GT));
-#define DQ_W6_PICK(SEL) do { const unsigned poff_ = (unsigned)__builtin_amdgcn_readfirstlane((int)(12u + (unsigned)(SEL) * 40u)); asm volatile("s_getpc_b64 s[96:97]\n\ts_add_u32 s96, s96, %4\n\ts_addc_u32 s97, s97, 0\n\ts_setpc_b64 s[96:97]\n\t" "v_accvgpr_read_b32 %0, a128\n\tv_accvgpr_read_b32 %1, a129\n\tv_accvgpr_read_b32 %2, a130\n\tv_accvgpr_read_b32 %3, a131\n\ts_branch 1f\n\ts_nop 0\n\t" "v_accvgpr_read_b32 %0, a132\n\tv_accvgpr_read_b32 %1, a133\n\tv_accvgpr_read_b32 %2, a134\n\tv_accvgpr_read_b32 %3, a135\n\ts_branch 1f\n\ts_nop 0\n\t" "v_accvgpr_read_b32 %0, a136\n\tv_accvgpr_read_b32 %1, a137\n\tv_accvgpr_read_b32 %2, a138\n\tv_accvgpr_read_b32 %3, a139\n\ts_branch 1f\n\ts_nop 0\n\t" "v_accvgpr_read_b32 %0, a140\n\tv_accvgpr_read_b32 %1, a141\n\tv_accvgpr_read_b32 %2, a142\n\tv_accvgpr_read_b32 %3, a143\n\ts_branch 1f\n\ts_nop 0\n\t" "v_accvgpr_read_b32 %0, a144\n\tv_accvgpr_read_b32 %1, a145\n\tv_accvgpr_read_b32 %2, a146\n\tv_accvgpr_read_b32 %3, a147\n\ts_branch 1f\n\ts_nop 0\n\t" "v_accvgpr_read_b32 %0, a148\n\tv_accvgpr_read_b32 %1, a149\n\tv_accvgpr_read_b32 %2, a150\n\tv_accvgpr_read_b32 %3, a151\n\ts_branch 1f\n\ts_nop 0\n\t" "v_accvgpr_read_b32 %0, a152\n\tv_accvgpr_read_b32 %1, a153\n\tv_accvgpr_read_b32 %2, a154\n\tv_accvgpr_read_b32 %3, a155\n\ts_branch 1f\n\ts_nop 0\n\t" "v_accvgpr_read_b32 %0, a156\n\tv_accvgpr_read_b32 %1, a157\n\tv_accvgpr_read_b32 %2, a158\n\tv_accvgpr_read_b32 %3, a159\n\ts_branch 1f\n\ts_nop 0\n\t" "v_accvgpr_read_b32 %0, a160\n\tv_accvgpr_read_b32 %1, a161\n\tv_accvgpr_read_b32 %2, a162\n\tv_accvgpr_read_b32 %3, a163\n\ts_branch 1f\n\ts_nop 0\n\t" "v_accvgpr_read_b32 %0, a164\n\tv_accvgpr_read_b32 %1, a165\n\tv_accvgpr_read_b32 %2, a166\n\tv_accvgpr_read_b32 %3, a167\n\ts_branch 1f\n\ts_nop 0\n\t" "v_accvgpr_read_b32 %0, a168\n\tv_accvgpr_read_b32 %1, a169\n\tv_accvgpr_read_b32 %2, a170\n\tv_accvgpr_read_b32 %3, a171\n\ts_branch 1f\n\ts_nop 0\n\t" "v_accvgpr_read_b32 %0, a172\n\tv_accvgpr_read_b32 %1, a173\n\tv_accvgpr_read_b32 %2, a174\n\tv_accvgpr_read_b32 %3, a175\n\ts_branch 1f\n\ts_nop 0\n\t" "v_accvgpr_read_b32 %0, a176\n\tv_accvgpr_read_b32 %1, a177\n\tv_accvgpr_read_b32 %2, a178\n\tv_accvgpr_read_b32 %3, a179\n\ts_branch 1f\n\ts_nop 0\n\t" "v_accvgpr_read_b32 %0, a180\n\tv_accvgpr_read_b32 %1, a181\n\tv_accvgpr_read_b32 %2, a182\n\tv_accvgpr_read_b32 %3, a183\n\ts_branch 1f\n\ts_nop 0\n\t" "v_accvgpr_read_b32 %0, a184\n\tv_accvgpr_read_b32 %1, a185\n\tv_accvgpr_read_b32 %2, a186\n\tv_accvgpr_read_b32 %3, a187\n\ts_branch 1f\n\ts_nop 0\n\t" "v_accvgpr_read_b32 %0, a188\n\tv_accvgpr_read_b32 %1, a189\n\tv_accvgpr_read_b32 %2, a190\n\tv_accvgpr_read_b32 %3, a191\n\ts_branch 1f\n\ts_nop 0\n\t" "v_accvgpr_read_b32 %0, a192\n\tv_accvgpr_read_b32 %1, a193\n\tv_accvgpr_read_b32 %2, a194\n\tv_accvgpr_read_b32 %3, a195\n\ts_branch 1f\n\ts_nop 0\n\t" "v_accvgpr_read_b32 %0, a196\n\tv_accvgpr_read_b32 %1, a197\n\tv_accvgpr_read_b32 %2, a198\n\tv_accvgpr_read_b32 %3, a199\n\ts_branch 1f\n\ts_nop 0\n\t" "v_accvgpr_read_b32 %0, a200\n\tv_accvgpr_read_b32 %1, a201\n\tv_accvgpr_read_b32 %2, a202\n\tv_accvgpr_read_b32 %3, a203\n\ts_branch 1f\n\ts_nop 0\n\t" "v_accvgpr_read_b32 %0, a204\n\tv_accvgpr_read_b32 %1, a205\n\tv_accvgpr_read_b32 %2, a206\n\tv_accvgpr_read_b32 %3, a207\n\ts_branch 1f\n\ts_nop 0\n\t" "v_accvgpr_read_b32 %0, a208\n\tv_accvgpr_read_b32 %1, a209\n\tv_accvgpr_read_b32 %2, a210\n\tv_accvgpr_read_b32 %3, a211\n\ts_branch 1f\n\ts_nop 0\n\t" "v_accvgpr_read_b32 %0, a212\n\tv_accvgpr_read_b32 %1, a213\n\tv_accvgpr_read_b32 %2, a214\n\tv_accvgpr_read_b32 %3, a215\n\ts_branch 1f\n\ts_nop 0\n\t" "v_accvgpr_read_b32 %0, a216\n\tv_accvgpr_read_b32 %1, a217\n\tv_accvgpr_read_b32 %2, a218\n\tv_accvgpr_read_b32 %3, a219\n\ts_branch 1f\n\ts_nop 0\n\t" "v_accvgpr_read_b32 %0, a220\n\tv_accvgpr_read_b32 %1, a221\n\tv_accvgpr_read_b32 %2, a222\n\tv_accvgpr_read_b32 %3, a223\n\ts_branch 1f\n\ts_nop 0\n\t" "1:" : "=v"(ulo), "=v"(uhi), "=v"(wlo), "=v"(whi) : "s"(poff_) : "s96", "s97", "scc"); } while (0)
+#define DQ_W6_LOADSET_3_PLAIN asm volatile("global_load_dwordx2 a[224:225], %0, %1\n\tglobal_load_dwordx2 a[226:227], %0, %2" :: "v"(off8[0]), "s"(G), "s"(GT)); asm volatile("global_load_dwordx2 a[228:229], %0, %1\n\tglobal_load_dwordx2 a[230:231], %0, %2" :: "v"(off8[1]), "s"(G), "s"(GT)); asm volatile("global_load_dwordx2 a[232:233], %0, %1\n\tglobal_load_dwordx2 a[234:235], %0, %2" :: "v"(off8[2]), "s"(G), "s"(GT)); asm volatile("global_load_dwordx2 a[236:237], %0, %1\n\tglobal_load_dwordx2 a[238:239], %0, %2" :: "v"(off8[3]), "s"(G), "s"(GT)); asm volatile("global_load_dwordx2 a[240:241], %0, %1\n\tglobal_load_dwordx2 a[242:243], %0, %2" :: "v"(off8[4]), "s"(G), "s"(GT)); asm volatile("global_load_dwordx2 a[244:245], %0, %1\n\tglobal_load_dwordx2 a[246:247], %0, %2" :: "v"(off8[5]), "s"(G), "s"(GT)); asm volatile("global_load_dwordx2 a[248:249], %0, %1\n\tglobal_load_dwordx2 a[250:251], %0, %2" :: "v"(off8[6]), "s"(G), "s"(GT)); asm volatile("global_load_dwordx2 a[252:253], %0, %1\n\tglobal_load_dwordx2 a[254:255], %0, %2" :: "v"(off8[7]), "s"(G), "s"(GT));
+#define DQ_W6_LOADSET_3_COH asm volatile("global_load_dwordx2 a[224:225], %0, %1 sc1\n\tglobal_load_dwordx2 a[226:227], %0, %2 sc1" :: "v"(off8[0]), "s"(G), "s"(GT)); asm volatile("global_load_dwordx2 a[228:229], %0, %1 sc1\n\tglobal_load_dwordx2 a[230:231], %0, %2 sc1" :: "v"(off8[1]), "s"(G), "s"(GT)); asm volatile("global_load_dwordx2 a[232:233], %0, %1 sc1\n\tglobal_load_dwordx2 a[234:235], %0, %2 sc1" :: "v"(off8[2]), "s"(G), "s"(GT)); asm volatile("global_load_dwordx2 a[236:237], %0, %1 sc1\n\tglobal_load_dwordx2 a[238:239], %0, %2 sc1" :: "v"(off8[3]), "s"(G), "s"(GT)); asm volatile("global_load_dwordx2 a[240:241], %0, %1 sc1\n\tglobal_load_dwordx2 a[242:243], %0, %2 sc1" :: "v"(off8[4]), "s"(G), "s"(GT)); asm volatile("global_load_dwordx2 a[244:245], %0, %1 sc1\n\tglobal_load_dwordx2 a[246:247], %0, %2 sc1" :: "v"(off8[5]), "s"(G), "s"(GT)); asm volatile("global_load_dwordx2 a[248:249], %0, %1 sc1\n\tglobal_load_dwordx2 a[250:251], %0, %2 sc1" :: "v"(off8[6]), "s"(G), "s"(GT)); asm volatile("global_load_dwordx2 a[252:253], %0, %1 sc1\n\tglobal_load_dwordx2 a[254:255], %0, %2 sc1" :: "v"(off8[7]), "s"(G), "s"(GT));
+#define DQ_W6_PICK(SEL) do { const unsigned poff_ = (unsigned)__builtin_amdgcn_readfirstlane((int)(12u + (unsigned)(SEL) * 40u)); asm volatile("s_getpc_b64 s[96:97]\n\ts_add_u32 s96, s96, %4\n\ts_addc_u32 s97, s97, 0\n\ts_setpc_b64 s[96:97]\n\t" "v_accvgpr_read_b32 %0, a128\n\tv_accvgpr_read_b32 %1, a129\n\tv_accvgpr_read_b32 %2, a130\n\tv_accvgpr_read_b32 %3, a131\n\ts_branch 1f\n\ts_nop 0\n\t" "v_accvgpr_read_b32 %0, a132\n\tv_accvgpr_read_b32 %1, a133\n\tv_accvgpr_read_b32 %2, a134\n\tv_accvgpr_read_b32 %3, a135\n\ts_branch 1f\n\ts_nop 0\n\t" "v_accvgpr_read_b32 %0, a136\n\tv_accvgpr_read_b32 %1, a137\n\tv_accvgpr_read_b32 %2, a138\n\tv_accvgpr_read_b32 %3, a139\n\ts_branch 1f\n\ts_nop 0\n\t" "v_accvgpr_read_b32 %0, a140\n\tv_accvgpr_read_b32 %1, a141\n\tv_accvgpr_read_b32 %2, a142\n\tv_accvgpr_read_b32 %3, a143\n\ts_branch 1f\n\ts_nop 0\n\t" "v_accvgpr_read_b32 %0, a144\n\tv_accvgpr_read_b32 %1, a145\n\tv_accvgpr_read_b32 %2, a146\n\tv_accvgpr_read_b32 %3, a147\n\ts_branch 1f\n\ts_nop 0\n\t" "v_accvgpr_read_b32 %0, a148\n\tv_accvgpr_read_b32 %1, a149\n\tv_accvgpr_read_b32 %2, a150\n\tv_accvgpr_read_b32 %3, a151\n\ts_branch 1f\n\ts_nop 0\n\t" "v_accvgpr_read_b32 %0, a152\n\tv_accvgpr_read_b32 %1, a153\n\tv_accvgpr_read_b32 %2, a154\n\tv_accvgpr_read_b32 %3, a155\n\ts_branch 1f\n\ts_nop 0\n\t" "v_accvgpr_read_b32 %0, a156\n\tv_accvgpr_read_b32 %1, a157\n\tv_accvgpr_read_b32 %2, a158\n\tv_accvgpr_read_b32 %3, a159\n\ts_branch 1f\n\ts_nop 0\n\t" "v_accvgpr_read_b32 %0, a160\n\tv_accvgpr_read_b32 %1, a161\n\tv_accvgpr_read_b32 %2, a162\n\tv_accvgpr_read_b32 %3, a163\n\ts_branch 1f\n\ts_nop 0\n\t" "v_accvgpr_read_b32 %0, a164\n\tv_accvgpr_read_b32 %1, a165\n\tv_accvgpr_read_b32 %2, a166\n\tv_accvgpr_read_b32 %3, a167\n\ts_branch 1f\n\ts_nop 0\n\t" "v_accvgpr_read_b32 %0, a168\n\tv_accvgpr_read_b32 %1, a169\n\tv_accvgpr_read_b32 %2, a170\n\tv_accvgpr_read_b32 %3, a171\n\ts_branch 1f\n\ts_nop 0\n\t" "v_accvgpr_read_b32 %0, a172\n\tv_accvgpr_read_b32 %1, a173\n\tv_accvgpr_read_b32 %2, a174\n\tv_accvgpr_read_b32 %3, a175\n\ts_branch 1f\n\ts_nop 0\n\t" "v_accvgpr_read_b32 %0, a176\n\tv_accvgpr_read_b32 %1, a177\n\tv_accvgpr_read_b32 %2, a178\n\tv_accvgpr_read_b32 %3, a179\n\ts_branch 1f\n\ts_nop 0\n\t" "v_accvgpr_read_b32 %0, a180\n\tv_accvgpr_read_b32 %1, a181\n\tv_accvgpr_read_b32 %2, a182\n\tv_accvgpr_read_b32 %3, a183\n\ts_branch 1f\n\ts_nop 0\n\t" "v_accvgpr_read_b32 %0, a184\n\tv_accvgpr_read_b32 %1, a185\n\tv_accvgpr_read_b32 %2, a186\n\tv_accvgpr_read_b32 %3, a187\n\ts_branch 1f\n\ts_nop 0\n\t" "v_accvgpr_read_b32 %0, a188\n\tv_accvgpr_read_b32 %1, a189\n\tv_accvgpr_read_b32 %2, a190\n\tv_accvgpr_read_b32 %3, a191\n\ts_branch 1f\n\ts_nop 0\n\t" "v_accvgpr_read_b32 %0, a192\n\tv_accvgpr_read_b32 %1, a193\n\tv_accvgpr_read_b32 %2, a194\n\tv_accvgpr_read_b32 %3, a195\n\ts_branch 1f\n\ts_nop 0\n\t" "v_accvgpr_read_b32 %0, a196\n\tv_accvgpr_read_b32 %1, a197\n\tv_accvgpr_read_b32 %2, a198\n\tv_accvgpr_read_b32 %3, a199\n\ts_branch 1f\n\ts_nop 0\n\t" "v_accvgpr_read_b32 %0, a200\n\tv_accvgpr_read_b32 %1, a201\n\tv_accvgpr_read_b32 %2, a202\n\tv_accvgpr_read_b32 %3, a203\n\ts_branch 1f\n\ts_nop 0\n\t" "v_accvgpr_read_b32 %0, a204\n\tv_accvgpr_read_b32 %1, a205\n\tv_accvgpr_read_b32 %2, a206\n\tv_accvgpr_read_b32 %3, a207\n\ts_branch 1f\n\ts_nop 0\n\t" "v_accvgpr_read_b32 %0, a208\n\tv_accvgpr_read_b32 %1, a209\n\tv_accvgpr_read_b32 %2, a210\n\tv_accvgpr_read_b32 %3, a211\n\ts_branch 1f\n\ts_nop 0\n\t" "v_accvgpr_read_b32 %0, a212\n\tv_accvgpr_read_b32 %1, a213\n\tv_accvgpr_read_b32 %2, a214\n\tv_accvgpr_read_b32 %3, a215\n\ts_branch 1f\n\ts_nop 0\n\t" "v_accvgpr_read_b32 %0, a216\n\tv_accvgpr_read_b32 %1, a217\n\tv_accvgpr_read_b32 %2, a218\n\tv_accvgpr_read_b32 %3, a219\n\ts_branch 1f\n\ts_nop 0\n\t" "v_accvgpr_read_b32 %0, a220\n\tv_accvgpr_read_b32 %1, a221\n\tv_accvgpr_read_b32 %2, a222\n\tv_accvgpr_read_b32 %3, a223\n\ts_branch 1f\n\ts_nop 0\n\t" "v_accvgpr_read_b32 %0, a224\n\tv_accvgpr_read_b32 %1, a225\n\tv_accvgpr_read_b32 %2, a226\n\tv_accvgpr_read_b32 %3, a227\n\ts_branch 1f\n\ts_nop 0\n\t" "v_accvgpr_read_b32 %0, a228\n\tv_accvgpr_read_b32 %1, a229\n\tv_accvgpr_read_b32 %2, a230\n\tv_accvgpr_read_b32 %3, a231\n\ts_branch 1f\n\ts_nop 0\n\t" "v_accvgpr_read_b32 %0, a232\n\tv_accvgpr_read_b32 %1, a233\n\tv_accvgpr_read_b32 %2, a234\n\tv_accvgpr_read_b32 %3, a235\n\ts_branch 1f\n\ts_nop 0\n\t" "v_accvgpr_read_b32 %0, a236\n\tv_accvgpr_read_b32 %1, a237\n\tv_accvgpr_read_b32 %2, a238\n\tv_accvgpr_read_b32 %3, a239\n\ts_branch 1f\n\ts_nop 0\n\t" "v_accvgpr_read_b32 %0, a240\n\tv_accvgpr_read_b32 %1, a241\n\tv_accvgpr_read_b32 %2, a242\n\tv_accvgpr_read_b32 %3, a243\n\ts_branch 1f\n\ts_nop 0\n\t" "v_accvgpr_read_b32 %0, a244\n\tv_accvgpr_read_b32 %1, a245\n\tv_accvgpr_read_b32 %2, a246\n\tv_accvgpr_read_b32 %3, a247\n\ts_branch 1f\n\ts_nop 0\n\t" "v_accvgpr_read_b32 %0, a248\n\tv_accvgpr_read_b32 %1, a249\n\tv_accvgpr_read_b32 %2, a250\n\tv_accvgpr_read_b32 %3, a251\n\ts_branch 1f\n\ts_nop 0\n\t" "v_accvgpr_read_b32 %0, a252\n\tv_accvgpr_read_b32 %1, a253\n\tv_accvgpr_read_b32 %2, a254\n\tv_accvgpr_read_b32 %3, a255\n\ts_branch 1f\n\ts_nop 0\n\t" "1:" : "=v"(ulo), "=v"(uhi), "=v"(wlo), "=v"(whi) : "s"(poff_) : "s96", "s97", "scc"); } while (0)
 #define DQ_W6_PAIRS do { const unsigned off_ = (unsigned)__builtin_amdgcn_readfirstlane((int)(12u + (unsigned)(32 - k) * 16u)); asm("s_getpc_b64 s[96:97]\n\t" "s_add_u32 s96, s96, %[off]\n\t" "s_addc_u32 s97, s97, 0\n\t" "s_setpc_b64 s[96:97]\n\t" "v_fmac_f64_dpp %[u1], %[pby], v[190:191] row_newbcast:15 row_mask:0xf bank_mask:0xf\n\t" "v_fmac_f64_dpp %[w1], %[pbx], v[254:255] row_newbcast:15 row_mask:0xf bank_mask:0xf\n\t" "v_fmac_f64_dpp %[uj], %[pby], v[188:189] row_newbcast:14 row_mask:0xf bank_mask:0xf\n\t" "v_fmac_f64_dpp %[wj], %[pbx], v[252:253] row_newbcast:14 row_mask:0xf bank_mask:0xf\n\t" "v_fmac_f64_dpp %[u1], %[pby], v[186:187] row_newbcast:13 row_mask:0xf bank_mask:0xf\n\t" "v_fmac_f64_dpp %[w1], %[pbx], v[250:251] row_newbcast:13 row_mask:0xf bank_mask:0xf\n\t" "v_fmac_f64_dpp %[uj], %[pby], v[184:185] row_newbcast:12 row_mask:0xf bank_mask:0xf\n\t" "v_fmac_f64_dpp %[wj], %[pbx], v[248:249] row_newbcast:12 row_mask:0xf bank_mask:0xf\n\t" "v_fmac_f64_dpp %[u1], %[pby], v[182:183] row_newbcast:11 row_mask:0xf bank_mask:0xf\n\t" "v_fmac_f64_dpp %[w1], %[pbx], v[246:247] row_newbcast:11 row_mask:0xf bank_mask:0xf\n\t" "v_fmac_f64_dpp %[uj], %[pby], v[180:181] row_newbcast:10 row_mask:0xf bank_mask:0xf\n\t" "v_fmac_f64_dpp %[wj], %[pbx], v[244:245] row_newbcast:10 row_mask:0xf bank_mask:0xf\n\t" "v_fmac_f64_dpp %[u1], %[pby], v[178:179] row_newbcast:9 row_mask:0xf bank_mask:0xf\n\t" "v_fmac_f64_dpp %[w1], %[pbx], v[242:243] row_newbcast:9 row_mask:0xf bank_mask:0xf\n\t" "v_fmac_f64_dpp %[uj], %[pby], v[176:177] row_newbcast:8 row_mask:0xf bank_mask:0xf\n\t" "v_fmac_f64_dpp %[wj], %[pbx], v[240:241] row_newbcast:8 row_mask:0xf bank_mask:0xf\n\t" "v_fmac_f64_dpp %[u1], %[pby], v[174:175] row_newbcast:7 row_mask:0xf bank_mask:0xf\n\t" "v_fmac_f64_dpp %[w1], %[pbx], v[238:239] row_newbcast:7 row_mask:0xf bank_mask:0xf\n\t" "v_fmac_f64_dpp %[uj], %[pby], v[172:173] row_newbcast:6 row_mask:0xf bank_mask:0xf\n\t" "v_fmac_f64_dpp %[wj], %[pbx], v[236:237] row_newbcast:6 row_mask:0xf bank_mask:0xf\n\t" "v_fmac_f64_dpp %[u1], %[pby], v[170:171] row_newbcast:5 row_mask:0xf bank_mask:0xf\n\t" "v_fmac_f64_dpp %[w1], %[pbx], v[234:235] row_newbcast:5 row_mask:0xf bank_mask:0xf\n\t" "v_fmac_f64_dpp %[uj], %[pby], v[168:169] row_newbcast:4 row_mask:0xf bank_mask:0xf\n\t" "v_fmac_f64_dpp %[wj], %[pbx], v[232:233] row_newbcast:4 row_mask:0xf bank_mask:0xf\n\t" "v_fmac_f64_dpp %[u1], %[pby], v[166:167] row_newbcast:3 row_mask:0xf bank_mask:0xf\n\t" "v_fmac_f64_dpp %[w1], %[pbx], v[230:231] row_newbcast:3 row_mask:0xf bank_mask:0xf\n\t" "v_fmac_f64_dpp %[uj], %[pby], v[164:165] row_newbcast:2 row_mask:0xf bank_mask:0xf\n\t" "v_fmac_f64_dpp %[wj], %[pbx], v[228:229] row_newbcast:2 row_mask:0xf bank_mask:0xf\n\t" "v_fmac_f64_dpp %[u1], %[pby], v[162:163] row_newbcast:1 row_mask:0xf bank_mask:0xf\n\t" "v_fmac_f64_dpp %[w1], %[pbx], v[226:227] row_newbcast:1 row_mask:0xf bank_mask:0xf\n\t" "v_fmac_f64_dpp %[uj], %[pby], v[160:161] row_newbcast:0 row_mask:0xf bank_mask:0xf\n\t" "v_fmac_f64_dpp %[wj], %[pbx], v[224:225] row_newbcast:0 row_mask:0xf bank_mask:0xf\n\t" "v_fmac_f64_dpp %[u1], %[pay], v[158:159] row_newbcast:15 row_mask:0xf bank_mask:0xf\n\t" "v_fmac_f64_dpp %[w1], %[pax], v[222:223] row_newbcast:15 row_mask:0xf bank_mask:0xf\n\t" "v_fmac_f64_dpp %[uj], %[pay], v[156:157] row_newbcast:14 row_mask:0xf bank_mask:0xf\n\t" "v_fmac_f64_dpp %[wj], %[pax], v[220:221] row_newbcast:14 row_mask:0xf bank_mask:0xf\n\t" "v_fmac_f64_dpp %[u1], %[pay], v[154:155] row_newbcast:13 row_mask:0xf bank_mask:0xf\n\t" "v_fmac_f64_dpp %[w1], %[pax], v[218:219] row_newbcast:13 row_mask:0xf bank_mask:0xf\n\t" "v_fmac_f64_dpp %[uj], %[pay], v[152:153] row_newbcast:12 row_mask:0xf bank_mask:0xf\n\t" "v_fmac_f64_dpp %[wj], %[pax], v[216:217] row_newbcast:12 row_mask:0xf bank_mask:0xf\n\t" "v_fmac_f64_dpp %[u1], %[pay], v[150:151] row_newbcast:11 row_mask:0xf bank_mask:0xf\n\t" "v_fmac_f64_dpp %[w1], %[pax], v[214:215] row_newbcast:11 row_mask:0xf bank_mask:0xf\n\t" "v_fmac_f64_dpp %[uj], %[pay], v[148:149] row_newbcast:10 row_mask:0xf bank_mask:0xf\n\t" "v_fmac_f64_dpp %[wj], %[pax], v[212:213] row_newbcast:10 row_mask:0xf bank_mask:0xf\n\t" "v_fmac_f64_dpp %[u1], %[pay], v[146:147] row_newbcast:9 row_mask:0xf bank_mask:0xf\n\t" "v_fmac_f64_dpp %[w1], %[pax], v[210:211] row_newbcast:9 row_mask:0xf bank_mask:0xf\n\t" "v_fmac_f64_dpp %[uj], %[pay], v[144:145] row_newbcast:8 row_mask:0xf bank_mask:0xf\n\t" "v_fmac_f64_dpp %[wj], %[pax], v[208:209] row_newbcast:8 row_mask:0xf bank_mask:0xf\n\t" "v_fmac_f64_dpp %[u1], %[pay], v[142:143] row_newbcast:7 row_mask:0xf bank_mask:0xf\n\t" "v_fmac_f64_dpp %[w1], %[pax], v[206:207] row_newbcast:7 row_mask:0xf bank_mask:0xf\n\t" "v_fmac_f64_dpp %[uj], %[pay], v[140:141] row_newbcast:6 row_mask:0xf bank_mask:0xf\n\t" "v_fmac_f64_dpp %[wj], %[pax], v[204:205] row_newbcast:6 row_mask:0xf bank_mask:0xf\n\t" "v_fmac_f64_dpp %[u1], %[pay], v[138:139] row_newbcast:5 row_mask:0xf bank_mask:0xf\n\t" "v_fmac_f64_dpp %[w1], %[pax], v[202:203] row_newbcast:5 row_mask:0xf bank_mask:0xf\n\t" "v_fmac_f64_dpp %[uj], %[pay], v[136:137] row_newbcast:4 row_mask:0xf bank_mask:0xf\n\t" "v_fmac_f64_dpp %[wj], %[pax], v[200:201] row_newbcast:4 row_mask:0xf bank_mask:0xf\n\t" "v_fmac_f64_dpp %[u1], %[pay], v[134:135] row_newbcast:3 row_mask:0xf bank_mask:0xf\n\t" "v_fmac_f64_dpp %[w1], %[pax], v[198:199] row_newbcast:3 row_mask:0xf bank_mask:0xf\n\t" "v_fmac_f64_dpp %[uj], %[pay], v[132:133] row_newbcast:2 row_mask:0xf bank_mask:0xf\n\t" "v_fmac_f64_dpp %[wj], %[pax], v[196:197] row_newbcast:2 row_mask:0xf bank_mask:0xf\n\t" "v_fmac_f64_dpp %[u1], %[pay], v[130:131] row_newbcast:1 row_mask:0xf bank_mask:0xf\n\t" "v_fmac_f64_dpp %[w1], %[pax], v[194:195] row_newbcast:1 row_mask:0xf bank_mask:0xf\n\t" "v_fmac_f64_dpp %[uj], %[pay], v[128:129] row_newbcast:0 row_mask:0xf bank_mask:0xf\n\t" "v_fmac_f64_dpp %[wj], %[pax], v[192:193] row_newbcast:0 row_mask:0xf bank_mask:0xf" : [uj] "+v"(uj), [wj] "+v"(wj), [u1] "+v"(u1), [w1] "+v"(w1) : [pax] "v"(pa.x), [pay] "v"(pa.y), [pbx] "v"(pb.x), [pby] "v"(pb.y), [off] "s"(off_) : "s96", "s97", "scc"); } while (0)
 #define DQ_W6_SETPAIR(PU, WJ) asm volatile("s_set_gpr_idx_on %4, gpr_idx(DST)\n\tv_mov_b32 v128, %0\n\tv_mov_b32 v129, %1\n\tv_mov_b32 v192, %2\n\tv_mov_b32 v193, %3\n\ts_set_gpr_idx_off" :: "v"(__double2loint(PU)), "v"(__double2hiint(PU)), "v"(__double2loint(WJ)), "v"(__double2hiint(WJ)), "s"(__builtin_amdgcn_readfirstlane(2 * k)) : "m0")
 #define DQ_W6_DUMP do { const unsigned long long rowpair_bytes = 16ull * (unsigned)n; unsigned long long ua_ = (unsigned long long)Up + 16ull * (unsigned)j, wa_ = (unsigned long long)Wp + 16ull * (unsigned)j; \
```
